# salute-developers/GigaAM

Hardware: AMD Instinct MI355X
Metric: RTFx v2_ctc batch32x20s (log-mel + encoder + greedy decode) (higher is better)
Workload: dtype f32 (GEMMs: 3-term split on fp16 MFMA, fp32 accumulate)

## Files before the change

### gigaam_amd/_lib.py

```python
from __future__ import annotations

import ctypes as C
import os
from typing import Optional

_HERE = os.path.dirname(os.path.abspath(__file__))
LIB_NAME = "libgigaam_hip.so"
LIB_PATH = os.path.join(_HERE, LIB_NAME)

SUBS_CONV2D, SUBS_CONV1D = 0, 1
ATT_ROTARY, ATT_REL_POS = 0, 1
NORM_BATCH, NORM_LAYER = 0, 1
HEAD_NONE, HEAD_CTC, HEAD_RNNT, HEAD_EMO = 0, 1, 2, 3
DTYPE_F32, DTYPE_F16, DTYPE_BF16, DTYPE_F64, DTYPE_I64 = 0, 1, 2, 3, 4
GEMM_F32, GEMM_F16X3, GEMM_F16 = 0, 1, 2
RS_U8, RS_I16, RS_I24, RS_I32, RS_F32, RS_MULAW, RS_ALAW = range(7)
RS_FORM_SINGLE, RS_FORM_TABLE, RS_FORM_ROWS = 0, 1, 2
PF_CLASSES = ["gemm", "conv2", "attn", "norm", "convmod", "stem", "frontend", "decode", "misc", "align_bt", "align_out"]


class GamConfig(C.Structure):
    _fields_ = [(n, C.c_int32) for n in (
        "sample_rate", "n_mels", "hop_length", "win_length", "n_fft", "center",
        "feat_in", "n_layers", "d_model", "subsampling", "subs_kernel_size", "subsampling_factor",
# ... 30 lines not shown
    "gam_ctc_greedy": (C.c_int, [_P, _P, _P, C.c_int, C.c_int64, _P, _P, _P, _P]),
    "gam_ctc_align": (C.c_int, [_P, _P, _P, C.c_int, C.c_int64, _P, _P, C.c_int, _P, _P, _P, _P, _P, _P, _P]),
    "gam_op_ctc_align": (C.c_int, [_P, _P, _P, C.c_int, C.c_int64, C.c_int, _P, _P, C.c_int, _P, _P, _P, _P, _P, _P, _P]),
    "gam_op_ctc_align_long": (C.c_int, [_P, _P, C.c_int64, C.c_int, _P, C.c_int, _P, _P, _P, _P, _P, _P, _P]),
    "gam_op_ctc_star_row": (C.c_int, [_P, _P, _P, C.c_int, C.c_int64, C.c_int, C.c_float, _P, _P]),
    "gam_ctc_align_star": (C.c_int, [_P, _P, _P, C.c_int, C.c_int64, _P, _P, C.c_int, C.c_float, _P, _P, _P, _P, _P, _P, _P]),
    "gam_op_ctc_align_star": (C.c_int, [_P, _P, _P, C.c_int, C.c_int64, C.c_int, _P, _P, _P, C.c_int, _P, _P, _P, _P, _P, _P, _P]),
    "gam_op_ctc_align_long_star": (C.c_int, [_P, _P, C.c_int64, C.c_int, _P, _P, C.c_int, _P, _P, _P, _P, _P, _P, _P]),
    "gam_op_ctc_stitch": (C.c_int, [_P, _P, _P, C.c_int, C.c_int64, C.c_int, _P, _P, _P, _P, C.c_int64, _P, _P]),
    "gam_op_ctc_greedy_long": (C.c_int, [_P, _P, C.c_int64, C.c_int, _P, _P, _P, _P]),
    "gam_set_ctc_align_workspace": (C.c_int, [_P, C.c_int64]),
    "gam_tune_ctc_align_long": (C.c_int, [C.c_int, C.c_int]),
    "gam_ctc_kws": (C.c_int, [_P, _P, _P, C.c_int, C.c_int64, C.c_int, _P, _P, _P, _P, _P, _P]),
    "gam_op_ctc_kws": (C.c_int, [_P, _P, _P, C.c_int, C.c_int64, C.c_int, C.c_int, _P, _P, _P, _P, _P, _P]),
    "gam_set_keywords": (C.c_int, [_P, _P, _P, C.c_int, _P]),
    "gam_ctc_kws_state_bytes": (C.c_int64, [_P]),
    "gam_op_ctc_kws_stream": (C.c_int, [_P, _P, C.c_int64, C.c_int, C.c_int64, C.c_int, _P, C.c_int, _P, _P, _P, _P, _P, _P, _P]),
    "gam_ctc_beam": (C.c_int, [_P, _P, _P, C.c_int, C.c_int64, C.c_int, _P, _P, _P, _P, _P, _P]),
    "gam_op_ctc_beam": (C.c_int, [_P, _P, _P, C.c_int, C.c_int64, C.c_int, C.c_int, _P, _P, _P, _P, _P, _P]),
    "gam_ctc_beam_stream_bytes": (C.c_int64, [_P, C.c_int, C.c_int64]),
    "gam_op_ctc_beam_stream": (C.c_int, [_P, _P, C.c_int64, C.c_int, C.c_int64, C.c_int, C.c_int, _P, C.c_int64, _P, _P, _P, _P, _P, _P, _P]),
    "gam_set_hotwords": (C.c_int, [_P, _P, _P, C.c_int, C.c_float]),
    "gam_set_lm": (C.c_int, [_P, _P, C.c_int, _P, C.c_int64, C.c_int, _P, C.c_int64, C.c_int, C.c_int, C.c_int, C.c_int, C.c_int,
                             C.c_float, C.c_float, C.c_float]),
    "gam_rnnt_greedy": (C.c_int, [_P, _P, _P, C.c_int, C.c_int64, C.c_int, _P, _P, _P, _P, _P, C.c_int, _P]),
    "gam_ctc_beam_nbest": (C.c_int, [_P, _P, _P, C.c_int, C.c_int64, C.c_int, C.c_int, _P, _P, _P, _P, _P, _P, _P]),
    "gam_op_ctc_beam_nbest": (C.c_int, [_P, _P, _P, C.c_int, C.c_int64, C.c_int, C.c_int, C.c_int, _P, _P, _P, _P, _P, _P, _P]),
    "gam_rnnt_beam_nbest": (C.c_int, [_P, _P, _P, C.c_int, C.c_int64, C.c_int, C.c_int, C.c_int, _P, _P, _P, _P, _P, _P, _P]),
    "gam_op_rnnt_beam_nbest": (C.c_int, [_P, _P, _P, C.c_int, C.c_int64, C.c_int, C.c_int, C.c_int, _P, _P, _P, _P, _P, _P, _P]),
    "gam_rnnt_beam": (C.c_int, [_P, _P, _P, C.c_int, C.c_int64, C.c_int, C.c_int, _P, _P, _P, _P, _P, _P]),
    "gam_op_rnnt_beam": (C.c_int, [_P, _P, _P, C.c_int, C.c_int64, C.c_int, C.c_int, _P, _P, _P, _P, _P, _P]),
    "gam_rnnt_align": (C.c_int, [_P, _P, _P, C.c_int, C.c_int64, _P, _P, C.c_int, _P, _P, _P, _P, _P]),
    "gam_op_rnnt_align": (C.c_int, [_P, _P, _P, C.c_int, C.c_int64, _P, _P, C.c_int, _P, _P, _P, _P, _P, _P]),
    "gam_op_rnnt_lattice_align": (C.c_int, [_P, _P, _P, C.c_int, C.c_int64, C.c_int, _P, _P, C.c_int, _P, _P, _P, _P, _P]),
    "gam_set_rnnt_align_workspace": (C.c_int, [_P, C.c_int64]),
    "gam_ctc_confidence": (C.c_int, [_P, _P, _P, C.c_int, C.c_int64, _P, _P, _P, C.c_int, C.c_int, C.c_int, _P, _P, _P, _P]),
    "gam_op_ctc_confidence": (C.c_int, [_P, _P, _P, C.c_int, C.c_int64, C.c_int, _P, _P, _P, C.c_int, C.c_int, C.c_int, _P, _P, _P, _P]),
    "gam_rnnt_confidence": (C.c_int, [_P, _P, _P, C.c_int, C.c_int64, _P, _P, _P, C.c_int, C.c_int, _P, _P, _P]),
    "gam_op_rnnt_confidence": (C.c_int, [_P, _P, _P, C.c_int, C.c_int64, _P, _P, _P, C.c_int, C.c_int, _P, _P, _P]),
    "gam_emo_probs": (C.c_int, [_P, _P, _P, C.c_int, C.c_int64, _P, _P]),
    "gam_rnnt_predict": (C.c_int, [_P, _P, _P, _P, C.c_int, _P, _P, _P, _P]),
    "gam_rnnt_joint": (C.c_int, [_P, _P, _P, C.c_int, C.c_int, C.c_int, _P, _P]),
    "gam_set_gemm_mode": (C.c_int, [_P, C.c_int]),
    "gam_get_gemm_mode": (C.c_int, [_P]),
    "gam_set_rnnt_cluster": (C.c_int, [_P, C.c_int]),
    "gam_get_rnnt_cluster": (C.c_int, [_P]),
    "gam_rnnt_cluster_plan_info": (C.c_int, [C.c_int] * 8 + [C.POINTER(C.c_int32)]),
    "gam_rnnt_last_decode": (C.c_int, [_P, C.POINTER(C.c_int32)]),
    "gam_debug_buffer_hash": (C.c_int, [_P, C.c_int, C.POINTER(C.c_uint64), C.POINTER(C.c_int64)]),
    "gam_range_flag": (C.c_int, [_P, C.POINTER(C.c_int), _P]),
    "gam_range_flag_fetch": (C.c_int, [_P, _P, _P]),
    "gam_op_gemm": (C.c_int, [_P, _P, _P, _P, _P, C.c_int, C.c_int, C.c_int, C.c_int, _P]),
    "gam_op_gemm_ex": (C.c_int, [_P, _P, _P, _P, _P, C.c_float, _P, C.c_int, C.c_int, C.c_int, C.c_int, _P]),
    "gam_op_attention": (C.c_int, [_P, _P, _P, _P, _P, _P, C.c_int, C.c_int, C.c_int, _P]),
    "gam_op_attention_ex": (C.c_int, [_P, _P, _P, _P, C.c_int64, _P, _P, _P, C.c_int, C.c_int, C.c_int, C.c_int, _P, _P, _P, _P]),
    "gam_op_layernorm": (C.c_int, [_P, C.POINTER(GamLnOp), _P]),
    "gam_op_convmod": (C.c_int, [_P, _P, _P, _P, _P, _P, _P, _P, _P, C.c_int, C.c_int, C.c_int, C.c_int, C.c_int, C.c_int, C.c_int, _P]),
    "gam_tune_sp": (C.c_int, [C.c_int, C.c_int, C.c_int]),
    "gam_plan_sp": (C.c_int, [C.c_int, C.c_int, C.c_int, C.c_int, C.POINTER(C.c_int), C.POINTER(C.c_int), C.POINTER(C.c_int)]),
    "gam_plan_sp_ex": (C.c_int, [C.c_int, C.c_int, C.c_int, C.c_int, C.POINTER(C.c_int), C.POINTER(C.c_int), C.POINTER(C.c_int), C.POINTER(C.c_int)]),
    "gam_tune_sp_stages": (C.c_int, [C.c_int]),
    "gam_resample_plan": (C.c_int, [C.c_int, C.c_int, C.POINTER(C.c_int), C.POINTER(C.c_int), C.POINTER(C.c_int)]),
    "gam_resample_tile": (C.c_int, [C.c_int, C.c_int, C.POINTER(C.c_int), C.POINTER(C.c_int)]),
    "gam_resample_table": (C.c_int, [C.c_int, C.c_int, _P, _P]),
    "gam_resample_out_len": (C.c_int64, [C.c_int, C.c_int, C.c_int64]),
    "gam_op_resample": (C.c_int, [_P, C.c_int, C.c_int, C.c_int, _P, C.c_int, C.c_int64, C.c_int, C.c_int, _P, _P, _P, C.c_int64, _P, _P]),
    "gam_profile_enable": (C.c_int, [_P, C.c_int]),
    "gam_profile_pause": (C.c_int, [_P, C.c_int]),
    "gam_profile_read": (C.c_int, [_P, C.c_int, C.POINTER(C.c_double), C.POINTER(C.c_int64), C.POINTER(C.c_double)]),
    "gam_profile_read_bytes": (C.c_int, [_P, C.c_int, C.POINTER(C.c_double)]),
    "gam_last_error": (C.c_char_p, [_P]),
    "gam_comm_unique_id": (C.c_int, [C.c_char_p]),
    "gam_comm_create": (C.c_int, [C.c_char_p, C.c_int, C.c_int, C.c_int, C.POINTER(_P)]),
    "gam_comm_world": (C.c_int, [_P]),
    "gam_gather_ids": (C.c_int, [_P, _P, _P, _P, _P, C.c_int, C.c_int, _P, _P, _P, _P, _P]),
    "gam_comm_last_error": (C.c_char_p, [_P]),
    "gam_comm_destroy": (None, [_P]),
}

_lib: Optional[C.CDLL] = None


class GigaAMHipError(RuntimeError):
    pass


def load_library(path: Optional[str] = None) -> C.CDLL:
    global _lib
    if _lib is not None and path is None:
        return _lib
    p = path or os.environ.get("GIGAAM_HIP_LIB", LIB_PATH)
    if not os.path.exists(p):
        raise GigaAMHipError(
            f"{p} not found: the HIP extension is not built. Run `python -c 'import __graft_entry__ as g; g.build()'` "
            "(hipcc --offload-arch=gfx950). There is no CPU fallback.")
    lib = C.CDLL(p)
    for name, (res, args) in SIGNATURES.items():
        fn = getattr(lib, name)
        fn.restype = res
        fn.argtypes = args
    if lib.gam_abi_version() != 1:
        raise GigaAMHipError("libgigaam_hip.so ABI version mismatch")
    if path is None:
        _lib = lib
    return lib
```

### gigaam_amd/csrc/gam_api.hip

```cpp
#include <hip/hip_runtime.h>

#include <algorithm>
#include <cmath>
#include <cstdarg>
#include <cstdio>
#include <cstring>
#include <map>
#include <string>
#include <vector>

#include "../../include/gigaam_hip.h"
#include "gam_align.h"
#include "gam_align_long.h"
#include "gam_kws.h"
#include "gam_attn.h"
#include "gam_beam.h"
#include "gam_beam_stream.h"
#include "gam_rnnt_beam.h"
#include "gam_attn16.h"
#include "gam_comm.h"
#include "gam_common.h"
#include "gam_convmod.h"
#include "gam_decode.h"
#include "gam_rnnt_align.h"
// ... 2 lines not shown
#include "gam_frontend.h"
#include "gam_gemm.h"
#include "gam_gemm_sp.h"
#include "gam_norm.h"
#include "gam_pack.h"
#include "gam_resample.h"
#include "gam_stem.h"
#include "gam_stitch.h"

namespace {

struct HostTensor {
  std::vector<float> data;
  std::vector<int64_t> shape;
  int64_t numel() const {
    int64_t n = 1;
    for (auto s : shape) n *= s;
    return n;
  }
};

struct DevBuf {
  float* p = nullptr;
  size_t cap = 0;
  DevBuf() = default;
  DevBuf(DevBuf&& o) noexcept : p(o.p), cap(o.cap) { o.p = nullptr; o.cap = 0; }
  DevBuf& operator=(DevBuf&& o) noexcept { std::swap(p, o.p); std::swap(cap, o.cap); return *this; }
  ~DevBuf() { (void)release(); }
  hipError_t release() {
    const hipError_t e = p ? hipFree(p) : hipSuccess;
    p = nullptr; cap = 0;
    return e;
  }
  hipError_t alloc(size_t floats) {
    hipError_t e = release();
    if (e == hipSuccess) e = hipMalloc(&p, floats * sizeof(float));
    if (e == hipSuccess) cap = floats; else p = nullptr;
    return e;
  }
  template <class T> T* as() const { return reinterpret_cast<T*>(p); }
};

struct W16 {
  _Float16* sp = nullptr;
  _Float16* h16 = nullptr;
  float inv = 1.0f;
};

struct LayerW {
  float *ln_ff1_w, *ln_ff1_b, *ff1_w1, *ff1_b1, *ff1_w2, *ff1_b2;
  float *ln_att_w, *ln_att_b, *wqkv, *bqkv, *wo, *bo;
  float *wpos, *pos_u, *pos_v;
  float *ln_conv_w, *ln_conv_b, *pw1_w, *pw1_b, *dw_w, *dw_b, *cn_scale, *cn_shift, *pw2_w, *pw2_b;
  float *ln_ff2_w, *ln_ff2_b, *ff2_w1, *ff2_b1, *ff2_w2, *ff2_b2;
  float *ln_out_w, *ln_out_b;
  W16 s_ff1_w1, s_ff1_w2, s_wqkv, s_wo, s_wpos, s_pw1, s_pw2, s_ff2_w1, s_ff2_w2;
};

struct ProfEvent {
  hipEvent_t a, b;
  int cls;
};

}

struct gam_handle {
  gam_config cfg;
  int device = 0;
  bool finalized = false;
  bool has_encoder = false, has_head = false;
  std::map<std::string, HostTensor> staged;
  std::vector<DevBuf> owned;
  std::string err;

  float* dft_basis = nullptr;
  int* mel_band = nullptr;
  float* mel_wts = nullptr;
  int mel_nw = 0;
  int nf = 0, kpad = 0;
  float *c1_w = nullptr, *c1_b = nullptr, *c2_w = nullptr, *c2_b = nullptr, *lin_w = nullptr, *lin_b = nullptr;
  W16 s_c1, s_c2, s_lin;
  int gemm_mode = 1;
  int f1 = 0, f2 = 0;
  std::vector<LayerW> layers;
  float *rot_cos = nullptr, *rot_sin = nullptr;
  float* rel_pe = nullptr;
  float* rel_pe_sp = nullptr;
  float *ctc_w = nullptr, *ctc_b = nullptr;
  float *emo_w = nullptr, *emo_b = nullptr;
  float *jn_enc_w = nullptr, *jn_enc_b = nullptr, *jn_pred_t = nullptr, *jn_pred_b = nullptr;
  float *jn_out_w = nullptr, *jn_out_b = nullptr, *lstm_whh_t = nullptr, *lstm_tab = nullptr;
  float *lstm_whh_q = nullptr, *jn_pred_q = nullptr;
  float* jn_pred_w = nullptr;
  DevBuf jz, jp, jl;
  float *lstm_wih_x = nullptr, *lstm_whh_x = nullptr, *lstm_bias_x = nullptr;
  int use_rowscale = 1;
  int use_range = 1;
  int ncu = 256;
  int rnnt_cluster = -1;
  int rnnt_coop = 1;
  int rnnt_force_timeout = 0;
  int rnnt_no_repair = 0;
  int rnnt_exclusive = 0;
  int last_rnnt_c = 0, last_rnnt_kern = -1, last_rnnt_refused = 0;
  DevBuf rnnt_x;
  hipEvent_t dec_evt = nullptr;
  hipStream_t dec_stream = nullptr;
  bool dec_evt_set = false;

  DevBuf wavp, spec, img, c2, xin, y1, x, y, yr, hbuf, qkv, ctx, ubuf, zbuf, tok, logits, encp, pbuf, aplanes;
  DevBuf op_planes, op_sp, splitk_ws;
  DevBuf align_star;
  DevBuf align_bp;
  DevBuf align_long_ws;
  DevBuf greedy_long_ws;
  size_t al_ws_limit = GAM_AL_WS_DEFAULT;
  DevBuf beam_nodes;
  DevBuf rb_ws, rb_nodes;
  DevBuf ra_g, ra_pp, ra_lat, ra_bp;
  DevBuf cf_stats;
  size_t ra_ws_limit = GAM_RA_WS_DEFAULT;
  DevBuf hw_trie;
  int hw_nodes = 0, hw_words = 0, hw_max_tok = -1;
  float hw_boost = 0.f;
  int hw_gen = 0, lm_gen = 0;
  DevBuf kw_dev;
  int kw_K = 0, kw_ntok = 0, kw_max_tok = -1;
  int kw_gen = 0;
  DevBuf kws_mb;
  DevBuf lm_cls, lm_wt, lm_ng;
  int lm_V = 0, lm_wslots = 0, lm_wprobe = 0, lm_nslots = 0, lm_nprobe = 0, lm_order = 0, lm_bos = 0, lm_eos = 0, lm_unk = 0;
  float lm_unk_logp = 0.f, lm_alpha = 0.f, lm_beta = 0.f;
  DevBuf dec_splitk_ws;
  int last_rows = 0, last_rows_padded = 0;
  DevBuf pack_idx;
  int use_pack = 1;
  int use_splitk = 1;
  int fuse_reduce = 1;
  int use_graph = 1;
  int graph_max_rows = 2048;
  uint64_t ws_generation = 0;
  struct GraphEntry {
    enum Seen { UNSEEN, SEEN_ONCE, PLAIN_ONLY };
    uint64_t gen = 0; Seen seen = UNSEEN; hipGraphExec_t exec = nullptr;
  };
  std::map<std::vector<int>, GraphEntry> graphs;
  long graph_replays = 0, graph_captures_failed = 0;
  int graph_count = 0;
  hipStream_t cap_stream = nullptr;
  DevBuf lens;
  DevBuf rsbuf, op_rs;
  int* range_flag = nullptr;

  int prof_on = 0;
  std::vector<ProfEvent> prof_events;
  size_t prof_used = 0;
  double prof_work[GAM_PF_NCLASS] = {0};
  double prof_bytes[GAM_PF_NCLASS] = {0};
  int64_t prof_launches[GAM_PF_NCLASS] = {0};
};

namespace {

int fail(gam_handle* h, int code, const char* fmt, ...) {
  char buf[512];
  va_list ap;
  va_start(ap, fmt);
  vsnprintf(buf, sizeof buf, fmt, ap);
  va_end(ap);
  if (h) h->err = buf;
  return code;
}

#define HIPCHK(h, expr)                                                                        \
  do {                                                                                         \
    hipError_t e_ = (expr);                                                                    \
    if (e_ != hipSuccess) return fail(h, -2, "%s failed: %s (%s:%d)", #expr, hipGetErrorString(e_), __FILE__, __LINE__); \
  } while (0)

void* dev_upload(gam_handle* h, const void* src, size_t bytes, size_t alloc_bytes) {
  h->owned.emplace_back();
  DevBuf& b = h->owned.back();
  if (b.alloc((alloc_bytes + 3) / 4) != hipSuccess) return nullptr;
  if (src && bytes && hipMemcpy(b.p, src, bytes, hipMemcpyHostToDevice) != hipSuccess) return nullptr;
  return b.p;
}

float* upload(gam_handle* h, const std::vector<float>& v) {
  return (float*)dev_upload(h, v.data(), v.size() * sizeof(float), std::max<size_t>(v.size(), 4) * sizeof(float));
}

// ... 104 lines not shown
  gam_handle* h;
  hipStream_t s;
  ProfEvent* ev = nullptr;
  ProfScope(gam_handle* h_, hipStream_t s_, int cls, double work) : h(h_), s(s_) {
    if (!h->prof_on || (h->prof_on == 2 && cls != GAM_PF_GEMM && cls != GAM_PF_CONV2)) return;
    if (h->prof_used == h->prof_events.size()) {
      ProfEvent e;
      if (hipEventCreate(&e.a) != hipSuccess || hipEventCreate(&e.b) != hipSuccess) return;
      h->prof_events.push_back(e);
    }
    ev = &h->prof_events[h->prof_used++];
    ev->cls = cls;
    h->prof_work[cls] += work;
    h->prof_launches[cls] += 1;
    hipEventRecord(ev->a, s);
  }
  ~ProfScope() {
    if (ev) hipEventRecord(ev->b, s);
  }
};

struct PendingReduce {
  const float* part = nullptr;
  int nsplit = 0;
  const float* bias = nullptr;
  const float* resid = nullptr;
  float alpha = 1.0f;
  GamGemmArgs full;
  int act = 0;
  void clear() { part = nullptr; nsplit = 0; }
};

int flush_pending(gam_handle* h, hipStream_t s, PendingReduce* p) {
  if (p == nullptr || p->part == nullptr) return 0;
  const hipError_t e = gam_launch_splitk_reduce(p->full, p->act, p->nsplit, s);
  const int M = p->full.M, N = p->full.N;
  p->clear();
  if (e != hipSuccess) return fail(h, -2, "split-K reduce launch (M=%d N=%d): %s", M, N, hipGetErrorString(e));
  return 0;
}

static inline bool split_mode(const gam_handle* h) { return h->gemm_mode != GAM_GEMM_F32; }

int gemm(gam_handle* h, hipStream_t s, const GamGemmArgs& a_in, int act, int cls = GAM_PF_GEMM, const W16* w16 = nullptr,
         PendingReduce* defer = nullptr) {
  GamGemmArgs a = a_in;
  if (int r = flush_pending(h, s, defer)) return r;
  a.range_flag = h->use_range ? h->range_flag : nullptr;
  if (!split_mode(h)) a.c_guard = 0;
  ProfScope ps(h, s, cls, 2.0 * (double)a.M * (double)a.N * (double)a.K);
  if (ps.ev) {
    const double abytes = a.a_mode == 0 ? ((double)(a.M - 1) * (double)std::min<long>(a.lda, a.K) + a.K) * 4.0
                                        : (double)a.M / a.conv_f2 * 2.0 * a.conv_fp * a.conv_c * 4.0;
    h->prof_bytes[cls] += abytes * (a.n_switch > 0 ? 2.0 : 1.0) + 4.0 * a.N * a.K + 4.0 * a.M * a.N * (a.R ? 2.0 : 1.0);
  }
  hipError_t e;
  if (a.Asp != nullptr) {
    if (!split_mode(h)) return fail(h, -2, "sp32 A operand outside the split-fp16 GEMM mode");
    if (w16 == nullptr || w16->sp == nullptr) return fail(h, -2, "sp32 A without sp32 W planes");
    a.wscale_inv = w16->inv;
    a.Wsp = w16->sp;
    a.h16 = 0;
    if (a.a_fmt == 2) {
      if (a.K % 64 != 0 || (a.a_mode == 0 ? a.lda % 64 != 0 : a.conv_c % 64 != 0) || w16->h16 == nullptr)
        return fail(h, -2, "GAM_GEMM_F16: K / row pitch of a GEMM operand is not a multiple of 64 (M=%d N=%d K=%d)", a.M, a.N, a.K);
      a.h16 = 1; a.K /= 2; a.lda /= 2; a.conv_c /= 2;
      a.Wsp = w16->h16;
    }
    GamSpPlan plan = gam_gemm_sp_plan(a.M, a.N, a.K, a.a_mode, h->ncu);
    if (!h->use_splitk) plan.s = 1;
    a.sp_mt = plan.mt; a.sp_nw = plan.nw; a.sp_ns = plan.ns;
    GamGemmArgs full = a;
    if (plan.s > 1) {
      if (int r = ensure(h, h->splitk_ws, (size_t)plan.s * a.M * a.N + 64)) return r;
      a.splitk = plan.s; a.partial = h->splitk_ws.p;
    }
    e = gam_launch_gemm_sp(a, act, s);
    if (e != hipSuccess) return fail(h, -2, "sp gemm launch (M=%d N=%d K=%d): %s", a.M, a.N, a.K, hipGetErrorString(e));
    if (plan.s > 1 && defer != nullptr && h->fuse_reduce && act == GAM_ACT_NONE && !a.c_split && !a.c_guard && a.lens == nullptr &&
        !a.remap && a.ldc == a.N && a.bias != nullptr && a.R != nullptr && a.ldr == a.N) {
      defer->part = a.partial; defer->nsplit = plan.s; defer->bias = a.bias; defer->resid = a.R; defer->alpha = a.alpha;
      defer->full = full; defer->full.partial = a.partial; defer->act = act;
    } else if (plan.s > 1) {
      full.partial = a.partial;
      e = gam_launch_splitk_reduce(full, act, plan.s, s);
      if (e != hipSuccess) return fail(h, -2, "split-K reduce launch (M=%d N=%d): %s", a.M, a.N, hipGetErrorString(e));
    }
    return 0;
  }
  if (a.a_rs != nullptr || a.c_split) return fail(h, -2, "row-scaled A or split C without sp32 operands (M=%d N=%d K=%d)", a.M, a.N, a.K);
  int S = 1;
  if (h->use_splitk && a.a_mode == 0 && a.K % 32 == 0) {
    const int tiles = gam_cdiv(a.M, 128) * gam_cdiv(a.N, 128), nk = a.K / 32, ncu = 256;
    if (tiles * 2 <= ncu && nk >= 4) {
      S = std::min(16, std::min(ncu / tiles, nk / 2));
      while (S > 1 && nk % S != 0) --S;
    }
  }
  GamGemmArgs full = a;
  if (S > 1) {
    DevBuf& ws = cls == GAM_PF_DECODE ? h->dec_splitk_ws : h->splitk_ws;
    if (int r = ensure(h, ws, (size_t)S * a.M * a.N + 64)) return r;
    a.splitk = S; a.ldw = a.K; a.K = a.K / S; a.partial = ws.p;
  }
  e = gam_launch_gemm(a, act, s);
  if (e != hipSuccess) return fail(h, -2, "gemm launch (M=%d N=%d K=%d): %s", a.M, a.N, a.K, hipGetErrorString(e));
  if (S > 1) {
// ... 33 lines not shown

int64_t half_up(int64_t l) { return l <= 0 ? 0 : (l + 1) / 2; }

struct DecodeScope {
  gam_handle* h;
  hipStream_t s;
  DecodeScope(gam_handle* h_, hipStream_t s_) : h(h_), s(s_) {
    if (h->dec_evt == nullptr && hipEventCreateWithFlags(&h->dec_evt, hipEventDisableTiming) != hipSuccess) { h->dec_evt = nullptr; (void)hipGetLastError(); }
    if (h->dec_evt != nullptr && h->dec_evt_set && h->dec_stream != s) (void)hipStreamWaitEvent(s, h->dec_evt, 0);
  }
  ~DecodeScope() {
    if (h->dec_evt != nullptr && hipEventRecord(h->dec_evt, s) == hipSuccess) { h->dec_stream = s; h->dec_evt_set = true; }
  }
};

#define GAM_DECODE_ENTRY(h, stream)      \
  hipStream_t s = (hipStream_t)(stream); \
  if (!(h)) return -1;                   \
  HIPCHK(h, hipSetDevice((h)->device));  \
  DecodeScope ds(h, s)

int head_check(gam_handle* h, int want, const char* who) {
  if (!h) return -1;
  if (who && !h->finalized) return fail(h, -1, "%s before gam_finalize", who);
  if (h->cfg.head_type != want || !h->has_head)
    return fail(h, -1, "model has no %s head", want == GAM_HEAD_CTC ? "CTC" : want == GAM_HEAD_RNNT ? "RNN-T" : "emotion");
  return 0;
}

template <class Args> void rnnt_pred_weights(const gam_handle* h, Args& a) {
  a.gate_tab = h->lstm_tab; a.whh_t = h->lstm_whh_t; a.wih_x = h->lstm_wih_x; a.whh_x = h->lstm_whh_x; a.bias_x = h->lstm_bias_x;
}
template <class Args> void rnnt_joint_weights(const gam_handle* h, Args& a) {
  a.wpred_t = h->jn_pred_t; a.bpred = h->jn_pred_b; a.wout = h->jn_out_w; a.bout = h->jn_out_b;
}

}

extern "C" {

int gam_abi_version(void) { return GAM_ABI_VERSION; }

const char* gam_last_error(const gam_handle* h) { return h ? h->err.c_str() : "null handle"; }

int gam_create(const gam_config* cfg, int device_id, gam_handle** out) {
  if (!cfg || !out) return -1;
  gam_handle* h = new gam_handle();
  h->cfg = *cfg;
  h->device = device_id;
  *out = h;
  if (const char* e = getenv("GAM_SPLITK")) h->use_splitk = atoi(e);
  if (const char* e = getenv("GAM_PACK")) h->use_pack = atoi(e);
  if (const char* e = getenv("GAM_FUSE_REDUCE")) h->fuse_reduce = atoi(e);
  if (const char* e = getenv("GAM_GRAPH")) h->use_graph = atoi(e);
  if (const char* e = getenv("GAM_GRAPH_MAX_ROWS")) h->graph_max_rows = atoi(e);
  if (const char* e = getenv("GAM_RNNT_CLUSTER")) h->rnnt_cluster = std::max(-1, std::min(8, atoi(e)));
  if (const char* e = getenv("GAM_RNNT_ALIGN_WS")) h->ra_ws_limit = (size_t)std::max(1ll, atoll(e));
  if (const char* e = getenv("GAM_CTC_ALIGN_WS")) h->al_ws_limit = (size_t)std::max(1ll, atoll(e));
  if (const char* e = getenv("GAM_RNNT_EXCLUSIVE")) h->rnnt_exclusive = atoi(e);
  if (const char* e = getenv("GAM_RNNT_COOP")) h->rnnt_coop = atoi(e);
  if (const char* e = getenv("GAM_RNNT_FORCE_TIMEOUT")) h->rnnt_force_timeout = atoi(e);
  if (const char* e = getenv("GAM_RNNT_NO_REPAIR")) h->rnnt_no_repair = atoi(e);
  {
    int n = 0;
    if (hipDeviceGetAttribute(&n, hipDeviceAttributeMultiprocessorCount, device_id) == hipSuccess && n > 0) h->ncu = n;
    int co = 0;
    if (hipDeviceGetAttribute(&co, hipDeviceAttributeCooperativeLaunch, device_id) != hipSuccess || co == 0) h->rnnt_coop = 0;
  }
  if (const char* e = getenv("GAM_ROWSCALE")) h->use_rowscale = atoi(e);
  if (const char* e = getenv("GAM_RANGE")) h->use_range = atoi(e);
  if (const char* e = getenv("GAM_GEMM_MODE"))
    h->gemm_mode = strcmp(e, "f32") == 0 ? GAM_GEMM_F32 : (strcmp(e, "f16") == 0 ? GAM_GEMM_F16 : GAM_GEMM_F16X3);
  const gam_config& c = h->cfg;
  if (c.d_model <= 0 || c.n_heads <= 0 || c.d_model % c.n_heads != 0)
    return fail(h, -1, "bad d_model/n_heads %d/%d", c.d_model, c.n_heads);
  if (c.d_model / c.n_heads != GAM_ATT_DK) return fail(h, -1, "head dim %d unsupported (kernels are built for %d)", c.d_model / c.n_heads, GAM_ATT_DK);
  if (c.d_model % 64 != 0 || c.d_model > 1024) return fail(h, -1, "d_model %d unsupported", c.d_model);
  if (c.subsampling_factor != 4) return fail(h, -1, "subsampling_factor %d unsupported", c.subsampling_factor);
  if (c.subsampling == GAM_SUBS_CONV2D && c.subs_kernel_size != 3) return fail(h, -1, "conv2d stem needs kernel 3");
  if (c.subsampling == GAM_SUBS_CONV1D && c.subs_kernel_size != 5) return fail(h, -1, "conv1d stem needs kernel 5");
  if (c.win_length != c.n_fft) return fail(h, -1, "win_length != n_fft unsupported");
  if (c.n_mels > 64 || c.n_mels != c.feat_in) return fail(h, -1, "n_mels %d / feat_in %d unsupported", c.n_mels, c.feat_in);
  if (c.head_type == GAM_HEAD_RNNT && (c.pred_rnn_layers < 1 || c.pred_rnn_layers > 4 || c.pred_hidden > GAM_RNNT_MAXH || c.joint_hidden > GAM_RNNT_MAXH || c.num_classes > GAM_RNNT_MAXV || c.joint_hidden % 16 != 0 || c.pred_hidden % 16 != 0))
    return fail(h, -1, "RNN-T head shape unsupported");
  if (hipSetDevice(device_id) != hipSuccess) return fail(h, -2, "hipSetDevice(%d) failed", device_id);
  return 0;
}

void gam_destroy(gam_handle* h) {
  if (!h) return;
  hipSetDevice(h->device);
  for (auto& e : h->prof_events) { hipEventDestroy(e.a); hipEventDestroy(e.b); }
  for (auto& g : h->graphs)
    if (g.second.exec) hipGraphExecDestroy(g.second.exec);
  if (h->cap_stream) hipStreamDestroy(h->cap_stream);
  if (h->dec_evt) hipEventDestroy(h->dec_evt);
  if (getenv("GAM_GRAPH_DEBUG")) fprintf(stderr, "[gam] graph replays %ld, failed captures %ld\n", h->graph_replays, h->graph_captures_failed);
  delete h;
}

int gam_set_weight(gam_handle* h, const char* key, const void* host_ptr, int dtype, const int64_t* shape, int ndim) {
  if (!h || !key || !host_ptr) return -1;
  if (h->finalized) return fail(h, -1, "gam_set_weight after gam_finalize");
  HostTensor t;
  for (int i = 0; i < ndim; ++i) t.shape.push_back(shape[i]);
  const int64_t n = t.numel();
// ... 148 lines not shown
  if (int r = need(h, pe + "conv.0.bias", C, &b0)) return r;
  if (int r = need(h, pe + "conv.2.weight", (int64_t)C * C * ks, &w2)) return r;
  if (int r = need(h, pe + "conv.2.bias", C, &b2)) return r;
  const std::vector<float> r0 = swap_inner(w0->data, C, F, ks), r2 = swap_inner(w2->data, C, C, ks);
  if (int r = upload_to(h, DST(h->c1_w), r0)) return r;
  if (int r = up_split(h, r0, &h->s_c1, ks * F)) return r;
  if (int r = upload_to(h, DST(h->c1_b), b0->data)) return r;
  if (int r = upload_to(h, DST(h->c2_w), r2)) return r;
  if (int r = up_split(h, r2, &h->s_c2, ks * C)) return r;
  return upload_to(h, DST(h->c2_b), b2->data);
}

static int fin_qkv(gam_handle* h, const std::string& p, LayerW& L) {
  const int D = h->cfg.d_model;
  const HostTensor *wq, *bq, *wk, *bk, *wv, *bv;
  if (int r = need(h, p + "self_attn.linear_q.weight", (int64_t)D * D, &wq)) return r;
  if (int r = need(h, p + "self_attn.linear_q.bias", D, &bq)) return r;
  if (int r = need(h, p + "self_attn.linear_k.weight", (int64_t)D * D, &wk)) return r;
  if (int r = need(h, p + "self_attn.linear_k.bias", D, &bk)) return r;
  if (int r = need(h, p + "self_attn.linear_v.weight", (int64_t)D * D, &wv)) return r;
  if (int r = need(h, p + "self_attn.linear_v.bias", D, &bv)) return r;
  std::vector<float> w(wq->data), b(bq->data);
  w.insert(w.end(), wk->data.begin(), wk->data.end());
  w.insert(w.end(), wv->data.begin(), wv->data.end());
  b.insert(b.end(), bk->data.begin(), bk->data.end());
  b.insert(b.end(), bv->data.begin(), bv->data.end());
  if (int r = upload_to(h, DST(L.wqkv), w)) return r;
  if (int r = upload_to(h, DST(L.bqkv), b)) return r;
  return up_split(h, w, &L.s_wqkv, D);
}

static int fin_conv_norm(gam_handle* h, const std::string& p, LayerW& L) {
  const int D = h->cfg.d_model;
  const HostTensor *g, *be;
  if (int r = need(h, p + "conv.batch_norm.weight", D, &g)) return r;
  if (int r = need(h, p + "conv.batch_norm.bias", D, &be)) return r;
  if (h->cfg.conv_norm_type != GAM_NORM_BATCH) {
    if (int r = upload_to(h, DST(L.cn_scale), g->data)) return r;
    return upload_to(h, DST(L.cn_shift), be->data);
  }
  const HostTensor *rm, *rv;
  if (int r = need(h, p + "conv.batch_norm.running_mean", D, &rm)) return r;
  if (int r = need(h, p + "conv.batch_norm.running_var", D, &rv)) return r;
  std::vector<float> sc(D), sh(D);
  for (int i = 0; i < D; ++i) {
    const float inv = 1.0f / sqrtf(rv->data[i] + 1e-5f);
    sc[i] = g->data[i] * inv;
    sh[i] = be->data[i] - rm->data[i] * sc[i];
  }
  if (int r = upload_to(h, DST(L.cn_scale), sc)) return r;
  return upload_to(h, DST(L.cn_shift), sh);
}

static int fin_layer(gam_handle* h, int li, LayerW& L) {
  const gam_config& c = h->cfg;
  const int D = c.d_model, DFF = D * c.ff_expansion_factor;
  const std::string p = "encoder.layers." + std::to_string(li) + ".";
  memset(&L, 0, sizeof L);
  if (int r = upload_ln(h, p + "norm_feed_forward1", D, DST(L.ln_ff1_w), DST(L.ln_ff1_b))) return r;
  if (int r = upload_linear(h, p + "feed_forward1.linear1", DFF, D, DST(L.ff1_w1), DST(L.ff1_b1), &L.s_ff1_w1)) return r;
  if (int r = upload_linear(h, p + "feed_forward1.linear2", D, DFF, DST(L.ff1_w2), DST(L.ff1_b2), &L.s_ff1_w2)) return r;
  if (int r = upload_ln(h, p + "norm_self_att", D, DST(L.ln_att_w), DST(L.ln_att_b))) return r;
  if (int r = fin_qkv(h, p, L)) return r;
  if (int r = upload_linear(h, p + "self_attn.linear_out", D, D, DST(L.wo), DST(L.bo), &L.s_wo)) return r;
  if (c.self_attention_model == GAM_ATT_REL_POS) {
    const HostTensor *wp, *pu, *pv;
    if (int r = need(h, p + "self_attn.linear_pos.weight", (int64_t)D * D, &wp)) return r;
    if (int r = need(h, p + "self_attn.pos_bias_u", D, &pu)) return r;
    if (int r = need(h, p + "self_attn.pos_bias_v", D, &pv)) return r;
    if (int r = upload_to(h, DST(L.wpos), wp->data)) return r;
    if (int r = up_split(h, wp->data, &L.s_wpos, D)) return r;
    if (int r = upload_to(h, DST(L.pos_u), pu->data)) return r;
    if (int r = upload_to(h, DST(L.pos_v), pv->data)) return r;
  }
  if (int r = upload_ln(h, p + "norm_conv", D, DST(L.ln_conv_w), DST(L.ln_conv_b))) return r;
  if (int r = upload_linear(h, p + "conv.pointwise_conv1", 2 * D, D, DST(L.pw1_w), DST(L.pw1_b), &L.s_pw1)) return r;
  if (int r = upload_linear(h, p + "conv.depthwise_conv", D, c.conv_kernel_size, DST(L.dw_w), DST(L.dw_b), nullptr)) return r;
  if (int r = fin_conv_norm(h, p, L)) return r;
  if (int r = upload_linear(h, p + "conv.pointwise_conv2", D, D, DST(L.pw2_w), DST(L.pw2_b), &L.s_pw2)) return r;
  if (int r = upload_ln(h, p + "norm_feed_forward2", D, DST(L.ln_ff2_w), DST(L.ln_ff2_b))) return r;
  if (int r = upload_linear(h, p + "feed_forward2.linear1", DFF, D, DST(L.ff2_w1), DST(L.ff2_b1), &L.s_ff2_w1)) return r;
  if (int r = upload_linear(h, p + "feed_forward2.linear2", D, DFF, DST(L.ff2_w2), DST(L.ff2_b2), &L.s_ff2_w2)) return r;
  return upload_ln(h, p + "norm_out", D, DST(L.ln_out_w), DST(L.ln_out_b));
}

static int fin_rotary(gam_handle* h) {
  const int dk = h->cfg.d_model / h->cfg.n_heads, half = dk / 2, n = h->cfg.pos_emb_max_len;
  std::vector<float> cs((size_t)n * half), sn((size_t)n * half);
  for (int i = 0; i < half; ++i) {
    const float inv_freq = 1.0f / powf((float)n, (float)(2 * i) / (float)dk);
    for (int t = 0; t < n; ++t) {
      const float fr = (float)t * inv_freq;
      cs[(size_t)t * half + i] = (float)cos((double)fr);
      sn[(size_t)t * half + i] = (float)sin((double)fr);
    }
  }
  if (int r = upload_to(h, DST(h->rot_cos), cs)) return r;
  return upload_to(h, DST(h->rot_sin), sn);
}

static int fin_rel_pos(gam_handle* h) {
  const int D = h->cfg.d_model, n = h->cfg.pos_emb_max_len;
  std::vector<float> pe((size_t)(2 * n - 1) * D);
  for (int i = 0; i < D / 2; ++i) {
    const float w = expf((float)(2 * i) * (float)(-(log(10000.0) / D)));
    for (int r = -(n - 1); r <= n - 1; ++r) {
      const float ang = (float)r * w;
      pe[(size_t)(r + n - 1) * D + 2 * i] = (float)sin((double)ang);
      pe[(size_t)(r + n - 1) * D + 2 * i + 1] = (float)cos((double)ang);
    }
  }
  if (int r = upload_to(h, DST(h->rel_pe), pe)) return r;
  h->rel_pe_sp = (float*)dev_upload(h, nullptr, 0, pe.size() * sizeof(float));
  if (!h->rel_pe_sp) return fail(h, -2, "device upload failed (h->rel_pe_sp)");
  hipLaunchKernelGGL(gam_to_sp32_kernel, dim3((int)std::min<size_t>((pe.size() / 4 + 255) / 256, 4096)), dim3(256), 0, nullptr, h->rel_pe,
                     reinterpret_cast<_Float16*>(h->rel_pe_sp), pe.size() / 4, (const float*)nullptr, D);
  HIPCHK(h, hipGetLastError());
  HIPCHK(h, hipStreamSynchronize(nullptr));
  return 0;
}

static int fin_rnnt_upper(gam_handle* h) {
  const int PH = h->cfg.pred_hidden, LX = h->cfg.pred_rnn_layers - 1;
  const size_t G = (size_t)4 * PH;
  std::vector<float> wih_x(LX * PH * G), whh_x(LX * PH * G), bias_x(LX * G);
  for (int l = 1; l <= LX; ++l) {
    const std::string sfx = "_l" + std::to_string(l);
    const HostTensor *wi, *wh, *bi, *bh;
    if (int r = need(h, "head.decoder.lstm.weight_ih" + sfx, (int64_t)4 * PH * PH, &wi)) return r;
// ... 105 lines not shown
  if (B <= 0 || L <= 0) return fail(h, -1, "bad shape B=%d L=%lld", B, (long long)L);
  const gam_config& c = h->cfg;
  hipStream_t s = (hipStream_t)stream;
  HIPCHK(h, hipSetDevice(h->device));
  const int hop = c.hop_length, n = c.n_fft, half = n / 2;
  if (c.center && L <= half) return fail(h, -1, "input of %lld samples is too short for reflect padding (%d)", (long long)L, half);
  const int64_t Tf = gam_feat_frames(h, L);
  if (Tf <= 0) return fail(h, -1, "input of %lld samples yields no frames", (long long)L);
  const int64_t need = (Tf - 1) * hop + h->kpad;
  const int64_t Tfa = (need + hop - 1) / hop;
  const int64_t Lp = Tfa * hop;
  const int lds = (2 * h->nf + 3) / 4 * 4;
  if (int r = ensure(h, h->wavp, (size_t)B * Lp + h->kpad + 64)) return r;
  if (int r = ensure(h, h->spec, (size_t)B * Tfa * lds)) return r;
  {
    ProfScope ps(h, s, GAM_PF_FRONTEND, (double)B * (L + Lp) * 4.0);
    dim3 grid(gam_cdiv(Lp, 256), B);
    hipLaunchKernelGGL(gam_pad_wav_kernel, grid, dim3(256), 0, s, wav, h->wavp.p, B, (long)L, (long)Lp, half, c.center);
    HIPCHK(h, hipGetLastError());
    HIPCHK(h, hipMemsetAsync(h->wavp.p + (size_t)B * Lp, 0, (h->kpad + 64) * sizeof(float), s));
  }
  GamGemmArgs g = gemm_args(h->wavp.p, hop, h->dft_basis, nullptr, h->spec.p, lds, (int)(B * Tfa), 2 * h->nf, h->kpad);
  if (int r = gemm(h, s, g, GAM_ACT_NONE, GAM_PF_FRONTEND, nullptr)) return r;
  {
    GamPowMelArgs a;
    a.spec = h->spec.p; a.wts = h->mel_wts; a.nw = h->mel_nw; a.band = h->mel_band; a.feat = feat; a.wav_len = (const long long*)wav_len; a.feat_len = (long long*)feat_len;
    a.B = B; a.Tfa = (int)Tfa; a.Tf = (int)Tf; a.nf = h->nf; a.n_mels = c.n_mels; a.lds = lds;
    a.hop = hop; a.win = c.win_length; a.center = c.center;
    ProfScope ps(h, s, GAM_PF_FRONTEND, (double)B * Tf * (2.0 * h->nf + c.n_mels) * 4.0);
    dim3 grid(gam_cdiv(Tf, 64), B);
    const size_t pm_lds = (size_t)(64 * (h->nf + 1) + h->mel_nw) * sizeof(float);
    if (pm_lds > 160 * 1024) return fail(h, -1, "n_fft %d: the power / mel kernel's LDS image (%zu bytes) does not fit", c.n_fft, pm_lds);
    if (pm_lds > 64 * 1024) {
      static std::atomic<unsigned long long> attr_devs{0};
      HIPCHK(h, gam_set_max_lds(reinterpret_cast<const void*>(gam_powmel_kernel), (int)pm_lds, attr_devs));
    }
    hipLaunchKernelGGL(gam_powmel_kernel, grid, dim3(256), pm_lds, s, a);
    HIPCHK(h, hipGetLastError());
  }
  return 0;
}

struct EncPlan {
  int B;
  int64_t T;
  int T1, Tv;
  int Ta, N;
  int NR, Tmax;
  int T1a;
  int D, DFF, F, H, dk, nl;
  bool conv2d, rel, packed;
  bool sp;
  int spf;
  bool sp_stem;
  bool graph;
};

struct EncBufs {
  int *len0, *len1, *len2, *elen;
  int *cu, *row_t, *row_src;
  float* rs;
};

struct EncCtx {
  EncPlan p;
  EncBufs w;
  GamLnArgs ln;
};

static int enc_plan(gam_handle* h, int B, int64_t T, int n_layers_run, const int64_t* feat_len_host, EncPlan& p) {
  const gam_config& c = h->cfg;
  if (B <= 0 || T <= 0) return fail(h, -1, "bad shape B=%d T=%lld", B, (long long)T);
  p.B = B; p.T = T;
  p.D = c.d_model; p.F = c.feat_in; p.H = c.n_heads; p.dk = p.D / p.H; p.DFF = p.D * c.ff_expansion_factor;
  p.T1 = (int)half_up(T); p.Tv = (int)half_up(p.T1);
  if (p.Tv > c.pos_emb_max_len) return fail(h, -1, "%d encoder frames exceed pos_emb_max_len %d", p.Tv, c.pos_emb_max_len);
  if (p.Tv <= 0) return fail(h, -1, "no encoder frames");
  p.conv2d = c.subsampling == GAM_SUBS_CONV2D;
  p.rel = c.self_attention_model == GAM_ATT_REL_POS;
  p.nl = n_layers_run < 0 ? c.n_layers : std::min(n_layers_run, c.n_layers);
  p.Ta = p.conv2d ? std::max(p.Tv + 1, (p.T1 + 3) / 2) : std::max(p.Tv, (p.T1 + 5) / 2);
  p.N = B * p.Ta;
  const int pad = (c.subs_kernel_size - 1) / 2;
  p.T1a = p.conv2d ? 0 : std::max(p.T1, (int)((T + 2 * pad + 1) / 2));
  p.packed = false;
  p.NR = p.N; p.Tmax = p.Ta;
  const bool pack_regime = h->use_pack >= 2 || !h->use_graph || p.N >= h->graph_max_rows;
  if (feat_len_host != nullptr && h->use_pack && pack_regime && B > 1 && B <= 1024) {
    long long sum = 0;
    int mx = 0;
    for (int b = 0; b < B; ++b) {
      const int64_t l = std::min<int64_t>(std::max<int64_t>(feat_len_host[b], 0), T);
      const int l2 = (int)half_up(half_up(l));
      sum += l2;
      mx = std::max(mx, l2);
    }
    if (sum > 0 && sum * 100 <= (long long)p.N * 97) { p.packed = true; p.NR = (int)sum; p.Tmax = mx; }
  }
  p.sp = split_mode(h) && p.D % 32 == 0 && p.DFF % 32 == 0;
  const bool f16_fmt_ok = p.D % 64 == 0 && p.DFF % 64 == 0;
  p.spf = p.sp ? (h->gemm_mode == GAM_GEMM_F16 && f16_fmt_ok ? 2 : 1) : 0;
  p.sp_stem = p.sp && p.F % 32 == 0;
  p.graph = h->use_graph && !h->prof_on && p.nl > 0 && p.N < h->graph_max_rows && !p.packed;
  return 0;
}

static int enc_workspace(gam_handle* h, const EncPlan& p, EncBufs& w) {
  const size_t B = p.B, N = p.N, D = p.D, Ta = p.Ta;
  if (int r = ensure(h, h->lens, 4 * B)) return r;
  const size_t maxB = h->lens.cap / 4;
  w.len0 = h->lens.as<int>(); w.len1 = w.len0 + maxB; w.len2 = w.len0 + 2 * maxB; w.elen = w.len0 + 3 * maxB;
  if (int r = ensure(h, h->x, N * D)) return r;
  if (int r = ensure(h, h->y, N * D)) return r;
  if (int r = ensure(h, h->yr, N * D)) return r;
  if (int r = ensure(h, h->hbuf, N * p.DFF)) return r;
  if (int r = ensure(h, h->qkv, N * 3 * D)) return r;
  if (int r = ensure(h, h->ctx, N * D)) return r;
  if (int r = ensure(h, h->ubuf, N * 2 * D)) return r;
  if (int r = ensure(h, h->zbuf, N * D)) return r;
  if (int r = ensure(h, h->rsbuf, N + 64)) return r;
  if (p.packed)
    if (int r = ensure(h, h->pack_idx, (size_t)1032 + 2 * N)) return r;
  w.cu = p.packed ? reinterpret_cast<int*>(h->pack_idx.p) : nullptr;
  w.row_t = p.packed ? w.cu + 1032 : nullptr;
  w.row_src = p.packed ? w.row_t + N : nullptr;
  w.rs = p.sp && h->use_rowscale ? h->rsbuf.p : nullptr;
  if (p.conv2d) {
    if (int r = ensure(h, h->img, (B * 2 * Ta + 2) * (h->f1 + 1) * D)) return r;
    if (int r = ensure(h, h->c2, N * h->f2 * D)) return r;
  } else {
    if (int r = ensure(h, h->xin, (B * 2 * p.T1a + 8) * p.F)) return r;
    if (int r = ensure(h, h->y1, (B * 2 * Ta + 8) * D)) return r;
  }
  if (p.rel)
    if (int r = ensure(h, h->pbuf, (size_t)(2 * p.Tv - 1) * D)) return r;
  if (p.graph)
    if (int r = ensure(h, h->splitk_ws, (size_t)16 * N * std::max(p.DFF, 2 * p.D) + 64)) return r;
  return 0;
}

static GamLnArgs enc_ln_args(const gam_handle* h, const EncPlan& p, const EncBufs& w) {
  GamLnArgs ln;
  memset(&ln, 0, sizeof ln);
  ln.rows = p.NR; ln.d = p.D; ln.ta = p.Ta; ln.row_t = w.row_t; ln.dk = p.dk; ln.eps = 1e-5f; ln.rcos = h->rot_cos; ln.rsin = h->rot_sin;
  ln.rope_rows = h->cfg.pos_emb_max_len;
  ln.rs = w.rs;
  return ln;
}

static int enc_lengths(gam_handle* h, hipStream_t s, const EncPlan& p, const EncBufs& w, const int64_t* feat_len) {
  ProfScope ps(h, s, GAM_PF_MISC, 0.0);
  hipLaunchKernelGGL(gam_lengths_kernel, dim3(gam_cdiv(p.B, 64)), dim3(64), 0, s, (const long long*)feat_len, p.B, (int)p.T, 2,
                     w.len0, w.len1, w.len2, w.elen);
  HIPCHK(h, hipGetLastError());
  if (p.packed) {
    hipLaunchKernelGGL(gam_pack_index_kernel, dim3(1), dim3(256), 0, s, w.len2, p.B, p.Ta, p.NR, w.cu, w.row_t, w.row_src, h->range_flag);
    HIPCHK(h, hipGetLastError());
  }
  return 0;
}

static inline void gemm_formats(GamGemmArgs& g, int a_fmt, const float* a_rs, int c_split, int c_guard) {
  if (a_fmt) { g.Asp = reinterpret_cast<const _Float16*>(g.A); g.a_fmt = a_fmt; }
  g.a_rs = a_rs; g.c_split = c_split; g.c_guard = c_guard;
}

static int stem_conv2d(gam_handle* h, hipStream_t s, const EncPlan& p, const EncBufs& w, const float* feat) {
  const int B = p.B, Ta = p.Ta, N = p.N, C = p.D, D = p.D, FP = h->f1 + 1, F2 = h->f2;
  {
    GamConv1Args a;
    a.feat = feat; a.img = h->img.p; a.w = h->c1_w; a.bias = h->c1_b; a.len0 = w.len0; a.len1 = w.len1;
// ... 23 lines not shown
static int stem_conv1d(gam_handle* h, hipStream_t s, const EncPlan& p, const EncBufs& w, const float* feat) {
  const int B = p.B, Ta = p.Ta, T1a = p.T1a, N = p.N, C = p.D, D = p.D, F = p.F;
  const int64_t T = p.T;
  const int ks = h->cfg.subs_kernel_size, pad = (ks - 1) / 2;
  const int fmt = p.sp_stem ? 1 : 0;
  {
    ProfScope ps(h, s, GAM_PF_STEM, (double)B * T * F * 8.0);
    HIPCHK(h, hipMemsetAsync(h->xin.p, 0, ((size_t)B * 2 * T1a + 8) * F * sizeof(float), s));
    HIPCHK(h, hipMemsetAsync(h->y1.p, 0, ((size_t)B * 2 * Ta + 8) * C * sizeof(float), s));
    dim3 grid(gam_cdiv(T, 32), gam_cdiv(F, 32), B);
    int* const rf = h->use_range ? h->range_flag : nullptr;
    if (p.sp_stem) hipLaunchKernelGGL(gam_feat_to_rows_kernel<1>, grid, dim3(256), 0, s, feat, h->xin.p, w.len0, B, F, (int)T, 2 * T1a, pad, rf);
    else hipLaunchKernelGGL(gam_feat_to_rows_kernel<0>, grid, dim3(256), 0, s, feat, h->xin.p, w.len0, B, F, (int)T, 2 * T1a, pad, rf);
    HIPCHK(h, hipGetLastError());
  }
  GamGemmArgs g1 = gemm_args(h->xin.p, 2L * F, h->c1_w, h->c1_b, h->y1.p, C, B * T1a, C, ks * F);
  g1.lens = w.len1; g1.rpb = T1a; g1.fdiv = 1;
  g1.remap = 1; g1.out_rpb = 2 * Ta; g1.out_shift = pad; g1.rows_valid = std::min(T1a, 2 * Ta - pad);
  gemm_formats(g1, fmt, nullptr, fmt, 1);
  if (int r = gemm(h, s, g1, GAM_ACT_RELU, GAM_PF_CONV2, &h->s_c1)) return r;
  GamGemmArgs g2 = gemm_args(h->y1.p, 2L * C, h->c2_w, h->c2_b, p.packed ? h->y.p : h->x.p, D, N, D, ks * C);
  g2.lens = w.len2; g2.rpb = Ta; g2.fdiv = 1;
  gemm_formats(g2, fmt, nullptr, 0, 0);
  return gemm(h, s, g2, GAM_ACT_RELU, GAM_PF_CONV2, &h->s_c2);
}

static int enc_stem(gam_handle* h, hipStream_t s, const EncPlan& p, const EncBufs& w, const float* feat) {
  if (int r = p.conv2d ? stem_conv2d(h, s, p, w, feat) : stem_conv1d(h, s, p, w, feat)) return r;
  if (p.packed) {
    ProfScope ps(h, s, GAM_PF_STEM, (double)p.NR * p.D * 8.0);
    hipLaunchKernelGGL(gam_gather_rows_kernel, dim3(std::min(4096, gam_cdiv(p.NR * (p.D / 4), 256))), dim3(256), 0, s, h->y.p, w.row_src, h->x.p, p.NR, p.D);
    HIPCHK(h, hipGetLastError());
  }
  return 0;
}

static int launch_attention(gam_handle* h, hipStream_t s, const float* q, const float* k, const float* v, long ldq, float* ctx, int ctx_split,
                            const int* lens, const int* cu, int B, int Ta, int Tv, int H, const float* pbuf, const float* pos_u,
                            const float* pos_v) {
  const int D = H * GAM_ATT_DK;
  GamAttnArgs at;
  memset(&at, 0, sizeof at);
  at.q = q; at.k = k; at.v = v; at.ctx = ctx; at.ctx_split = ctx_split; at.lens = lens; at.cu = cu;
  at.B = B; at.Ta = Ta; at.Tv = Tv; at.H = H; at.ldq = ldq; at.ldv = ldq; at.ldo = D;
  at.scale = 1.0f / sqrtf((float)GAM_ATT_DK);
  at.pbuf = pbuf; at.pos_u = pos_u; at.pos_v = pos_v; at.ldp = D;
  hipError_t e = gam_launch_attn_mode(at, GAM_ATT_DK, split_mode(h), s, h->gemm_mode == GAM_GEMM_F16 ? 1 : 3, h->ncu);
  if (e != hipSuccess) return fail(h, -2, "attention launch: %s", hipGetErrorString(e));
  return 0;
}

static hipError_t launch_convmod(gam_handle* h, hipStream_t s, const float* u, float* z, const float* dw_w, const float* dw_b, const float* n_scale,
                                 const float* n_shift, const int* lens, const int* cu, int B, int Ta, int Tv, int d, int ks, bool layer_norm,
                                 int z_split) {
  GamConvModArgs cm;
  memset(&cm, 0, sizeof cm);
  cm.u = u; cm.z = z; cm.dw_w = dw_w; cm.dw_b = dw_b; cm.n_scale = n_scale; cm.n_shift = n_shift;
  cm.lens = lens; cm.cu = cu; cm.B = B; cm.Ta = Ta; cm.Tv = Tv; cm.d = d; cm.ks = ks; cm.eps = 1e-5f;
  cm.z_split = z_split; cm.range_flag = h->use_range ? h->range_flag : nullptr;
  return gam_launch_convmod(cm, layer_norm, s);
}

static int norm_to_y(gam_handle* h, hipStream_t s, const EncCtx& c, const float* w, const float* b, PendingReduce* pend) {
  GamLnArgs a = c.ln;
  a.x = h->x.p; a.out1 = h->y.p; a.w1 = w; a.b1 = b;
  a.split1 = c.p.spf;
  return layernorm(h, s, a, 0, pend);
}

static int ffn_block(gam_handle* h, hipStream_t s, const EncCtx& c, const float* w1, const float* b1, const W16& s_w1, const float* w2,
                     const float* b2, const W16& s_w2, PendingReduce* pend) {
  const int D = c.p.D, DFF = c.p.DFF, NR = c.p.NR, spf = c.p.spf;
  GamGemmArgs g = gemm_args(h->y.p, D, w1, b1, h->hbuf.p, DFF, NR, DFF, D);
  gemm_formats(g, spf, c.w.rs, spf, 1);
  if (int r = gemm(h, s, g, GAM_ACT_SILU, GAM_PF_GEMM, &s_w1)) return r;
  GamGemmArgs g2 = gemm_args(h->hbuf.p, DFF, w2, b2, h->x.p, D, NR, D, DFF);
  g2.R = h->x.p; g2.ldr = D; g2.alpha = 0.5f;
  gemm_formats(g2, spf, nullptr, 0, 0);
  return gemm(h, s, g2, GAM_ACT_NONE, GAM_PF_GEMM, &s_w2, pend);
}

static int attn_block(gam_handle* h, hipStream_t s, const EncCtx& c, const LayerW& L, PendingReduce* pend) {
  const EncPlan& p = c.p;
  const int D = p.D, NR = p.NR, Tv = p.Tv, spf = p.spf;
  float* const rs = c.w.rs;
  GamLnArgs a = c.ln;
  a.x = h->x.p; a.out1 = h->y.p; a.out2 = h->yr.p; a.w1 = L.ln_att_w; a.b1 = L.ln_att_b;
  a.split1 = spf; a.split2 = spf;
  if (int r = layernorm(h, s, a, p.rel ? 0 : 1, pend)) return r;
  const bool one_launch = p.rel || (p.sp && (2 * D) % 256 == 0);
  if (one_launch) {
    GamGemmArgs gq = gemm_args(p.rel ? h->y.p : h->yr.p, D, L.wqkv, L.bqkv, h->qkv.p, 3 * D, NR, 3 * D, D);
    gemm_formats(gq, spf, rs, 0, 1);
    if (!p.rel) { gq.Asp2 = reinterpret_cast<const _Float16*>(h->y.p); gq.n_switch = 2 * D; }
    if (int r = gemm(h, s, gq, GAM_ACT_NONE, GAM_PF_GEMM, &L.s_wqkv)) return r;
  } else {
    GamGemmArgs gq = gemm_args(h->yr.p, D, L.wqkv, L.bqkv, h->qkv.p, 3 * D, NR, 2 * D, D);
    gemm_formats(gq, spf, rs, 0, 1);
    if (int r = gemm(h, s, gq, GAM_ACT_NONE, GAM_PF_GEMM, &L.s_wqkv)) return r;
    W16 wv16 = L.s_wqkv;
    const size_t off = (size_t)2 * D * D;
    wv16.h16 += off;
    if (wv16.sp) wv16.sp += 2 * off;
    GamGemmArgs gv = gemm_args(h->y.p, D, L.wqkv + off, L.bqkv + 2 * D, h->qkv.p + 2 * D, 3 * D, NR, D, D);
    gemm_formats(gv, spf, rs, 0, 1);
    if (int r = gemm(h, s, gv, GAM_ACT_NONE, GAM_PF_GEMM, &wv16)) return r;
  }
  if (p.rel) {
    const size_t pe0 = (size_t)(h->cfg.pos_emb_max_len - 1 - (Tv - 1)) * D;
    GamGemmArgs gp = gemm_args(h->rel_pe + pe0, D, L.wpos, nullptr, h->pbuf.p, D, 2 * Tv - 1, D, D);
    if (p.sp) { gp.Asp = reinterpret_cast<const _Float16*>(h->rel_pe_sp + pe0); gp.a_fmt = 1; }
    if (int r = gemm(h, s, gp, GAM_ACT_NONE, GAM_PF_GEMM, &L.s_wpos)) return r;
  }
  {
    ProfScope ps(h, s, GAM_PF_ATTN, 4.0 * (double)p.B * p.H * (double)Tv * Tv * p.dk);
    if (int r = launch_attention(h, s, h->qkv.p, h->qkv.p + D, h->qkv.p + 2 * D, 3 * D, h->ctx.p, spf, p.B > 1 ? c.w.len2 : nullptr, c.w.cu, p.B,
                                 p.packed ? p.Tmax : p.Ta, Tv, p.H, p.rel ? h->pbuf.p : nullptr, L.pos_u, L.pos_v))
      return r;
  }
  GamGemmArgs go = gemm_args(h->ctx.p, D, L.wo, L.bo, h->x.p, D, NR, D, D);
  go.R = h->x.p; go.ldr = D;
  gemm_formats(go, spf, nullptr, 0, 0);
  return gemm(h, s, go, GAM_ACT_NONE, GAM_PF_GEMM, &L.s_wo, pend);
}

static int conv_block(gam_handle* h, hipStream_t s, const EncCtx& c, const LayerW& L, PendingReduce* pend) {
  const EncPlan& p = c.p;
  const int D = p.D, NR = p.NR, ks = h->cfg.conv_kernel_size;
  if (int r = norm_to_y(h, s, c, L.ln_conv_w, L.ln_conv_b, pend)) return r;
  GamGemmArgs g1 = gemm_args(h->y.p, D, L.pw1_w, L.pw1_b, h->ubuf.p, 2 * D, NR, 2 * D, D);
  gemm_formats(g1, p.spf, c.w.rs, 0, 0);
  if (int r = gemm(h, s, g1, GAM_ACT_NONE, GAM_PF_GEMM, &L.s_pw1)) return r;
  {
    ProfScope ps(h, s, GAM_PF_CONVMOD, (double)NR * D * 3 * 4.0);
    hipError_t e = launch_convmod(h, s, h->ubuf.p, h->zbuf.p, L.dw_w, L.dw_b, L.cn_scale, L.cn_shift, c.w.len2, c.w.cu, p.B,
                                  p.packed ? p.Tmax : p.Ta, p.Tv, D, ks, h->cfg.conv_norm_type == GAM_NORM_LAYER, p.spf);
    if (e != hipSuccess) return fail(h, -2, "conv-module launch (k=%d): %s", ks, hipGetErrorString(e));
  }
  GamGemmArgs g2 = gemm_args(h->zbuf.p, D, L.pw2_w, L.pw2_b, h->x.p, D, NR, D, D);
  g2.R = h->x.p; g2.ldr = D;
  gemm_formats(g2, p.spf, nullptr, 0, 0);
  return gemm(h, s, g2, GAM_ACT_NONE, GAM_PF_GEMM, &L.s_pw2, pend);
}

static int norm_out_block(gam_handle* h, hipStream_t s, const EncCtx& c, const LayerW& L, const LayerW* next, PendingReduce* pend) {
  GamLnArgs a = c.ln;
  a.x = h->x.p; a.out1 = h->x.p; a.w1 = L.ln_out_w; a.b1 = L.ln_out_b;
  if (next != nullptr) {
    a.out2 = h->y.p; a.w2 = next->ln_ff1_w; a.b2 = next->ln_ff1_b;
    a.split2 = c.p.spf;
    return layernorm(h, s, a, 2, pend);
  }
  a.rs = nullptr;
  return layernorm(h, s, a, 0, pend);
}

static int run_layers(gam_handle* h, hipStream_t s, const EncCtx& c) {
  const int nl = c.p.nl;
  if (nl > 0)
    if (int r = norm_to_y(h, s, c, h->layers[0].ln_ff1_w, h->layers[0].ln_ff1_b, nullptr)) return r;
  PendingReduce pend;
  for (int li = 0; li < nl; ++li) {
    const LayerW& L = h->layers[li];
    if (int r = ffn_block(h, s, c, L.ff1_w1, L.ff1_b1, L.s_ff1_w1, L.ff1_w2, L.ff1_b2, L.s_ff1_w2, &pend)) return r;
    if (int r = attn_block(h, s, c, L, &pend)) return r;
    if (int r = conv_block(h, s, c, L, &pend)) return r;
    if (int r = norm_to_y(h, s, c, L.ln_ff2_w, L.ln_ff2_b, &pend)) return r;
    if (int r = ffn_block(h, s, c, L.ff2_w1, L.ff2_b1, L.s_ff2_w1, L.ff2_w2, L.ff2_b2, L.s_ff2_w2, &pend)) return r;
    if (int r = norm_out_block(h, s, c, L, li + 1 < nl ? &h->layers[li + 1] : nullptr, &pend)) return r;
  }
  return flush_pending(h, s, &pend);
}

static int replay_layers(gam_handle* h, hipStream_t s, const EncCtx& c, bool* replayed) {
  typedef gam_handle::GraphEntry Entry;
  const EncPlan& p = c.p;
  *replayed = false;
  if (!p.graph) return 0;
  const GamSpForce& frc = gam_sp_force();
  const std::vector<int> key = {p.B, p.Ta, p.Tv, p.nl, h->gemm_mode, (int)p.sp, h->use_splitk, h->fuse_reduce, frc.mt.load(), frc.nw.load(), frc.s.load(), frc.ns.load()};
  Entry& ge = h->graphs[key];
  if (ge.gen != h->ws_generation) {
    if (ge.exec) { hipGraphExecDestroy(ge.exec); --h->graph_count; }
    ge = Entry();
    ge.gen = h->ws_generation;
  }
  if (ge.exec == nullptr && ge.seen == Entry::SEEN_ONCE && h->graph_count >= 32) ge.seen = Entry::PLAIN_ONLY;
  if (ge.exec == nullptr && ge.seen == Entry::SEEN_ONCE) {
    hipGraph_t graph = nullptr;
// ... 1250 lines not shown
int gam_rnnt_joint(gam_handle* h, const float* enc, const float* dec, int B, int T, int U, float* log_probs, void* stream) {
  if (int r = head_check(h, GAM_HEAD_RNNT, "gam_rnnt_joint")) return r;
  if (B <= 0 || T <= 0 || U <= 0 || !enc || !dec || !log_probs) return fail(h, -1, "bad gam_rnnt_joint arguments");
  HIPCHK(h, hipSetDevice(h->device));
  const gam_config& c = h->cfg;
  const int D = c.d_model, PH = c.pred_hidden, JH = c.joint_hidden, V = c.num_classes;
  const size_t rows = (size_t)B * T * U;
  if (rows * std::max(JH, V) > ((size_t)1 << 31)) return fail(h, -1, "gam_rnnt_joint: B x T x U = %zu rows is too large for one call", rows);
  hipStream_t s = (hipStream_t)stream;
  DecodeScope ds(h, s);
  if (int r = ensure(h, h->encp, (size_t)B * T * JH)) return r;
  if (int r = ensure(h, h->jp, (size_t)B * U * JH)) return r;
  if (int r = ensure(h, h->jz, rows * JH)) return r;
  if (int r = ensure(h, h->jl, rows * V)) return r;
  GamGemmArgs ge = gemm_args(enc, D, h->jn_enc_w, h->jn_enc_b, h->encp.p, JH, B * T, JH, D);
  if (int r = gemm(h, s, ge, GAM_ACT_NONE, GAM_PF_DECODE)) return r;
  GamGemmArgs gp = gemm_args(dec, PH, h->jn_pred_w, h->jn_pred_b, h->jp.p, JH, B * U, JH, PH);
  if (int r = gemm(h, s, gp, GAM_ACT_NONE, GAM_PF_DECODE)) return r;
  {
    ProfScope ps(h, s, GAM_PF_DECODE, (double)rows * JH * 4.0);
    const int grid = (int)std::min<size_t>((rows * JH + 255) / 256, 8192);
    hipLaunchKernelGGL(gam_joint_hidden_kernel, dim3(grid), dim3(256), 0, s, h->encp.p, h->jp.p, h->jz.p, B, T, U, JH);
    HIPCHK(h, hipGetLastError());
  }
  GamGemmArgs go = gemm_args(h->jz.p, JH, h->jn_out_w, h->jn_out_b, h->jl.p, V, (int)rows, V, JH);
  if (int r = gemm(h, s, go, GAM_ACT_NONE, GAM_PF_DECODE)) return r;
  ProfScope ps(h, s, GAM_PF_DECODE, (double)rows * V * 8.0);
  hipLaunchKernelGGL(gam_log_softmax_kernel, dim3(gam_cdiv((long)rows, 4)), dim3(256), 0, s, h->jl.p, log_probs, (int)rows, V);
  HIPCHK(h, hipGetLastError());
  return 0;
}

int gam_emo_probs(gam_handle* h, const float* encoded, const int32_t* enc_len, int B, int64_t Tp, float* probs,
                  void* stream) {
  if (int r = head_check(h, GAM_HEAD_EMO, nullptr)) return r;
  if (B <= 0 || Tp <= 0 || !encoded || !probs) return fail(h, -1, "bad emotion-head arguments");
  HIPCHK(h, hipSetDevice(h->device));
  hipStream_t s = (hipStream_t)stream;
  const int D = h->cfg.d_model, NC = h->cfg.num_classes;
  ProfScope ps(h, s, GAM_PF_DECODE, (double)B * D * Tp * 4.0);
  hipLaunchKernelGGL(gam_emo_head_kernel, dim3(B), dim3(256), (size_t)(D + NC) * sizeof(float), s, encoded, enc_len,
                     h->emo_w, h->emo_b, probs, D, (int)Tp, NC);
  HIPCHK(h, hipGetLastError());
  return 0;
}

int gam_op_gemm(gam_handle* h, const float* A, const float* W, const float* bias, float* C, int M, int N, int K, int act,
                void* stream) {
  return gam_op_gemm_ex(h, A, W, bias, nullptr, 1.0f, C, M, N, K, act, stream);
}

int gam_op_gemm_ex(gam_handle* h, const float* A, const float* W, const float* bias, const float* R, float alpha, float* C, int M,
                   int N, int K, int act, void* stream) {
  if (!h) return -1;
  HIPCHK(h, hipSetDevice(h->device));
  GamGemmArgs g = gemm_args(A, K, W, bias, C, N, M, N, K);
  g.R = R; g.ldr = N; g.alpha = alpha;
  hipStream_t s = (hipStream_t)stream;
  if (!split_mode(h) || K % 32 != 0 || N % 4 != 0) return gemm(h, s, g, act);
  const size_t wn = (size_t)N * K, an = (size_t)M * K;
  W16 w16;
  if (int r = ensure(h, h->op_sp, wn + 64)) return r;
  hipLaunchKernelGGL(gam_to_sp32_kernel, dim3((int)std::min<size_t>((wn / 4 + 255) / 256, 4096)), dim3(256), 0, s, W,
                     (_Float16*)h->op_sp.p, wn / 4, (const float*)nullptr, K);
  w16.sp = (_Float16*)h->op_sp.p;
  if (int r = ensure(h, h->op_rs, (size_t)M + 64)) return r;
  hipLaunchKernelGGL(gam_rowscale_kernel, dim3(gam_cdiv(M, 4)), dim3(256), 0, s, A, h->op_rs.p, M, K, (long)K);
  g.a_rs = h->op_rs.p;
  if (int r = ensure(h, h->aplanes, an + 64)) return r;
  g.Asp = (const _Float16*)h->aplanes.p;
  g.a_fmt = (h->gemm_mode == GAM_GEMM_F16 && K % 64 == 0) ? 2 : 1;
  if (g.a_fmt == 2) {
    if (int r = ensure(h, h->op_planes, wn / 2 + 64)) return r;
    w16.h16 = (_Float16*)h->op_planes.p;
    hipLaunchKernelGGL(gam_to_h16_kernel, dim3((int)std::min<size_t>((wn / 4 + 255) / 256, 4096)), dim3(256), 0, s, W, w16.h16,
                       wn / 4, (const float*)nullptr, K);
    hipLaunchKernelGGL(gam_to_h16_kernel, dim3((int)std::min<size_t>((an / 4 + 255) / 256, 8192)), dim3(256), 0, s, A,
                       (_Float16*)h->aplanes.p, an / 4, (const float*)h->op_rs.p, K);
  } else {
    hipLaunchKernelGGL(gam_to_sp32_kernel, dim3((int)std::min<size_t>((an / 4 + 255) / 256, 8192)), dim3(256), 0, s, A,
                       (_Float16*)h->aplanes.p, an / 4, (const float*)h->op_rs.p, K);
  }
  return gemm(h, s, g, act, GAM_PF_GEMM, &w16);
}

int gam_op_attention(gam_handle* h, const float* q, const float* k, const float* v, float* ctx, const int32_t* lens, int B,
                     int T, int H, void* stream) {
  if (!h) return -1;
  if (B <= 0 || T <= 0 || H <= 0) return fail(h, -1, "bad attention shape");
  HIPCHK(h, hipSetDevice(h->device));
  return launch_attention(h, (hipStream_t)stream, q, k, v, H * GAM_ATT_DK, ctx, 0, lens, nullptr, B, T, T, H, nullptr, nullptr, nullptr);
}

int gam_op_attention_ex(gam_handle* h, const float* q, const float* k, const float* v, int64_t ldq, float* ctx, const int32_t* lens,
                        const int32_t* cu, int B, int Ta, int Tv, int H, const float* pbuf, const float* pos_u, const float* pos_v,
                        void* stream) {
  if (!h) return -1;
  const int D = H * GAM_ATT_DK;
  if (B <= 0 || Ta <= 0 || Tv <= 0 || H <= 0) return fail(h, -1, "bad attention shape");
  if (cu == nullptr && Tv > Ta) return fail(h, -1, "attention: Tv %d > Ta %d in the padded layout", Tv, Ta);
  if (ldq < D || ldq % 4 != 0) return fail(h, -1, "attention: row stride %ld (H*48 = %d, multiple of 4)", (long)ldq, D);
  if (pbuf != nullptr && (pos_u == nullptr || pos_v == nullptr)) return fail(h, -1, "attention: pbuf without pos_u / pos_v");
  auto al16 = [](const void* p) { return (reinterpret_cast<uintptr_t>(p) & 15) == 0; };
  if (!al16(q) || !al16(k) || !al16(v) || !al16(ctx) || (pbuf && (!al16(pbuf) || !al16(pos_u) || !al16(pos_v))))
    return fail(h, -1, "attention: operands must be 16-byte aligned");
  HIPCHK(h, hipSetDevice(h->device));
  return launch_attention(h, (hipStream_t)stream, q, k, v, (long)ldq, ctx, 0, lens, cu, B, Ta, Tv, H, pbuf, pos_u, pos_v);
}

int gam_op_layernorm(gam_handle* h, const gam_ln_op* op, void* stream) {
  if (!h) return -1;
  if (!op) return fail(h, -1, "layernorm: null argument block");
  const gam_ln_op& o = *op;
  if (o.mode < 0 || o.mode > 2) return fail(h, -1, "layernorm: mode %d outside 0..2", o.mode);
  if (o.rows <= 0 || o.d <= 0) return fail(h, -1, "layernorm: bad shape rows %d d %d", o.rows, o.d);
  if (o.split1 < 0 || o.split1 > 2 || o.split2 < 0 || o.split2 > 2)
    return fail(h, -1, "layernorm: store format %d / %d outside 0..2", o.split1, o.split2);
  if (!o.out1 || !o.w1 || !o.b1) return fail(h, -1, "layernorm: out1 / w1 / b1 are mandatory");
  if (!o.part && !o.x) return fail(h, -1, "layernorm: x is mandatory without part");
  if (o.part && o.mode != 2 && !o.xstore) return fail(h, -1, "layernorm: part without xstore");
  if (o.mode != 0 && !o.out2) return fail(h, -1, "layernorm: mode %d needs out2", o.mode);
  if (o.mode == 2 && (!o.w2 || !o.b2)) return fail(h, -1, "layernorm: mode 2 needs w2 / b2");
  if (o.mode == 1) {
    if (!o.rcos || !o.rsin || o.rope_rows <= 0) return fail(h, -1, "layernorm: mode 1 needs rcos / rsin of rope_rows > 0 rows");
    if (o.dk <= 0) return fail(h, -1, "layernorm: mode 1 needs dk > 0");
    if (!o.row_t && o.ta <= 0) return fail(h, -1, "layernorm: mode 1 needs row_t or ta > 0");
  }
  auto al16 = [](const void* p) { return (reinterpret_cast<uintptr_t>(p) & 15) == 0; };
  if (!al16(o.x) || !al16(o.out1) || !al16(o.out2) || !al16(o.w1) || !al16(o.b1) || !al16(o.w2) || !al16(o.b2) || !al16(o.rcos) ||
      !al16(o.rsin) || !al16(o.part) || !al16(o.pbias) || !al16(o.presid) || !al16(o.xstore))
    return fail(h, -1, "layernorm: operands must be 16-byte aligned");
  HIPCHK(h, hipSetDevice(h->device));
  GamLnArgs a;
  memset(&a, 0, sizeof a);
  a.x = o.x; a.out1 = o.out1; a.out2 = o.out2; a.w1 = o.w1; a.b1 = o.b1; a.w2 = o.w2; a.b2 = o.b2;
  a.rcos = o.rcos; a.rsin = o.rsin; a.rows = o.rows; a.d = o.d; a.ta = o.ta; a.dk = o.dk; a.eps = o.eps;
  a.split1 = o.split1; a.split2 = o.split2; a.rs = o.rs; a.rope_rows = o.rope_rows;
  a.part = o.part; a.nsplit = o.nsplit; a.pbias = o.pbias; a.presid = o.presid; a.palpha = o.palpha; a.xstore = o.xstore;
  a.row_t = o.row_t;
  hipError_t e = gam_launch_layernorm(a, o.mode, (hipStream_t)stream);
  if (e != hipSuccess)
    return fail(h, -2, "layernorm launch (mode %d, rows %d, d %d, dk %d, split %d/%d, nsplit %d): %s", o.mode, o.rows, o.d, o.dk,
                o.split1, o.split2, o.part ? o.nsplit : 0, hipGetErrorString(e));
  return 0;
}

int gam_op_convmod(gam_handle* h, const float* u, float* z, const float* dw_w, const float* dw_b, const float* n_scale,
                   const float* n_shift, const int32_t* lens, const int32_t* cu, int B, int Ta, int Tv, int d, int ks, int layer_norm,
                   int z_split, void* stream) {
  if (!h) return -1;
  if (!h->finalized) return fail(h, -1, "gam_op_convmod before gam_finalize");
  if (!u || !z || !dw_w || !dw_b || !n_scale || !n_shift || !lens) return fail(h, -1, "conv module: null operand");
  if (B <= 0 || Ta <= 0 || Tv <= 0 || d <= 0) return fail(h, -1, "conv module: bad shape B %d Ta %d Tv %d d %d", B, Ta, Tv, d);
  if (cu == nullptr && Tv > Ta) return fail(h, -1, "conv module: Tv %d > Ta %d in the padded layout", Tv, Ta);
  if (z_split < 0 || z_split > 2) return fail(h, -1, "conv module: store format %d outside 0..2", z_split);
  if (z_split && d % 32 != 0) return fail(h, -1, "conv module: a split-fp16 z needs d %% 32 == 0 (d = %d)", d);
  auto al16 = [](const void* p) { return (reinterpret_cast<uintptr_t>(p) & 15) == 0; };
  if (d % 4 == 0 && (!al16(u) || !al16(z) || !al16(dw_b) || !al16(n_scale) || !al16(n_shift)))
    return fail(h, -1, "conv module: operands must be 16-byte aligned");
  HIPCHK(h, hipSetDevice(h->device));
  hipError_t e = launch_convmod(h, (hipStream_t)stream, u, z, dw_w, dw_b, n_scale, n_shift, lens, cu, B, Ta, Tv, d, ks, layer_norm != 0, z_split);
  if (e != hipSuccess) return fail(h, -2, "conv-module launch (k=%d, d=%d, %s): %s", ks, d, layer_norm ? "LayerNorm" : "BatchNorm", hipGetErrorString(e));
  return 0;
}

int gam_set_gemm_mode(gam_handle* h, int mode) {
  if (!h || (mode != GAM_GEMM_F32 && mode != GAM_GEMM_F16X3 && mode != GAM_GEMM_F16)) return fail(h, -1, "unknown GEMM mode %d", mode);
  h->gemm_mode = mode;
  return 0;
}

int gam_get_gemm_mode(const gam_handle* h) { return h ? h->gemm_mode : -1; }

int gam_debug_buffer_hash(gam_handle* h, int which, uint64_t* hash_out, int64_t* floats_out) {
  if (!h || !hash_out) return -1;
  const DevBuf* b = which == 0 ? &h->tok : which == 1 ? &h->encp : which == 2 ? &h->rnnt_x : which == 3 ? &h->logits : nullptr;
  if (!b) return fail(h, -1, "no such buffer %d", which);
  HIPCHK(h, hipSetDevice(h->device));
  HIPCHK(h, hipDeviceSynchronize());
  std::vector<uint32_t> host(b->cap);
  if (b->cap) HIPCHK(h, hipMemcpy(host.data(), b->p, b->cap * sizeof(float), hipMemcpyDeviceToHost));
  uint64_t x = 1469598103934665603ull;
  for (uint32_t v : host) { x ^= v; x *= 1099511628211ull; }
  *hash_out = x;
  if (floats_out) *floats_out = (int64_t)b->cap;
  return 0;
}

int gam_set_rnnt_cluster(gam_handle* h, int workgroups_per_utterance) {
  if (!h) return -1;
  if (workgroups_per_utterance < -1 || workgroups_per_utterance > 8) return fail(h, -1, "cluster size %d outside -1 (auto) .. 8", workgroups_per_utterance);
  h->rnnt_cluster = workgroups_per_utterance;
  return 0;
}

int gam_get_rnnt_cluster(gam_handle* h) { return h ? h->rnnt_cluster : -2; }

int gam_rnnt_cluster_plan_info(int ncu, int cluster, int exclusive, int B, int H, int JH, int V, int L, int32_t* out) {
  if (!out || B <= 0 || H <= 0 || JH <= 0 || V <= 0 || L <= 0) return -1;
  const RnntClusterPlan p = rnnt_cluster_plan(ncu, cluster, exclusive, B, H, JH, V, L);
  memset(out, 0, 8 * sizeof(int32_t));
  if (p.C == 0) return 0;
  out[0] = p.C; out[1] = p.nr; out[2] = p.kern; out[3] = p.resident ? 1 : 0;
  out[4] = p.wout_slice_in_lds; out[5] = p.wpred_slice_in_lds; out[6] = (int32_t)p.lds; out[7] = (int32_t)p.grid;
  return 0;
}

int gam_rnnt_last_decode(gam_handle* h, int32_t* out) {
  if (!h || !out) return -1;
  out[0] = h->last_rnnt_c; out[1] = h->last_rnnt_kern; out[2] = h->last_rnnt_refused;
  return 0;
}

int gam_last_encode_rows(gam_handle* h, int* rows_padded) {
  if (!h) return -1;
  if (rows_padded) *rows_padded = h->last_rows_padded;
  return h->last_rows;
// ... 127 lines not shown
```

### gigaam_amd/csrc/gam_common.h

```cpp
#pragma once
#include <hip/hip_runtime.h>
#include <stdint.h>
#include <math.h>

#define GAM_WAVE 64

typedef float f32x4 __attribute__((ext_vector_type(4)));
typedef float f32x2 __attribute__((ext_vector_type(2)));
typedef float f32x16 __attribute__((ext_vector_type(16)));

static inline int gam_cdiv(long a, long b) { return (int)((a + b - 1) / b); }

#include <atomic>
static inline hipError_t gam_set_max_lds(const void* kern, int bytes, std::atomic<unsigned long long>& mask) {
  int dev = 0;
  hipError_t e = hipGetDevice(&dev);
  if (e != hipSuccess) return e;
  const unsigned long long bit = 1ull << (dev & 63);
  if (mask.load(std::memory_order_acquire) & bit) return hipSuccess;
  e = hipFuncSetAttribute(kern, hipFuncAttributeMaxDynamicSharedMemorySize, bytes);
  if (e == hipSuccess) mask.fetch_or(bit, std::memory_order_release);
  return e;
}

// ... 127 lines not shown
  } else {
    _Float16* p = reinterpret_cast<_Float16*>(base) + row_off * 2 + (c >> 5) * 64 + (c & 31);
    unsigned h, l;
    gam_split2(x0, x1, h, l);
    *reinterpret_cast<unsigned*>(p) = h;
    *reinterpret_cast<unsigned*>(p + 32) = l;
  }
}
__device__ __forceinline__ void gam_store1(float* base, size_t row_off, int c, float x, int split) {
  if (!split) {
    base[row_off + c] = x;
  } else if (split == 2) {
    reinterpret_cast<_Float16*>(base)[row_off + c] = (_Float16)x;
  } else {
    _Float16* p = reinterpret_cast<_Float16*>(base) + row_off * 2 + (c >> 5) * 64 + (c & 31);
    const _Float16 h = (_Float16)x;
    p[0] = h;
    p[32] = (_Float16)(x - (float)h);
  }
}

template <int NS>
__device__ __forceinline__ f32x4 gam_sum_slices_n(const float* __restrict__ p, size_t slice) {
  f32x4 t[NS];
#pragma unroll
  for (int s_ = 0; s_ < NS; ++s_) t[s_] = *reinterpret_cast<const f32x4*>(p + s_ * slice);
  f32x4 acc = (f32x4){0.f, 0.f, 0.f, 0.f};
#pragma unroll
  for (int s_ = 0; s_ < NS; ++s_) acc += t[s_];
  return acc;
}
template <int SMAX = 16>
__device__ __forceinline__ f32x4 gam_sum_slices(const float* __restrict__ p, size_t slice, int ns) {
  switch (ns) {
    case 1: return gam_sum_slices_n<1>(p, slice);
    case 2: return gam_sum_slices_n<2>(p, slice);
    case 3: return gam_sum_slices_n<3>(p, slice);
    case 4: return gam_sum_slices_n<4>(p, slice);
    default: break;
  }
  if (SMAX >= 8) {
    if (ns == 6) return gam_sum_slices_n<6>(p, slice);
    if (ns == 8) return gam_sum_slices_n<8>(p, slice);
  }
  if (SMAX >= 16) {
    if (ns == 12) return gam_sum_slices_n<12>(p, slice);
    if (ns == 16) return gam_sum_slices_n<16>(p, slice);
  }
  f32x4 acc = (f32x4){0.f, 0.f, 0.f, 0.f};
  for (int s_ = 0; s_ < ns; ++s_) acc += *reinterpret_cast<const f32x4*>(p + s_ * slice);
  return acc;
}

enum { GAM_ACT_NONE = 0, GAM_ACT_SILU = 1, GAM_ACT_RELU = 2 };
```

### gigaam_amd/csrc/gam_convmod.h

```cpp
#pragma once
#include "gam_common.h"
#include "gam_pack.h"
#include <type_traits>

struct GamConvModArgs {
  const float* u;
  float* z;
  const float* dw_w;
  const float* dw_b;
  const float* n_scale;
  const float* n_shift;
  const int* lens;
  const int* cu;
  int B, Ta, Tv, d, ks;
  float eps;
  int z_split;
  int* range_flag;
};

template <int KS>
__global__ __launch_bounds__(512, 4) void gam_convmod_bn_kernel(GamConvModArgs a) {
  constexpr int NRG = 32, TT = 128, PAD = (KS - 1) / 2, ROWS = (TT + KS - 1 + NRG - 1) / NRG * NRG, OUT = TT / NRG;
  __shared__ f32x4 tile[ROWS * 16];
  __shared__ f32x4 wl[KS * 16];
  const int tid = threadIdx.x;
  const int q = tid & 15, rg = tid >> 4;
  const int b = blockIdx.z, c = blockIdx.y * 64 + q * 4, t0 = blockIdx.x * TT;
  int klen = a.lens[b];
  klen = klen < a.Tv ? klen : a.Tv;
  const GamRows ur = gam_rows(a.cu, b, a.Ta, klen);
  if (t0 >= ur.lim) return;
  const size_t rowbase = ur.base;
  const int rlim = ur.lim;
  constexpr int NLD = ROWS / NRG;
  f32x4 ua[NLD], ub[NLD];
#pragma unroll
  for (int u = 0; u < NLD; ++u) {
    const int t = t0 - PAD + rg + NRG * u;
    const int tc = t < 0 ? 0 : (t < rlim ? t : rlim - 1);
    const float* up = a.u + (rowbase + tc) * (size_t)(2 * a.d);
    ua[u] = *reinterpret_cast<const f32x4*>(up + c);
    ub[u] = *reinterpret_cast<const f32x4*>(up + a.d + c);
  }
  {
#pragma unroll
    for (int i = 0; i < (KS + NRG - 1) / NRG; ++i) {
      const int k = rg + NRG * i;
      if (k < KS) wl[k * 16 + q] = (f32x4){a.dw_w[(size_t)c * KS + k], a.dw_w[(size_t)(c + 1) * KS + k],
                                           a.dw_w[(size_t)(c + 2) * KS + k], a.dw_w[(size_t)(c + 3) * KS + k]};
    }
  }
#pragma unroll
  for (int u = 0; u < NLD; ++u) {
    const int rr = rg + NRG * u;
    const int t = t0 - PAD + rr;
    const bool live = t >= 0 && t < klen;
    const f32x4 glu = (f32x4){ua[u].x * gam_sigmoid(ub[u].x), ua[u].y * gam_sigmoid(ub[u].y),
                              ua[u].z * gam_sigmoid(ub[u].z), ua[u].w * gam_sigmoid(ub[u].w)};
    tile[rr * 16 + q] = live ? glu : (f32x4){0.f, 0.f, 0.f, 0.f};
  }
  __syncthreads();
  const f32x4* trow = tile + (rg * OUT) * 16 + q;
  const f32x4* wq = wl + q;
  int lofs = 0;
  f32x4 win[OUT + KS - 1];
#pragma unroll
  for (int r = 0; r < OUT + 1; ++r) win[r] = trow[r * 16];
  f32x4 acc[OUT];
#pragma unroll
  for (int i = 0; i < OUT; ++i) acc[i] = (f32x4){0.f, 0.f, 0.f, 0.f};
  f32x4 w_cur = wq[0], w_nxt = wq[16];
#pragma unroll
  for (int k = 0; k < KS; ++k) {
    const f32x4 w = w_cur;
    w_cur = w_nxt;
#pragma unroll
    for (int i = 0; i < OUT; ++i) {
      acc[i].x = fmaf(w.x, win[i + k].x, acc[i].x);
      acc[i].y = fmaf(w.y, win[i + k].y, acc[i].y);
      acc[i].z = fmaf(w.z, win[i + k].z, acc[i].z);
      acc[i].w = fmaf(w.w, win[i + k].w, acc[i].w);
    }
    static_assert(OUT == 4, "the pin below names the 16 accumulator components of a tap");
    asm volatile("" : "+v"(lofs), "+v"(acc[0].x), "+v"(acc[0].y), "+v"(acc[0].z), "+v"(acc[0].w), "+v"(acc[1].x), "+v"(acc[1].y),
                 "+v"(acc[1].z), "+v"(acc[1].w), "+v"(acc[2].x), "+v"(acc[2].y), "+v"(acc[2].z), "+v"(acc[2].w), "+v"(acc[3].x),
                 "+v"(acc[3].y), "+v"(acc[3].z), "+v"(acc[3].w));
    if (k + 2 < KS) w_nxt = wq[(k + 2) * 16 + lofs];
    if (k + OUT + 1 < OUT + KS - 1) win[k + OUT + 1] = trow[(k + OUT + 1) * 16 + lofs];
  }
  const f32x4 bias = *reinterpret_cast<const f32x4*>(a.dw_b + c);
  const f32x4 sc = *reinterpret_cast<const f32x4*>(a.n_scale + c);
  const f32x4 sh = *reinterpret_cast<const f32x4*>(a.n_shift + c);
#pragma unroll
  for (int i = 0; i < OUT; ++i) {
    const int t = t0 + rg * OUT + i;
    const f32x4 y = (acc[i] + bias) * sc + sh;
    const float v0 = gam_silu(y.x), v1 = gam_silu(y.y), v2 = gam_silu(y.z), v3 = gam_silu(y.w);
    if (t < rlim) {
      gam_range_note(a.range_flag, v0, v1, v2, v3);
      gam_store4(a.z, (rowbase + t) * (size_t)a.d, c, v0, v1, v2, v3, a.z_split);
    }
  }
}

template <int KS>
__global__ __launch_bounds__(256) void gam_convmod_ln_kernel(GamConvModArgs a) {
  constexpr int TT = 8, PAD = (KS - 1) / 2, ROWS = TT + KS - 1, MAXC = 4;
  extern __shared__ __attribute__((aligned(16))) float gam_smem_cm[];
  float* tile = gam_smem_cm;
  float* red = gam_smem_cm + ROWS * a.d;
  const int tid = threadIdx.x, lane = tid & 63, wave = tid >> 6;
  const int b = blockIdx.y, t0 = blockIdx.x * TT;
  int klen = a.lens[b];
  klen = klen < a.Tv ? klen : a.Tv;
  const GamRows ur = gam_rows(a.cu, b, a.Ta, klen);
  if (t0 >= ur.lim) return;
  const size_t rowbase = ur.base;
  const int rlim = ur.lim;
  for (int r0 = 0; r0 < ROWS; r0 += 4) {
    float ua[4][MAXC], ub[4][MAXC];
#pragma unroll
    for (int q = 0; q < 4; ++q) {
      const int t = t0 - PAD + r0 + q;
      const int tc = t < 0 ? 0 : (t < rlim ? t : rlim - 1);
      const float* up = a.u + (rowbase + tc) * (size_t)(2 * a.d);
#pragma unroll
      for (int ci = 0; ci < MAXC; ++ci) {
        const int c = tid + ci * 256 < a.d ? tid + ci * 256 : a.d - 1;
        ua[q][ci] = up[c];
        ub[q][ci] = up[a.d + c];
      }
    }
#pragma unroll
    for (int q = 0; q < 4; ++q) {
      const int rr = r0 + q, t = t0 - PAD + rr;
      const bool ok = t >= 0 && t < klen;
#pragma unroll
      for (int ci = 0; ci < MAXC; ++ci) {
        const int c = tid + ci * 256;
        if (rr < ROWS && c < a.d) tile[rr * a.d + c] = ok ? ua[q][ci] * gam_sigmoid(ub[q][ci]) : 0.f;
      }
    }
  }
  __syncthreads();
  float y[MAXC][TT];
#pragma unroll
  for (int ci = 0; ci < MAXC; ++ci) {
    const int c = tid + ci * 256;
    if (c < a.d) {
      float w[KS];
#pragma unroll
      for (int k = 0; k < KS; ++k) w[k] = a.dw_w[(size_t)c * KS + k];
      const float bias = a.dw_b[c];
#pragma unroll
      for (int i = 0; i < TT; ++i) {
        float acc = 0.f;
#pragma unroll
        for (int k = 0; k < KS; ++k) acc = fmaf(w[k], tile[(i + k) * a.d + c], acc);
        y[ci][i] = acc + bias;
      }
    } else {
#pragma unroll
      for (int i = 0; i < TT; ++i) y[ci][i] = 0.f;
    }
  }
  float mean[TT], rstd[TT];
#pragma unroll
  for (int i = 0; i < TT; ++i) {
    float s = 0.f;
#pragma unroll
    for (int ci = 0; ci < MAXC; ++ci) s += y[ci][i];
    s = gam_wave_sum(s);
    if (lane == 0) red[wave * TT + i] = s;
  }
  __syncthreads();
#pragma unroll
  for (int i = 0; i < TT; ++i) mean[i] = (red[i] + red[TT + i] + red[2 * TT + i] + red[3 * TT + i]) / (float)a.d;
  __syncthreads();
#pragma unroll
  for (int i = 0; i < TT; ++i) {
    float s = 0.f;
#pragma unroll
    for (int ci = 0; ci < MAXC; ++ci) {
      const int c = tid + ci * 256;
      if (c < a.d) { const float dlt = y[ci][i] - mean[i]; s += dlt * dlt; }
    }
    s = gam_wave_sum(s);
    if (lane == 0) red[wave * TT + i] = s;
  }
  __syncthreads();
#pragma unroll
  for (int i = 0; i < TT; ++i)
    rstd[i] = 1.0f / sqrtf((red[i] + red[TT + i] + red[2 * TT + i] + red[3 * TT + i]) / (float)a.d + a.eps);
#pragma unroll
  for (int ci = 0; ci < MAXC; ++ci) {
    const int c = tid + ci * 256;
    if (c < a.d) {
      const float g = a.n_scale[c], be = a.n_shift[c];
#pragma unroll
      for (int i = 0; i < TT; ++i) {
        const int t = t0 + i;
        if (t < rlim) {
          const float v = gam_silu((y[ci][i] - mean[i]) * rstd[i] * g + be);
          gam_range_note(a.range_flag, v, 0.f, 0.f, 0.f);
          gam_store1(a.z, (rowbase + t) * (size_t)a.d, c, v, a.z_split);
        }
      }
    }
  }
}

template <int KS>
__global__ __launch_bounds__(256) void gam_convmod_ln4_kernel(GamConvModArgs a) {
  constexpr int TT = 16, PAD = (KS - 1) / 2, ROWS = TT + KS - 1;
  __shared__ float red[4][TT];
  const int tid = threadIdx.x, lane = tid & 63, wave = tid >> 6;
  const int b = blockIdx.y, t0 = blockIdx.x * TT;
  const bool live = tid * 4 < a.d;
  const int c = live ? tid * 4 : 0;
  int klen = a.lens[b];
  klen = klen < a.Tv ? klen : a.Tv;
  const GamRows ur = gam_rows(a.cu, b, a.Ta, klen);
  if (t0 >= ur.lim) return;
  const size_t rowbase = ur.base;
  const int rlim = ur.lim;
  f32x4 ua[ROWS], ub[ROWS];
#pragma unroll
  for (int r = 0; r < ROWS; ++r) {
    const int t = t0 - PAD + r;
    const int tc = t < 0 ? 0 : (t < rlim ? t : rlim - 1);
    const float* up = a.u + (rowbase + tc) * (size_t)(2 * a.d);
    ua[r] = *reinterpret_cast<const f32x4*>(up + c);
    ub[r] = *reinterpret_cast<const f32x4*>(up + a.d + c);
  }
  f32x4 w[KS];
#pragma unroll
  for (int k = 0; k < KS; ++k)
    w[k] = (f32x4){a.dw_w[(size_t)c * KS + k], a.dw_w[(size_t)(c + 1) * KS + k], a.dw_w[(size_t)(c + 2) * KS + k],
                   a.dw_w[(size_t)(c + 3) * KS + k]};
  const f32x4 bias = *reinterpret_cast<const f32x4*>(a.dw_b + c);
#pragma unroll
  for (int r = 0; r < ROWS; ++r) {
    const int t = t0 - PAD + r;
    const bool live = t >= 0 && t < klen;
    const f32x4 glu = (f32x4){ua[r].x * gam_sigmoid(ub[r].x), ua[r].y * gam_sigmoid(ub[r].y), ua[r].z * gam_sigmoid(ub[r].z),
                              ua[r].w * gam_sigmoid(ub[r].w)};
    ua[r] = live ? glu : (f32x4){0.f, 0.f, 0.f, 0.f};
  }
  f32x4 y[TT];
#pragma unroll
  for (int i = 0; i < TT; ++i) {
    f32x4 acc = (f32x4){0.f, 0.f, 0.f, 0.f};
#pragma unroll
    for (int k = 0; k < KS; ++k) {
      acc.x = fmaf(w[k].x, ua[i + k].x, acc.x);
      acc.y = fmaf(w[k].y, ua[i + k].y, acc.y);
      acc.z = fmaf(w[k].z, ua[i + k].z, acc.z);
      acc.w = fmaf(w[k].w, ua[i + k].w, acc.w);
    }
    y[i] = acc + bias;
  }
  float mean[TT], rstd[TT];
#pragma unroll
  for (int i = 0; i < TT; ++i) {
    float s = live ? (y[i].x + y[i].y) + (y[i].z + y[i].w) : 0.f;
    s = gam_wave_sum(s);
    if (lane == 0) red[wave][i] = s;
  }
  __syncthreads();
#pragma unroll
  for (int i = 0; i < TT; ++i) mean[i] = (red[0][i] + red[1][i] + red[2][i] + red[3][i]) / (float)a.d;
  __syncthreads();
#pragma unroll
  for (int i = 0; i < TT; ++i) {
    const float d0 = y[i].x - mean[i], d1 = y[i].y - mean[i], d2 = y[i].z - mean[i], d3 = y[i].w - mean[i];
    float s = live ? (d0 * d0 + d1 * d1) + (d2 * d2 + d3 * d3) : 0.f;
    s = gam_wave_sum(s);
    if (lane == 0) red[wave][i] = s;
  }
  __syncthreads();
#pragma unroll
  for (int i = 0; i < TT; ++i) rstd[i] = 1.0f / sqrtf((red[0][i] + red[1][i] + red[2][i] + red[3][i]) / (float)a.d + a.eps);
  if (!live) return;
  const f32x4 gm = *reinterpret_cast<const f32x4*>(a.n_scale + c);
  const f32x4 be = *reinterpret_cast<const f32x4*>(a.n_shift + c);
#pragma unroll
  for (int i = 0; i < TT; ++i) {
    const int t = t0 + i;
    if (t < rlim) {
      const float v0 = gam_silu((y[i].x - mean[i]) * rstd[i] * gm.x + be.x), v1 = gam_silu((y[i].y - mean[i]) * rstd[i] * gm.y + be.y);
      const float v2 = gam_silu((y[i].z - mean[i]) * rstd[i] * gm.z + be.z), v3 = gam_silu((y[i].w - mean[i]) * rstd[i] * gm.w + be.w);
      gam_range_note(a.range_flag, v0, v1, v2, v3);
      gam_store4(a.z, (rowbase + t) * (size_t)a.d, c, v0, v1, v2, v3, a.z_split);
    }
  }
}

static inline hipError_t gam_launch_convmod(const GamConvModArgs& a, int layer_norm, hipStream_t s) {
  if (!layer_norm) {
    if (a.d % 64 != 0) return hipErrorInvalidValue;
    dim3 grid(gam_cdiv(a.Ta, 128), a.d / 64, a.B);
    if (a.ks == 31) hipLaunchKernelGGL(gam_convmod_bn_kernel<31>, grid, dim3(512), 0, s, a);
    else if (a.ks == 5) hipLaunchKernelGGL(gam_convmod_bn_kernel<5>, grid, dim3(512), 0, s, a);
    else if (a.ks == 9) hipLaunchKernelGGL(gam_convmod_bn_kernel<9>, grid, dim3(512), 0, s, a);
    else return hipErrorInvalidValue;
  } else {
    if (a.d > 1024) return hipErrorInvalidValue;
    dim3 grid(gam_cdiv(a.Ta, 8), a.B);
    if ((a.ks == 5 || a.ks == 9) && a.d % 4 == 0) {
      dim3 g4(gam_cdiv(a.Ta, 16), a.B);
      if (a.ks == 5) hipLaunchKernelGGL(gam_convmod_ln4_kernel<5>, g4, dim3(256), 0, s, a);
      else hipLaunchKernelGGL(gam_convmod_ln4_kernel<9>, g4, dim3(256), 0, s, a);
    } else if (a.ks == 5) {
      const size_t sm = ((8 + 4) * a.d + 32) * sizeof(float);
      hipLaunchKernelGGL(gam_convmod_ln_kernel<5>, grid, dim3(256), sm, s, a);
    } else if (a.ks == 31) {
      const size_t sm = ((8 + 30) * a.d + 32) * sizeof(float);
      static std::atomic<unsigned long long> attr_devs{0};
      if (hipError_t e = gam_set_max_lds(reinterpret_cast<const void*>(gam_convmod_ln_kernel<31>), 160 * 1024, attr_devs)) return e;
      hipLaunchKernelGGL(gam_convmod_ln_kernel<31>, grid, dim3(256), sm, s, a);
    } else if (a.ks == 9) {
      const size_t sm = ((8 + 8) * a.d + 32) * sizeof(float);
      if (sm > 64 * 1024) {
        static std::atomic<unsigned long long> attr_devs9{0};
        if (hipError_t e = gam_set_max_lds(reinterpret_cast<const void*>(gam_convmod_ln_kernel<9>), 160 * 1024, attr_devs9)) return e;
      }
      hipLaunchKernelGGL(gam_convmod_ln_kernel<9>, grid, dim3(256), sm, s, a);
    } else return hipErrorInvalidValue;
  }
  return hipGetLastError();
}
```

### gigaam_amd/csrc/gam_gemm.h

```cpp
#pragma once
#include "gam_common.h"
#include <stdlib.h>

struct GamGemmArgs {
  const float* A;
  const float* W;
  const float* bias;
  const float* R;
  float* C;
  int M, N, K;
  long lda, ldc, ldr;
  float alpha;
  int a_mode;
  int conv_fp;
  int conv_c;
  int conv_f2;
  const int* lens;
  int rpb, fdiv;
  int remap, out_rpb, out_shift, rows_valid;
  int skip_pad;
  const _Float16* Asp;
  const _Float16* Wsp;
  const _Float16* Asp2;
  int n_switch;
// ... 154 lines not shown
    *reinterpret_cast<float4*>(a_ + 32 * LD) = va1;                             \
    *reinterpret_cast<float4*>(a_ + 64 * LD) = va2;                             \
    *reinterpret_cast<float4*>(a_ + 96 * LD) = va3;                             \
    *reinterpret_cast<float4*>(b_) = vb0;                                       \
    *reinterpret_cast<float4*>(b_ + 32 * LD) = vb1;                             \
    *reinterpret_cast<float4*>(b_ + 64 * LD) = vb2;                             \
    *reinterpret_cast<float4*>(b_ + 96 * LD) = vb3;                             \
  }
#define GAM_MFMA(AV, BV, ACC) ACC = __builtin_amdgcn_mfma_f32_32x32x2f32(AV, BV, ACC, 0, 0, 0)

  const int frag = (lane & 31) * LD + (lane >> 5) * 4;
#define GAM_COMPUTE(AB, BB)                                                                     \
  _Pragma("unroll") for (int s = 0; s < 4; ++s) {                                               \
    const float4 a0 = *reinterpret_cast<const float4*>((AB) + s * 8);                           \
    const float4 a1 = *reinterpret_cast<const float4*>((AB) + 32 * LD + s * 8);                 \
    const float4 b0 = *reinterpret_cast<const float4*>((BB) + s * 8);                           \
    const float4 b1 = *reinterpret_cast<const float4*>((BB) + 32 * LD + s * 8);                 \
                         \
    GAM_MFMA(a0.x, b0.x, acc00); GAM_MFMA(a0.x, b1.x, acc01); GAM_MFMA(a1.x, b0.x, acc10); GAM_MFMA(a1.x, b1.x, acc11); \
    GAM_MFMA(a0.y, b0.y, acc00); GAM_MFMA(a0.y, b1.y, acc01); GAM_MFMA(a1.y, b0.y, acc10); GAM_MFMA(a1.y, b1.y, acc11); \
    GAM_MFMA(a0.z, b0.z, acc00); GAM_MFMA(a0.z, b1.z, acc01); GAM_MFMA(a1.z, b0.z, acc10); GAM_MFMA(a1.z, b1.z, acc11); \
    GAM_MFMA(a0.w, b0.w, acc00); GAM_MFMA(a0.w, b1.w, acc01); GAM_MFMA(a1.w, b0.w, acc10); GAM_MFMA(a1.w, b1.w, acc11); \
  }
  GAM_GLOAD(0);
  const float* Ab = As + wm * 64 * LD + frag;
  const float* Bb = Bs + wn * 64 * LD + frag;
  for (int kt = 0; kt < nk; ++kt) {
    __syncthreads();
    GAM_LSTORE();
    __syncthreads();
    if (kt + 1 < nk) GAM_GLOAD(kt + 1);
    GAM_COMPUTE(Ab, Bb);
  }
#undef GAM_COMPUTE
#undef GAM_GLOAD
#undef GAM_LSTORE
#undef GAM_MFMA

  gam_gemm_epilogue<ACT>(g, acc00, acc01, acc10, acc11, m0, n0, wm, wn, lane);
}

template <int ACT>
static inline void gam_launch_gemm_t(const GamGemmArgs& a, int grid, hipStream_t stream) {
  static std::atomic<unsigned long long> attr_devs{0};
  if (gam_set_max_lds(reinterpret_cast<const void*>(gam_gemm_f32_kernel<ACT>), GAM_GEMM_SMEM, attr_devs) != hipSuccess) return;
  hipLaunchKernelGGL((gam_gemm_f32_kernel<ACT>), dim3(grid, a.splitk > 1 ? a.splitk : 1), dim3(256), GAM_GEMM_SMEM, stream, a);
}

static inline hipError_t gam_launch_gemm(const GamGemmArgs& a_in, int act, hipStream_t stream) {
  GamGemmArgs a = a_in;
  if (a.ldw == 0) a.ldw = a.K;
  if (a.M <= 0 || a.N <= 0) return hipSuccess;
  if (a.K % GAM_GEMM_BK != 0 || a.K <= 0) return hipErrorInvalidValue;
  const int grid = gam_cdiv(a.M, GAM_GEMM_BM) * gam_cdiv(a.N, GAM_GEMM_BN);
  switch (act) {
    case GAM_ACT_SILU: gam_launch_gemm_t<GAM_ACT_SILU>(a, grid, stream); break;
    case GAM_ACT_RELU: gam_launch_gemm_t<GAM_ACT_RELU>(a, grid, stream); break;
    default: gam_launch_gemm_t<GAM_ACT_NONE>(a, grid, stream); break;
  }
  return hipGetLastError();
}

template <int ACT, int VEC, int SMAX = 16>
__global__ __launch_bounds__(256) void gam_splitk_reduce_kernel(GamGemmArgs g, int S) {
  const int cpr = (g.N + VEC - 1) / VEC;
  const size_t total = (size_t)g.M * cpr;
  const size_t slice = (size_t)g.M * (size_t)g.N;
  for (size_t i = (size_t)blockIdx.x * 256 + threadIdx.x; i < total; i += (size_t)gridDim.x * 256) {
    const int row = (int)(i / cpr), col = (int)(i % cpr) * VEC;
    float v[VEC];
#pragma unroll
    for (int e = 0; e < VEC; ++e) v[e] = 0.f;
    const float* p = g.partial + (size_t)row * g.N + col;
    if (VEC == 4) {
      const f32x4 t = gam_sum_slices<SMAX>(p, slice, S);
      v[0] = t.x; v[1 % VEC] = t.y; v[2 % VEC] = t.z; v[3 % VEC] = t.w;
    } else {
      for (int s = 0; s < S; ++s) v[0] += p[s * slice];
    }
    bool masked = false;
    long orow = row;
    if (g.lens != nullptr || g.remap) {
      const int bb = row / g.rpb, tt = row - bb * g.rpb;
      if (g.lens != nullptr) masked = (tt / g.fdiv) >= g.lens[bb];
      if (g.remap) {
        if (tt >= g.rows_valid) continue;
        orow = (long)bb * g.out_rpb + tt + g.out_shift;
      }
    }
#pragma unroll
    for (int e = 0; e < VEC; ++e) {
      float x = v[e];
      if (g.bias != nullptr) x += g.bias[col + e];
      if (ACT == GAM_ACT_SILU) x = gam_silu(x);
      if (ACT == GAM_ACT_RELU) x = fmaxf(x, 0.0f);
      if (masked) x = 0.0f;
      x *= g.alpha;
      if (g.R != nullptr) x += g.R[orow * g.ldr + col + e];
      v[e] = x;
    }
    if (VEC == 4) {
      if (g.c_guard) gam_range_note(g.range_flag, v[0], v[1 % VEC], v[2 % VEC], v[3 % VEC]);
      if (g.c_split) gam_store4(g.C, (size_t)orow * g.ldc, col, v[0], v[1 % VEC], v[2 % VEC], v[3 % VEC], g.c_split);
      else *reinterpret_cast<f32x4*>(g.C + orow * g.ldc + col) = (f32x4){v[0], v[1 % VEC], v[2 % VEC], v[3 % VEC]};
    } else {
      if (g.c_guard) gam_range_note(g.range_flag, v[0], 0.f, 0.f, 0.f);
      gam_store1(g.C, (size_t)orow * g.ldc, col, v[0], g.c_split);
    }
  }
}

static inline hipError_t gam_launch_splitk_reduce(const GamGemmArgs& a, int act, int S, hipStream_t stream) {
  auto al16 = [](const void* p) { return (reinterpret_cast<uintptr_t>(p) & 15) == 0; };
  const bool vec = a.N % 4 == 0 && a.ldc % 4 == 0 && al16(a.C) && al16(a.partial) &&
                   (a.R == nullptr || (a.ldr % 4 == 0 && al16(a.R)));
  const size_t total = (size_t)a.M * (vec ? a.N / 4 : a.N);
  const int grid = (int)((total + 255) / 256 < 2048 ? (total + 255) / 256 : 2048);
#define GAM_RED(ACTV)                                                                                      \
  if (vec && S <= 4) hipLaunchKernelGGL((gam_splitk_reduce_kernel<ACTV, 4, 4>), dim3(grid), dim3(256), 0, stream, a, S); \
  else if (vec) hipLaunchKernelGGL((gam_splitk_reduce_kernel<ACTV, 4, 16>), dim3(grid), dim3(256), 0, stream, a, S); \
  else hipLaunchKernelGGL((gam_splitk_reduce_kernel<ACTV, 1>), dim3(grid), dim3(256), 0, stream, a, S);
  switch (act) {
    case GAM_ACT_SILU: GAM_RED(GAM_ACT_SILU); break;
    case GAM_ACT_RELU: GAM_RED(GAM_ACT_RELU); break;
    default: GAM_RED(GAM_ACT_NONE); break;
  }
#undef GAM_RED
  return hipGetLastError();
}
```

### gigaam_amd/csrc/gam_gemm_sp.h

```cpp
#pragma once
#include "gam_gemm.h"
#include <type_traits>
#if defined(GAM_SP_INSTRUMENT) && GAM_SP_INSTRUMENT
#include <algorithm>
#include <vector>
#endif

#ifndef GAM_SP_INSTRUMENT
#define GAM_SP_INSTRUMENT 0
#endif
#if GAM_SP_INSTRUMENT
#define GAM_SP_TL(i)                                                                  \
  if (g.tlog != nullptr && threadIdx.x == 0) {                                        \
    g.tlog[(size_t)lid * 8 + (i)] = wall_clock64();                                   \
    if ((i) == 1 || (i) == 2) g.tlog[(size_t)lid * 8 + 4 + (i)] = clock64();          \
    if ((i) == 0) g.tlog[(size_t)lid * 8 + 7] = blockIdx.x;                            \
  }
#else
#define GAM_SP_TL(i)
#endif

template <int MT, int NW, int NS = 2>
struct GamGemmSpCfg {
  static constexpr int BM = 64 * MT;
// ... 265 lines not shown
      }
    }
    r_rsc[i] = accscale * ((ok && g.a_rs != nullptr) ? g.a_rs[row] : 1.0f);
    r_ok[i] = ok; r_masked[i] = masked; r_orow[i] = orow;
  }
  if (part) {
#pragma unroll
    for (int i = 0; i < 2 * MT; ++i) {
      if (!r_ok[i]) continue;
      float* P = g.partial + ((size_t)blockIdx.y * (size_t)g.M + (size_t)(mw + 16 * i + lrow)) * (size_t)g.N;
#pragma unroll
      for (int pp = 0; pp < 2; ++pp)
#pragma unroll
        for (int hf = 0; hf < 2; ++hf) {
          const int ecol = nw + 32 * pp + lq8 + 4 * hf;
          if (ecol < g.N) *reinterpret_cast<f32x4*>(P + ecol) = acc[i][2 * pp + hf] * r_rsc[i];
        }
    }
  }
#define GAM_SP_LDR(I, D)                                                                          \
  _Pragma("unroll") for (int pp = 0; pp < 2; ++pp) _Pragma("unroll") for (int hf = 0; hf < 2; ++hf) { \
    const int col = nw + 32 * pp + lq8 + 4 * hf;                                                  \
    D[pp][hf] = (r_ok[I] && col < g.N) ? *reinterpret_cast<const f32x4*>(g.R + r_orow[I] * g.ldr + col) : (f32x4){0.f, 0.f, 0.f, 0.f}; \
  }
  f32x4 rv[2][2], rn[2][2];
  const bool resid = g.R != nullptr && !part;
  if (resid) GAM_SP_LDR(0, rv);
#pragma unroll
  for (int i = 0; i < 2 * MT; ++i) {
    if (resid && i + 1 < 2 * MT) GAM_SP_LDR(i + 1, rn);
    const bool masked = r_masked[i];
    const long orow = r_orow[i];
    const float rsc = r_rsc[i];
    if (r_ok[i] && !part) {
#pragma unroll
      for (int pp = 0; pp < 2; ++pp) {
        const int ecol = nw + 32 * pp + lq8;
        if (ecol >= g.N) continue;
        const bool both = ecol + 4 < g.N;
        f32x4 v[2];
#pragma unroll
        for (int hf = 0; hf < 2; ++hf) {
          f32x4 t = acc[i][2 * pp + hf];
          t = t * rsc + bv[pp][hf];
          if (ACT == GAM_ACT_SILU) { t.x = gam_silu(t.x); t.y = gam_silu(t.y); t.z = gam_silu(t.z); t.w = gam_silu(t.w); }
          if (ACT == GAM_ACT_RELU) { t.x = fmaxf(t.x, 0.f); t.y = fmaxf(t.y, 0.f); t.z = fmaxf(t.z, 0.f); t.w = fmaxf(t.w, 0.f); }
          if (masked) t = (f32x4){0.f, 0.f, 0.f, 0.f};
          t = t * g.alpha;
          if (resid) t += rv[pp][hf];
          if (!both && hf == 1) t = (f32x4){0.f, 0.f, 0.f, 0.f};
          v[hf] = t;
        }
        if (g.c_guard) { gam_range_note(g.range_flag, v[0].x, v[0].y, v[0].z, v[0].w); gam_range_note(g.range_flag, v[1].x, v[1].y, v[1].z, v[1].w); }
        if (g.c_split == 2) {
          _Float16* cp = reinterpret_cast<_Float16*>(g.C) + orow * g.ldc + ecol;
          const gam_half4 h0 = __builtin_convertvector(v[0], gam_half4), h1 = __builtin_convertvector(v[1], gam_half4);
          if (both) *reinterpret_cast<gam_half8*>(cp) = (gam_half8){h0[0], h0[1], h0[2], h0[3], h1[0], h1[1], h1[2], h1[3]};
          else *reinterpret_cast<gam_half4*>(cp) = h0;
        } else if (g.c_split) {
          _Float16* cp = reinterpret_cast<_Float16*>(g.C) + orow * (2 * g.ldc) + (ecol >> 5) * 64 + (ecol & 31);
          gam_half4 hi0, lo0, hi1, lo1;
          gam_split4(v[0], hi0, lo0);
          gam_split4(v[1], hi1, lo1);
          if (both) {
            *reinterpret_cast<gam_half8*>(cp) = (gam_half8){hi0[0], hi0[1], hi0[2], hi0[3], hi1[0], hi1[1], hi1[2], hi1[3]};
            *reinterpret_cast<gam_half8*>(cp + 32) = (gam_half8){lo0[0], lo0[1], lo0[2], lo0[3], lo1[0], lo1[1], lo1[2], lo1[3]};
          } else {
            *reinterpret_cast<gam_half4*>(cp) = hi0;
            *reinterpret_cast<gam_half4*>(cp + 32) = lo0;
          }
        } else {
          *reinterpret_cast<f32x4*>(g.C + orow * g.ldc + ecol) = v[0];
          if (both) *reinterpret_cast<f32x4*>(g.C + orow * g.ldc + ecol + 4) = v[1];
        }
      }
    }
    if (resid && i + 1 < 2 * MT) {
#pragma unroll
      for (int pp = 0; pp < 2; ++pp)
#pragma unroll
        for (int hf = 0; hf < 2; ++hf) rv[pp][hf] = rn[pp][hf];
    }
  }
#undef GAM_SP_LDR
#if GAM_SP_INSTRUMENT
  if (g.tlog != nullptr) { __builtin_amdgcn_s_waitcnt(0x0070); __syncthreads(); }
  GAM_SP_TL(3);
#endif
}

static inline bool gam_gemm_sp_epilogue_ok(const GamGemmArgs& a) {
  auto al16 = [](const void* p) { return (reinterpret_cast<uintptr_t>(p) & 15) == 0; };
  return a.N % 4 == 0 && a.ldc % 4 == 0 && al16(a.C) && (a.bias == nullptr || al16(a.bias)) &&
         (a.R == nullptr || (a.ldr % 4 == 0 && al16(a.R)));
}

template <int ACT, int MT, int NW, int NS = 2, bool H16 = false>
static inline void gam_launch_gemm_sp_t(const GamGemmArgs& a, int grid, hipStream_t stream) {
  static std::atomic<unsigned long long> attr_devs{0};
  constexpr int smem = GamGemmSpCfg<MT, NW, NS>::SMEM;
  static_assert(smem <= 160 * 1024, "LDS stages do not fit a CU");
  auto kern = gam_gemm_sp_kernel<ACT, MT, NW, NS, H16>;
  if (gam_set_max_lds(reinterpret_cast<const void*>(kern), smem, attr_devs) != hipSuccess) return;
  hipLaunchKernelGGL(kern, dim3(grid, a.splitk > 1 ? a.splitk : 1), dim3(128 * NW), smem, stream, a);
}

struct GamSpPlan { int mt, nw, s, ns; };
// ... 23 lines not shown
    const bool shared = wgs > ncu;
    const double tk_u = 0.256 * t + 0.142, tf_u = S > 1 ? 4.9 : 14.1;
    t_kt = tk_u * (shared ? 1.82 : 1.0);
    t_fix = tf_u * (shared ? 0.73 : 1.0);
    rounds = (double)((wgs + (shared ? 2 : 1) * ncu - 1) / ((shared ? 2 : 1) * ncu));
    const long cap2 = 2L * ncu, rem = wgs % cap2;
    if (shared && wgs > cap2 && rem != 0 && rem <= ncu) {
      (void)a_mode;
      double us2 = (double)(wgs / cap2) * (nkt * t_kt + t_fix) + (nkt * tk_u + tf_u);
      if (S > 1) us2 += 7.1 + (double)(S + 2) * M * N * 4.0 / 3.87e6;
      return us2;
    }
  }
  (void)a_mode;
  double us = rounds * (nkt * t_kt + t_fix);
  if (S > 1) us += 7.1 + (double)(S + 2) * M * N * 4.0 / 3.87e6;
  return us;
}
static inline GamSpPlan gam_gemm_sp_plan(int M, int N, int K, int a_mode = 0, int ncu = 256) {
  GamSpForce& frc = gam_sp_force();
  const int f_mt = frc.mt.load(std::memory_order_relaxed), f_nw = frc.nw.load(std::memory_order_relaxed);
  int f_s = frc.s.load(std::memory_order_relaxed), f_ns = frc.ns.load(std::memory_order_relaxed);
  GamSpPlan best = {3, 4, 1, 2};
  double bt = 1e30;
  const int nk = K / 32;
  if (f_s > 1 && (f_s > 8 || nk % f_s != 0 || nk / f_s < 4)) f_s = 1;
  if (f_ns == 3 && a_mode != 0) f_ns = 2;
  for (int w = 4; w >= 2; w -= 2) {
    if ((f_nw == 2 || f_nw == 4) && w != f_nw) continue;
    for (int t = (w == 2 ? 3 : 4); t >= 2; --t) {
      if (f_mt >= 2 && f_mt <= 4 && t != f_mt && !(w == 2 && f_mt == 4)) continue;
      for (int S = 1; S <= 8; ++S) {
        if (f_s >= 1 && S != f_s) continue;
        if (S > 1 && (nk % S != 0 || nk / S < 4)) continue;
        if (f_s < 1 && S > 1 && (long)gam_cdiv(M, 64 * t) * gam_cdiv(N, 64 * w) * 2 > ncu) continue;
        for (int ns = 2; ns <= 3; ++ns) {
          if (ns == 3 && (!gam_sp_has_ns3(t, w) || a_mode != 0)) continue;
          if ((f_ns == 2 || f_ns == 3) && ns != f_ns && !(f_ns == 3 && !gam_sp_has_ns3(t, w))) continue;
          const double us = gam_gemm_sp_model(M, N, K, a_mode, t, w, S, ncu, ns);
          if (us < bt - 1e-9) { bt = us; best = {t, w, S, ns}; }
        }
      }
    }
  }
  return best;
}

static inline hipError_t gam_launch_gemm_sp(const GamGemmArgs& a_in, int act, hipStream_t stream) {
  GamGemmArgs a = a_in;
  if (a.M <= 0 || a.N <= 0) return hipSuccess;
  if (a.K <= 0 || a.K % 32 != 0 || a.Asp == nullptr || a.Wsp == nullptr) return hipErrorInvalidValue;
  if (a.a_mode == 0 ? (a.lda % 32 != 0) : (a.conv_c % 32 != 0)) return hipErrorInvalidValue;
  if (!gam_gemm_sp_epilogue_ok(a)) return hipErrorInvalidValue;
  int mt = a.sp_mt, nw = a.sp_nw, ns = a.sp_ns;
  if (mt < 2 || mt > 4 || (nw != 2 && nw != 4) || (nw == 2 && mt == 4)) {
    const GamSpPlan p = gam_gemm_sp_plan(a.M, a.N, a.K, a.a_mode);
    mt = p.mt; nw = p.nw; ns = p.ns;
    if (a.splitk > 1 && a.partial == nullptr) return hipErrorInvalidValue;
  }
  if (ns != 3 || !gam_sp_has_ns3(mt, nw)) ns = 2;
  if (a.splitk > 1 && (a.partial == nullptr || (a.K / 32) % a.splitk != 0)) return hipErrorInvalidValue;
  if (a.n_switch > 0 && (a.Asp2 == nullptr || a.a_mode != 0 || a.n_switch % (64 * nw) != 0)) return hipErrorInvalidValue;
  if (a.splitk <= 1) { a.splitk = 0; a.partial = nullptr; }
  const int grid = gam_cdiv(a.M, 64 * mt) * gam_cdiv(a.N, 64 * nw);
  a.ntiles = grid;
#if GAM_SP_INSTRUMENT
  static long long* tl_dev = nullptr;
  static int tl_cap = 0;
  static const bool tl_on = getenv("GAM_SP_TLOG") != nullptr;
  a.tlog = nullptr;
  if (tl_on) {
    if (grid > tl_cap) { if (tl_dev) (void)hipFree(tl_dev); (void)hipMalloc(&tl_dev, (size_t)grid * 64); tl_cap = grid; }
    (void)hipMemsetAsync(tl_dev, 0, (size_t)grid * 64, stream);
    a.tlog = tl_dev;
  }
#endif
#define GAM_LSP(ACTV)                                                            \
  if (a.h16) {           \
    if (ns == 3) {                                                               \
      if (nw == 4) gam_launch_gemm_sp_t<ACTV, 2, 4, 3, true>(a, grid, stream);   \
      else if (mt == 2) gam_launch_gemm_sp_t<ACTV, 2, 2, 3, true>(a, grid, stream); \
      else gam_launch_gemm_sp_t<ACTV, 3, 2, 3, true>(a, grid, stream);           \
    } else if (nw == 2) {                                                        \
      if (mt == 2) gam_launch_gemm_sp_t<ACTV, 2, 2, 2, true>(a, grid, stream);   \
      else gam_launch_gemm_sp_t<ACTV, 3, 2, 2, true>(a, grid, stream);           \
    } else switch (mt) {                                                         \
      case 2: gam_launch_gemm_sp_t<ACTV, 2, 4, 2, true>(a, grid, stream); break; \
      case 3: gam_launch_gemm_sp_t<ACTV, 3, 4, 2, true>(a, grid, stream); break; \
      default: gam_launch_gemm_sp_t<ACTV, 4, 4, 2, true>(a, grid, stream); break; \
    }                                                                            \
  } else if (ns == 3) {                                                          \
    if (nw == 4) gam_launch_gemm_sp_t<ACTV, 2, 4, 3>(a, grid, stream);           \
    else if (mt == 2) gam_launch_gemm_sp_t<ACTV, 2, 2, 3>(a, grid, stream);      \
    else gam_launch_gemm_sp_t<ACTV, 3, 2, 3>(a, grid, stream);                   \
  } else if (nw == 2) switch (mt) {                                              \
    case 2: gam_launch_gemm_sp_t<ACTV, 2, 2>(a, grid, stream); break;            \
    default: gam_launch_gemm_sp_t<ACTV, 3, 2>(a, grid, stream); break;           \
  } else switch (mt) {                                                           \
    case 2: gam_launch_gemm_sp_t<ACTV, 2, 4>(a, grid, stream); break;            \
    case 3: gam_launch_gemm_sp_t<ACTV, 3, 4>(a, grid, stream); break;            \
    default: gam_launch_gemm_sp_t<ACTV, 4, 4>(a, grid, stream); break;           \
  }
  switch (act) {
    case GAM_ACT_SILU: GAM_LSP(GAM_ACT_SILU); break;
    case GAM_ACT_RELU: GAM_LSP(GAM_ACT_RELU); break;
    default: GAM_LSP(GAM_ACT_NONE); break;
  }
#undef GAM_LSP
#if GAM_SP_INSTRUMENT
  if (tl_on) {
    std::vector<long long> t((size_t)grid * 8);
    (void)hipStreamSynchronize(stream);
    (void)hipMemcpy(t.data(), tl_dev, t.size() * 8, hipMemcpyDeviceToHost);
    long long t_first = t[0], t_last = 0;
    for (int i = 0; i < grid; ++i) { t_first = std::min(t_first, t[i * 8]); t_last = std::max(t_last, t[i * 8 + 3]); }
    auto stat = [&](auto f, const char* name) {
      std::vector<double> v(grid);
      for (int i = 0; i < grid; ++i) v[i] = f(i);
      std::sort(v.begin(), v.end());
      fprintf(stderr, "    %-26s min %7.2f  p50 %7.2f  p90 %7.2f  max %7.2f us\n", name, v[0], v[grid / 2], v[(size_t)(grid * 0.9)], v[grid - 1]);
    };
    fprintf(stderr, "[tlog] M=%d N=%d K=%d MT=%d NW=%d tiles=%d: first entry -> last exit %.2f us\n", a.M, a.N, a.K, mt, nw, grid, (t_last - t_first) * 0.01);
    stat([&](int i) { return (t[i * 8] - t_first) * 0.01; }, "entry after first entry");
    stat([&](int i) { return (t[i * 8 + 1] - t[i * 8]) * 0.01; }, "prologue (2 k-tiles land)");
    stat([&](int i) { return (t[i * 8 + 2] - t[i * 8 + 1]) * 0.01; }, "main loop");
    stat([&](int i) { return (t[i * 8 + 2] - t[i * 8 + 1]) * 0.01 / (a.K / 32); }, "  per k-tile");
    stat([&](int i) { return (double)(t[i * 8 + 6] - t[i * 8 + 5]) / std::max<long long>(1, t[i * 8 + 2] - t[i * 8 + 1]) * 100.0; }, "  shader MHz in loop");
    stat([&](int i) { return (t[i * 8 + 3] - t[i * 8 + 2]) * 0.01; }, "epilogue");
    stat([&](int i) { return (t_last - t[i * 8 + 3]) * 0.01; }, "idle after exit");
    double x_loop[8] = {0}; int x_n[8] = {0};
    for (int i = 0; i < grid; ++i) { const int x = (int)(t[i * 8 + 7] & 7); x_loop[x] += (t[i * 8 + 2] - t[i * 8 + 1]) * 0.01; ++x_n[x]; }
    fprintf(stderr, "    mean loop us by XCD:");
    for (int x = 0; x < 8; ++x) fprintf(stderr, " %.1f", x_n[x] ? x_loop[x] / x_n[x] : 0.0);
    fprintf(stderr, "\n");
  }
#endif
  return hipGetLastError();
}

__global__ __launch_bounds__(256) void gam_to_sp32_kernel(const float* __restrict__ x, _Float16* __restrict__ y,
                                                          size_t n4, const float* __restrict__ rs, int K) {
  const size_t stride = (size_t)gridDim.x * 256;
  for (size_t i = (size_t)blockIdx.x * 256 + threadIdx.x; i < n4; i += stride) {
    f32x4 v = reinterpret_cast<const f32x4*>(x)[i];
    const size_t e = i * 4;
    if (rs != nullptr) v = v * (1.0f / rs[e / (size_t)K]);
    gam_half4 h, l;
    gam_split4(v, h, l);
    _Float16* p = y + (e >> 5) * 64 + (e & 31);
    *reinterpret_cast<gam_half4*>(p) = h;
    *reinterpret_cast<gam_half4*>(p + 32) = l;
  }
}

__global__ __launch_bounds__(256) void gam_to_h16_kernel(const float* __restrict__ x, _Float16* __restrict__ y, size_t n4,
                                                         const float* __restrict__ rs, int K) {
  const size_t stride = (size_t)gridDim.x * 256;
  for (size_t i = (size_t)blockIdx.x * 256 + threadIdx.x; i < n4; i += stride) {
    f32x4 v = reinterpret_cast<const f32x4*>(x)[i];
    if (rs != nullptr) v = v * (1.0f / rs[(i * 4) / (size_t)K]);
    reinterpret_cast<gam_half4*>(y)[i] = __builtin_convertvector(v, gam_half4);
  }
}

__global__ __launch_bounds__(256) void gam_rowscale_kernel(const float* __restrict__ x, float* __restrict__ rs, int rows,
                                                           int K, long lda) {
  const int row = blockIdx.x * 4 + (threadIdx.x >> 6), lane = threadIdx.x & 63;
  if (row >= rows) return;
  const float* xr = x + (size_t)row * lda;
  float m = 0.f;
  for (int k = lane; k < K; k += 64) m = fmaxf(m, fabsf(xr[k]));
  m = gam_wave_max(m);
  float s_, inv_;
  gam_row_scale(m, s_, inv_);
  if (lane == 0) rs[row] = inv_;
}
```

### gigaam_amd/engine.py

```python
from __future__ import annotations

import contextlib
import ctypes as C
import functools
import math
import os
import threading
from typing import Any, Callable, Dict, List, Mapping, Optional, Sequence, Tuple

import numpy as np
import torch
from torch import Tensor

from . import _lib
from ._lib import GamConfig, GigaAMHipError


def _get(cfg: Any, key: str, default: Any = None) -> Any:
    if cfg is None:
        return default
    if isinstance(cfg, Mapping):
        return cfg.get(key, default)
    return getattr(cfg, key, default)

# ... 1202 lines not shown
                dump = dcount = None
                if dump_cap > 0:
                    dump = torch.zeros((b, dump_cap, self.cfg.num_classes), dtype=torch.float32, device=self.device)
                    dcount = torch.zeros((b,), dtype=torch.int32, device=self.device)
                rc = self.lib.gam_rnnt_greedy(self._h, _ptr(encoded), _ptr(enc_len), b, tp, max_symbols, _ptr(ids),
                                              _ptr(frames), _ptr(counts), _ptr(dump), _ptr(dcount), dump_cap, self._stream())
                self._check(rc, "gam_rnnt_greedy")
                if overlap:
                    st = torch.cuda.current_stream(self.device)
                    evt = torch.cuda.Event()
                    evt.record(st)
                    for t in (encoded, enc_len, whole):
                        t.record_stream(st)
                else:
                    evt, st = self._fetch_flag(word)
        finally:
            if overlap:
                self._check(self.lib.gam_set_rnnt_cluster(self._h, self._rnnt_cluster_user), "gam_set_rnnt_cluster")
        return Decoded(ids, frames, counts, out.ext, evt, st, dump, dcount, whole=whole)

    def rnnt_predict(self, labels: Optional[Tensor], state: Optional[Tuple[Tensor, Tensor]], batch_size: int = 1):
        ph, nl = self.cfg.pred_hidden, self.cfg.pred_rnn_layers
        if labels is not None:
            labels = self._dev(labels.reshape(-1), torch.int32)
            b = labels.shape[0]
        else:
            b = batch_size if state is None else state[0].shape[1]
        h_in = c_in = None
        if state is not None:
            h_in, c_in = self._dev(state[0], torch.float32), self._dev(state[1], torch.float32)
            if tuple(h_in.shape) != (nl, b, ph) or tuple(c_in.shape) != (nl, b, ph):
                raise GigaAMHipError(f"predictor state must be two [{nl},{b},{ph}] tensors, got {tuple(h_in.shape)} / {tuple(c_in.shape)}")
        g = torch.empty((b, ph), dtype=torch.float32, device=self.device)
        h_out = torch.empty((nl, b, ph), dtype=torch.float32, device=self.device)
        c_out = torch.empty_like(h_out)
        with torch.cuda.device(self.device):
            rc = self.lib.gam_rnnt_predict(self._h, _ptr(labels), _ptr(h_in), _ptr(c_in), b, _ptr(g), _ptr(h_out), _ptr(c_out), self._stream())
        self._check(rc, "gam_rnnt_predict")
        return g, (h_out, c_out)

    def rnnt_joint(self, enc: Tensor, dec: Tensor) -> Tensor:
        enc, dec = self._dev(enc, torch.float32), self._dev(dec, torch.float32)
        b, t, d = enc.shape
        b2, u, ph = dec.shape
        if b != b2 or d != self.cfg.d_model or ph != self.cfg.pred_hidden:
            raise GigaAMHipError(f"joint expects [B,T,{self.cfg.d_model}] and [B,U,{self.cfg.pred_hidden}], got {tuple(enc.shape)} / {tuple(dec.shape)}")
        out = torch.empty((b, t, u, self.cfg.num_classes), dtype=torch.float32, device=self.device)
        with torch.cuda.device(self.device):
            rc = self.lib.gam_rnnt_joint(self._h, _ptr(enc), _ptr(dec), b, t, u, _ptr(out), self._stream())
        self._check(rc, "gam_rnnt_joint")
        return out

    def op_gemm(self, a: Tensor, w: Tensor, bias: Optional[Tensor] = None, act: int = 0, resid: Optional[Tensor] = None,
                alpha: float = 1.0) -> Tensor:
        a = self._dev(a, torch.float32)
        w = self._dev(w, torch.float32)
        bias = None if bias is None else self._dev(bias, torch.float32)
        resid = None if resid is None else self._dev(resid, torch.float32)
        m, k = a.shape
        n = w.shape[0]
        out = torch.empty((m, n), dtype=torch.float32, device=self.device)
        with torch.cuda.device(self.device):
            rc = self.lib.gam_op_gemm_ex(self._h, _ptr(a), _ptr(w), _ptr(bias), _ptr(resid), alpha, _ptr(out), m, n, k, act,
                                         self._stream())
        self._check(rc, "gam_op_gemm_ex")
        return out

    def op_attention(self, q: Tensor, k: Tensor, v: Tensor, lens: Optional[Tensor] = None) -> Tensor:
        q, k, v = (self._dev(t, torch.float32) for t in (q, k, v))
        b, t, d = q.shape
        lens_d = None if lens is None else self._dev(lens, torch.int32)
        out = torch.empty_like(q)
        with torch.cuda.device(self.device):
            rc = self.lib.gam_op_attention(self._h, _ptr(q), _ptr(k), _ptr(v), _ptr(out), _ptr(lens_d), b, t, d // 48, self._stream())
        self._check(rc, "gam_op_attention")
        return out

    def op_attention_ex(self, q: Tensor, k: Tensor, v: Tensor, B: int, Ta: int, Tv: int, H: int, lens: Optional[Tensor] = None,
                        cu: Optional[Tensor] = None, pbuf: Optional[Tensor] = None, pos_u: Optional[Tensor] = None,
                        pos_v: Optional[Tensor] = None) -> Tensor:
        ldq = q.stride(0)
        if not (q.is_cuda and k.is_cuda and v.is_cuda) or k.stride(0) != ldq or v.stride(0) != ldq or any(t.stride(1) != 1 for t in (q, k, v)):
            raise GigaAMHipError("op_attention_ex: q, k, v must be CUDA row views with one row stride")
        lens_d, cu_d = (None if t is None else self._dev(t, torch.int32) for t in (lens, cu))
        pbuf, pos_u, pos_v = (None if t is None else self._dev(t, torch.float32) for t in (pbuf, pos_u, pos_v))
        out = torch.full((q.shape[0], H * 48), float("nan"), dtype=torch.float32, device=self.device)
        with torch.cuda.device(self.device):
            rc = self.lib.gam_op_attention_ex(self._h, _ptr(q), _ptr(k), _ptr(v), ldq, _ptr(out), _ptr(lens_d), _ptr(cu_d), B, Ta, Tv, H,
                                              _ptr(pbuf), _ptr(pos_u), _ptr(pos_v), self._stream())
        self._check(rc, "gam_op_attention_ex")
        return out

    def _op_ptr(self, what: str, name: str, t: Optional[Tensor], dtype: torch.dtype = torch.float32) -> Optional[int]:
        if t is None:
            return None
        if not (t.is_cuda and t.device == self.device and t.dtype == dtype and t.is_contiguous()):
            raise GigaAMHipError(f"{what}: {name} must be a contiguous {dtype} tensor on {self.device}")
        return t.data_ptr()

    def op_layernorm(self, mode: int, rows: int, d: int, x: Optional[Tensor], out1: Tensor, w1: Tensor, b1: Tensor, *,
                     out2: Optional[Tensor] = None, w2: Optional[Tensor] = None, b2: Optional[Tensor] = None, split1: int = 0,
                     split2: int = 0, rs: Optional[Tensor] = None, rcos: Optional[Tensor] = None, rsin: Optional[Tensor] = None,
                     dk: int = 0, ta: int = 0, rope_rows: Optional[int] = None, row_t: Optional[Tensor] = None,
                     part: Optional[Tensor] = None, nsplit: int = 0, pbias: Optional[Tensor] = None, presid: Optional[Tensor] = None,
                     palpha: float = 1.0, xstore: Optional[Tensor] = None, eps: float = 1e-5) -> None:
        what = "op_layernorm"
        op = _lib.GamLnOp()
        for name, t in (("x", x), ("out1", out1), ("out2", out2), ("w1", w1), ("b1", b1), ("w2", w2), ("b2", b2), ("rcos", rcos),
                        ("rsin", rsin), ("rs", rs), ("part", part), ("pbias", pbias), ("presid", presid), ("xstore", xstore)):
            setattr(op, name, self._op_ptr(what, name, t))
        op.row_t = self._op_ptr(what, "row_t", row_t, torch.int32)
        op.mode, op.rows, op.d, op.split1, op.split2, op.dk, op.ta, op.nsplit = mode, rows, d, split1, split2, dk, ta, nsplit
        op.rope_rows = (0 if rcos is None else rcos.shape[0]) if rope_rows is None else rope_rows
        op.eps, op.palpha = eps, palpha
        with torch.cuda.device(self.device):
            rc = self.lib.gam_op_layernorm(self._h, C.byref(op), self._stream())
        self._check(rc, "gam_op_layernorm")

    def op_convmod(self, u: Tensor, z: Tensor, dw_w: Tensor, dw_b: Tensor, n_scale: Tensor, n_shift: Tensor, lens: Tensor, B: int,
                   Ta: int, Tv: int, d: int, ks: int, layer_norm: bool, z_split: int = 0, cu: Optional[Tensor] = None) -> None:
        what = "op_convmod"
        ptrs = [self._op_ptr(what, n, t) for n, t in (("u", u), ("z", z), ("dw_w", dw_w), ("dw_b", dw_b), ("n_scale", n_scale),
                                                      ("n_shift", n_shift))]
        ptrs += [self._op_ptr(what, "lens", lens, torch.int32), self._op_ptr(what, "cu", cu, torch.int32)]
        with torch.cuda.device(self.device):
            rc = self.lib.gam_op_convmod(self._h, *ptrs, B, Ta, Tv, d, ks, int(bool(layer_norm)), z_split, self._stream())
        self._check(rc, "gam_op_convmod")

    def profile_enable(self, on=True) -> None:
        self._check(self.lib.gam_profile_enable(self._h, int(on)), "gam_profile_enable")

    def profile_level(self, on) -> None:
        self._check(self.lib.gam_profile_pause(self._h, int(on)), "gam_profile_pause")

    def profile_read(self) -> Dict[str, Dict[str, float]]:
        out = {}
        for i, name in enumerate(_lib.PF_CLASSES):
            ms, n, work = C.c_double(), C.c_int64(), C.c_double()
            self._check(self.lib.gam_profile_read(self._h, i, C.byref(ms), C.byref(n), C.byref(work)), "gam_profile_read")
            nbytes = C.c_double()
            self._check(self.lib.gam_profile_read_bytes(self._h, i, C.byref(nbytes)), "gam_profile_read_bytes")
            out[name] = {"ms": ms.value, "launches": int(n.value), "work": work.value, "bytes": nbytes.value}
        return out
```

### include/gigaam_hip.h

```cpp
#ifndef GIGAAM_HIP_H
#define GIGAAM_HIP_H

#include <stdint.h>

#ifdef __cplusplus
extern "C" {
#endif

#define GAM_ABI_VERSION 1

typedef struct gam_handle gam_handle;

enum { GAM_SUBS_CONV2D = 0, GAM_SUBS_CONV1D = 1 };
enum { GAM_ATT_ROTARY = 0, GAM_ATT_REL_POS = 1 };
enum { GAM_NORM_BATCH = 0, GAM_NORM_LAYER = 1 };
enum { GAM_HEAD_NONE = 0, GAM_HEAD_CTC = 1, GAM_HEAD_RNNT = 2, GAM_HEAD_EMO = 3 };
enum { GAM_DTYPE_F32 = 0, GAM_DTYPE_F16 = 1, GAM_DTYPE_BF16 = 2, GAM_DTYPE_F64 = 3, GAM_DTYPE_I64 = 4 };

typedef struct gam_config {
  int32_t sample_rate, n_mels, hop_length, win_length, n_fft, center;
  int32_t feat_in, n_layers, d_model, subsampling, subs_kernel_size, subsampling_factor;
  int32_t ff_expansion_factor, self_attention_model, n_heads, pos_emb_max_len;
  int32_t conv_norm_type, conv_kernel_size;
  int32_t head_type, num_classes, pred_hidden, pred_rnn_layers, joint_hidden;
// ... 100 lines not shown
int gam_op_rnnt_beam(gam_handle* h, const float* encp, const int32_t* enc_len, int B, int64_t Tp, int W, int max_symbols, int32_t* ids,
                     int32_t* frames, int32_t* counts, float* score, float* logp, void* stream);

int gam_rnnt_beam_nbest(gam_handle* h, const float* encoded, const int32_t* enc_len, int B, int64_t Tp, int W, int max_symbols, int N,
                        int32_t* ids, int32_t* frames, int32_t* counts, float* score, float* logp, int32_t* n_hyp, void* stream);
int gam_op_rnnt_beam_nbest(gam_handle* h, const float* encp, const int32_t* enc_len, int B, int64_t Tp, int W, int max_symbols, int N,
                           int32_t* ids, int32_t* frames, int32_t* counts, float* score, float* logp, int32_t* n_hyp, void* stream);

int gam_rnnt_align(gam_handle* h, const float* encoded, const int32_t* enc_len, int B, int64_t Tp, const int32_t* targets,
                   const int32_t* target_len, int Umax, int32_t* tok_frame, float* score, float* loglik, int32_t* status, void* stream);
int gam_op_rnnt_align(gam_handle* h, const float* encp, const int32_t* enc_len, int B, int64_t Tp, const int32_t* targets,
                      const int32_t* target_len, int Umax, int32_t* tok_frame, float* score, float* loglik, int32_t* status,
                      float* lattice_out, void* stream);
int gam_op_rnnt_lattice_align(gam_handle* h, const float* lattice, const int32_t* enc_len, int B, int64_t Tp, int V, const int32_t* targets,
                              const int32_t* target_len, int Umax, int32_t* tok_frame, float* score, float* loglik, int32_t* status,
                              void* stream);
int gam_set_rnnt_align_workspace(gam_handle* h, int64_t bytes);

int gam_ctc_confidence(gam_handle* h, const float* encoded, const int32_t* enc_len, int B, int64_t Tp, const int32_t* ids,
                       const int32_t* frames, const int32_t* counts, int cap, int measure, int agg, float* conf, int32_t* span,
                       int32_t* status, void* stream);
int gam_op_ctc_confidence(gam_handle* h, const float* log_probs, const int32_t* enc_len, int B, int64_t Tp, int V, const int32_t* ids,
                          const int32_t* frames, const int32_t* counts, int cap, int measure, int agg, float* conf, int32_t* span,
                          int32_t* status, void* stream);
int gam_rnnt_confidence(gam_handle* h, const float* encoded, const int32_t* enc_len, int B, int64_t Tp, const int32_t* ids,
                        const int32_t* frames, const int32_t* counts, int cap, int measure, float* conf, int32_t* status, void* stream);
int gam_op_rnnt_confidence(gam_handle* h, const float* encp, const int32_t* enc_len, int B, int64_t Tp, const int32_t* ids,
                           const int32_t* frames, const int32_t* counts, int cap, int measure, float* conf, int32_t* status, void* stream);

int gam_set_rnnt_cluster(gam_handle* h, int workgroups_per_utterance);
int gam_get_rnnt_cluster(gam_handle* h);
int gam_rnnt_cluster_plan_info(int ncu, int cluster, int exclusive, int B, int H, int JH, int V, int L, int32_t* out);
int gam_rnnt_last_decode(gam_handle* h, int32_t* out);

int gam_debug_buffer_hash(gam_handle* h, int which, uint64_t* hash_out, int64_t* floats_out);

int gam_rnnt_predict(gam_handle* h, const int32_t* labels, const float* h_in, const float* c_in, int B, float* g_out,
                     float* h_out, float* c_out, void* stream);
int gam_rnnt_joint(gam_handle* h, const float* enc, const float* dec, int B, int T, int U, float* log_probs, void* stream);

int gam_emo_probs(gam_handle* h, const float* encoded, const int32_t* enc_len, int B, int64_t Tp, float* probs,
                  void* stream);

enum { GAM_GEMM_F32 = 0, GAM_GEMM_F16X3 = 1, GAM_GEMM_F16 = 2 };
int gam_set_gemm_mode(gam_handle* h, int mode);
int gam_range_flag(gam_handle* h, int* flag_host, void* stream);
int gam_range_flag_fetch(gam_handle* h, int32_t* flag_dev, void* stream);
int gam_get_gemm_mode(const gam_handle* h);

int gam_op_gemm(gam_handle* h, const float* A, const float* W, const float* bias, float* C,
                int M, int N, int K, int act, void* stream);
int gam_op_gemm_ex(gam_handle* h, const float* A, const float* W, const float* bias, const float* R, float alpha,
                   float* C, int M, int N, int K, int act, void* stream);

int gam_op_attention(gam_handle* h, const float* q, const float* k, const float* v, float* ctx,
                     const int32_t* lens, int B, int T, int H, void* stream);
int gam_op_attention_ex(gam_handle* h, const float* q, const float* k, const float* v, int64_t ldq, float* ctx,
                        const int32_t* lens, const int32_t* cu, int B, int Ta, int Tv, int H, const float* pbuf,
                        const float* pos_u, const float* pos_v, void* stream);

typedef struct gam_ln_op {
  const float* x;
  float* out1;
  float* out2;
  const float* w1;
  const float* b1;
  const float* w2;
  const float* b2;
  const float* rcos;
  const float* rsin;
  const int32_t* row_t;
  float* rs;
  const float* part;
  const float* pbias;
  const float* presid;
  float* xstore;
  int32_t mode, rows, d, split1, split2, dk, ta, rope_rows, nsplit;
  float eps, palpha;
} gam_ln_op;
int gam_op_layernorm(gam_handle* h, const gam_ln_op* op, void* stream);

int gam_op_convmod(gam_handle* h, const float* u, float* z, const float* dw_w, const float* dw_b, const float* n_scale,
                   const float* n_shift, const int32_t* lens, const int32_t* cu, int B, int Ta, int Tv, int d, int ks,
                   int layer_norm, int z_split, void* stream);

int gam_tune_sp(int mt, int nw, int splitk);
int gam_plan_sp(int M, int N, int K, int n_cu, int* mt, int* nw, int* splitk);
int gam_plan_sp_ex(int M, int N, int K, int n_cu, int* mt, int* nw, int* splitk, int* stages);
int gam_tune_sp_stages(int stages);

enum { GAM_RS_FMT_U8 = 0, GAM_RS_FMT_I16 = 1, GAM_RS_FMT_I24 = 2, GAM_RS_FMT_I32 = 3, GAM_RS_FMT_F32 = 4, GAM_RS_FMT_MULAW = 5,
       GAM_RS_FMT_ALAW = 6 };
int gam_resample_plan(int rate_in, int rate_out, int* up, int* down, int* taps);
int gam_resample_tile(int rate_in, int rate_out, int* tile, int* form);
int gam_resample_table(int rate_in, int rate_out, float* coeff, int32_t* first);
int64_t gam_resample_out_len(int rate_in, int rate_out, int64_t n_in);
int gam_op_resample(const void* src, int fmt, int channels, int channel, const int64_t* len_in, int B, int64_t frames, int rate_in,
                    int rate_out, const float* coeff, const int32_t* first, float* dst, int64_t L_out, int64_t* len_out, void* stream);

enum { GAM_PF_GEMM = 0, GAM_PF_CONV2 = 1, GAM_PF_ATTN = 2, GAM_PF_NORM = 3, GAM_PF_CONVMOD = 4,
       GAM_PF_STEM = 5, GAM_PF_FRONTEND = 6, GAM_PF_DECODE = 7, GAM_PF_MISC = 8,
       GAM_PF_ALIGN_BT = 9, GAM_PF_ALIGN_OUT = 10,
       GAM_PF_NCLASS = 11 };
int gam_profile_enable(gam_handle* h, int on);
int gam_profile_read(gam_handle* h, int cls, double* ms, int64_t* launches, double* work);
int gam_profile_pause(gam_handle* h, int on);
int gam_profile_read_bytes(gam_handle* h, int cls, double* bytes);

typedef struct gam_comm gam_comm;
#define GAM_COMM_ID_BYTES 128
int gam_comm_unique_id(char id_out[GAM_COMM_ID_BYTES]);
int gam_comm_create(const char id[GAM_COMM_ID_BYTES], int rank, int world, int device_id, gam_comm** out);
int gam_comm_world(const gam_comm* c);
int gam_gather_ids(gam_comm* c, const int32_t* index, const int32_t* counts, const int32_t* ids, const int32_t* frames,
                   int rows, int cap, int32_t* all_index, int32_t* all_counts, int32_t* all_ids, int32_t* all_frames,
                   void* stream);
const char* gam_comm_last_error(const gam_comm* c);
void gam_comm_destroy(gam_comm* c);

const char* gam_last_error(const gam_handle* h);

#ifdef __cplusplus
}
#endif
#endif
```

Before: 21010.

## Fuse GLU gate into pointwise_conv1 split-fp16 GEMM epilogue with interleaved weights

Result: no change. 21150, median of 6 (+0.7%).

```diff
diff --git a/gigaam_amd/_lib.py b/gigaam_amd/_lib.py
--- a/gigaam_amd/_lib.py
+++ b/gigaam_amd/_lib.py
@@ -106,10 +106,15 @@
     "gam_range_flag_fetch": (C.c_int, [_P, _P, _P]),
     "gam_op_gemm": (C.c_int, [_P, _P, _P, _P, _P, C.c_int, C.c_int, C.c_int, C.c_int, _P]),
     "gam_op_gemm_ex": (C.c_int, [_P, _P, _P, _P, _P, C.c_float, _P, C.c_int, C.c_int, C.c_int, C.c_int, _P]),
+    "gam_op_gemm_fmt": (C.c_int, [_P, _P, _P, _P, _P, C.c_float, _P, C.c_int, C.c_int, C.c_int, C.c_int, C.c_int, _P]),
+    "gam_op_glu": (C.c_int, [_P, _P, _P, C.c_int64, C.c_int, _P]),
+    "gam_glu_column": (C.c_int, [C.c_int, C.c_int]),
+    "gam_glu_interleave": (C.c_int, [_P, _P, C.c_int, C.c_int, _P, _P]),
     "gam_op_attention": (C.c_int, [_P, _P, _P, _P, _P, _P, C.c_int, C.c_int, C.c_int, _P]),
     "gam_op_attention_ex": (C.c_int, [_P, _P, _P, _P, C.c_int64, _P, _P, _P, C.c_int, C.c_int, C.c_int, C.c_int, _P, _P, _P, _P]),
     "gam_op_layernorm": (C.c_int, [_P, C.POINTER(GamLnOp), _P]),
     "gam_op_convmod": (C.c_int, [_P, _P, _P, _P, _P, _P, _P, _P, _P, C.c_int, C.c_int, C.c_int, C.c_int, C.c_int, C.c_int, C.c_int, _P]),
+    "gam_op_convmod_gated": (C.c_int, [_P, _P, _P, _P, _P, _P, _P, _P, _P, C.c_int, C.c_int, C.c_int, C.c_int, C.c_int, C.c_int, C.c_int, _P]),
     "gam_tune_sp": (C.c_int, [C.c_int, C.c_int, C.c_int]),
     "gam_plan_sp": (C.c_int, [C.c_int, C.c_int, C.c_int, C.c_int, C.POINTER(C.c_int), C.POINTER(C.c_int), C.POINTER(C.c_int)]),
     "gam_plan_sp_ex": (C.c_int, [C.c_int, C.c_int, C.c_int, C.c_int, C.POINTER(C.c_int), C.POINTER(C.c_int), C.POINTER(C.c_int), C.POINTER(C.c_int)]),
diff --git a/gigaam_amd/csrc/gam_api.hip b/gigaam_amd/csrc/gam_api.hip
--- a/gigaam_amd/csrc/gam_api.hip
+++ b/gigaam_amd/csrc/gam_api.hip
@@ -78,6 +78,7 @@
   float *ln_att_w, *ln_att_b, *wqkv, *bqkv, *wo, *bo;
   float *wpos, *pos_u, *pos_v;
   float *ln_conv_w, *ln_conv_b, *pw1_w, *pw1_b, *dw_w, *dw_b, *cn_scale, *cn_shift, *pw2_w, *pw2_b;
+  float* pw1_bg;
   float *ln_ff2_w, *ln_ff2_b, *ff2_w1, *ff2_b1, *ff2_w2, *ff2_b2;
   float *ln_out_w, *ln_out_b;
   W16 s_ff1_w1, s_ff1_w2, s_wqkv, s_wo, s_wpos, s_pw1, s_pw2, s_ff2_w1, s_ff2_w2;
@@ -136,6 +137,7 @@
 
   DevBuf wavp, spec, img, c2, xin, y1, x, y, yr, hbuf, qkv, ctx, ubuf, zbuf, tok, logits, encp, pbuf, aplanes;
   DevBuf op_planes, op_sp, splitk_ws;
+  DevBuf op_glu;
   DevBuf align_star;
   DevBuf align_bp;
   DevBuf align_long_ws;
@@ -163,6 +165,7 @@
   int use_pack = 1;
   int use_splitk = 1;
   int fuse_reduce = 1;
+  int glu_epilogue = 1;
   int use_graph = 1;
   int graph_max_rows = 2048;
   uint64_t ws_generation = 0;
@@ -373,7 +376,7 @@
   if (ps.ev) {
     const double abytes = a.a_mode == 0 ? ((double)(a.M - 1) * (double)std::min<long>(a.lda, a.K) + a.K) * 4.0
                                         : (double)a.M / a.conv_f2 * 2.0 * a.conv_fp * a.conv_c * 4.0;
-    h->prof_bytes[cls] += abytes * (a.n_switch > 0 ? 2.0 : 1.0) + 4.0 * a.N * a.K + 4.0 * a.M * a.N * (a.R ? 2.0 : 1.0);
+    h->prof_bytes[cls] += abytes * (a.n_switch > 0 ? 2.0 : 1.0) + 4.0 * a.N * a.K + 4.0 * a.M * a.N * (a.R ? 2.0 : act == GAM_ACT_GLU ? 0.5 : 1.0);
   }
   hipError_t e;
   if (a.Asp != nullptr) {
@@ -513,6 +516,7 @@
   if (const char* e = getenv("GAM_SPLITK")) h->use_splitk = atoi(e);
   if (const char* e = getenv("GAM_PACK")) h->use_pack = atoi(e);
   if (const char* e = getenv("GAM_FUSE_REDUCE")) h->fuse_reduce = atoi(e);
+  if (const char* e = getenv("GAM_GLU_EPILOGUE")) h->glu_epilogue = atoi(e) != 0;
   if (const char* e = getenv("GAM_GRAPH")) h->use_graph = atoi(e);
   if (const char* e = getenv("GAM_GRAPH_MAX_ROWS")) h->graph_max_rows = atoi(e);
   if (const char* e = getenv("GAM_RNNT_CLUSTER")) h->rnnt_cluster = std::max(-1, std::min(8, atoi(e)));
@@ -767,6 +771,20 @@
   return upload_to(h, DST(L.cn_shift), sh);
 }
 
+static void glu_interleave(const std::vector<float>& w, const std::vector<float>& b, int d, int K, std::vector<float>& wg, std::vector<float>& bg) {
+  wg.resize((size_t)2 * d * K);
+  bg.resize(b.empty() ? 0 : (size_t)2 * d);
+  for (int j = 0; j < 2 * d; ++j) {
+    const int src = gam_glu_col(j, d);
+    std::copy(w.begin() + (size_t)src * K, w.begin() + (size_t)(src + 1) * K, wg.begin() + (size_t)j * K);
+    if (!b.empty()) bg[j] = b[src];
+  }
+}
+
+static inline bool glu_epilogue_model(const gam_handle* h) {
+  return h->glu_epilogue && h->cfg.d_model % 32 == 0 && (h->cfg.d_model * h->cfg.ff_expansion_factor) % 32 == 0;
+}
+
 static int fin_layer(gam_handle* h, int li, LayerW& L) {
   const gam_config& c = h->cfg;
   const int D = c.d_model, DFF = D * c.ff_expansion_factor;
@@ -789,7 +807,15 @@
     if (int r = upload_to(h, DST(L.pos_v), pv->data)) return r;
   }
   if (int r = upload_ln(h, p + "norm_conv", D, DST(L.ln_conv_w), DST(L.ln_conv_b))) return r;
-  if (int r = upload_linear(h, p + "conv.pointwise_conv1", 2 * D, D, DST(L.pw1_w), DST(L.pw1_b), &L.s_pw1)) return r;
+  if (glu_epilogue_model(h)) {
+    if (int r = upload_linear(h, p + "conv.pointwise_conv1", 2 * D, D, DST(L.pw1_w), DST(L.pw1_b), nullptr)) return r;
+    std::vector<float> wg, bg;
+    glu_interleave(find(h, p + "conv.pointwise_conv1.weight")->data, find(h, p + "conv.pointwise_conv1.bias")->data, D, D, wg, bg);
+    if (int r = up_split(h, wg, &L.s_pw1, D)) return r;
+    if (int r = upload_to(h, DST(L.pw1_bg), bg)) return r;
+  } else if (int r = upload_linear(h, p + "conv.pointwise_conv1", 2 * D, D, DST(L.pw1_w), DST(L.pw1_b), &L.s_pw1)) {
+    return r;
+  }
   if (int r = upload_linear(h, p + "conv.depthwise_conv", D, c.conv_kernel_size, DST(L.dw_w), DST(L.dw_b), nullptr)) return r;
   if (int r = fin_conv_norm(h, p, L)) return r;
   if (int r = upload_linear(h, p + "conv.pointwise_conv2", D, D, DST(L.pw2_w), DST(L.pw2_b), &L.s_pw2)) return r;
@@ -1001,6 +1027,7 @@
   bool conv2d, rel, packed;
   bool sp;
   int spf;
+  bool glu;
   bool sp_stem;
   bool graph;
 };
@@ -1050,6 +1077,7 @@
   const bool f16_fmt_ok = p.D % 64 == 0 && p.DFF % 64 == 0;
   p.spf = p.sp ? (h->gemm_mode == GAM_GEMM_F16 && f16_fmt_ok ? 2 : 1) : 0;
   p.sp_stem = p.sp && p.F % 32 == 0;
+  p.glu = p.sp && glu_epilogue_model(h);
   p.graph = h->use_graph && !h->prof_on && p.nl > 0 && p.N < h->graph_max_rows && !p.packed;
   return 0;
 }
@@ -1065,7 +1093,7 @@
   if (int r = ensure(h, h->hbuf, N * p.DFF)) return r;
   if (int r = ensure(h, h->qkv, N * 3 * D)) return r;
   if (int r = ensure(h, h->ctx, N * D)) return r;
-  if (int r = ensure(h, h->ubuf, N * 2 * D)) return r;
+  if (int r = ensure(h, h->ubuf, N * (p.glu ? D : 2 * D))) return r;
   if (int r = ensure(h, h->zbuf, N * D)) return r;
   if (int r = ensure(h, h->rsbuf, N + 64)) return r;
   if (p.packed)
@@ -1195,13 +1223,13 @@
 
 static hipError_t launch_convmod(gam_handle* h, hipStream_t s, const float* u, float* z, const float* dw_w, const float* dw_b, const float* n_scale,
                                  const float* n_shift, const int* lens, const int* cu, int B, int Ta, int Tv, int d, int ks, bool layer_norm,
-                                 int z_split) {
+                                 int z_split, bool gated = false) {
   GamConvModArgs cm;
   memset(&cm, 0, sizeof cm);
   cm.u = u; cm.z = z; cm.dw_w = dw_w; cm.dw_b = dw_b; cm.n_scale = n_scale; cm.n_shift = n_shift;
   cm.lens = lens; cm.cu = cu; cm.B = B; cm.Ta = Ta; cm.Tv = Tv; cm.d = d; cm.ks = ks; cm.eps = 1e-5f;
   cm.z_split = z_split; cm.range_flag = h->use_range ? h->range_flag : nullptr;
-  return gam_launch_convmod(cm, layer_norm, s);
+  return gam_launch_convmod(cm, layer_norm, s, gated);
 }
 
 static int norm_to_y(gam_handle* h, hipStream_t s, const EncCtx& c, const float* w, const float* b, PendingReduce* pend) {
@@ -1271,13 +1299,13 @@
   const EncPlan& p = c.p;
   const int D = p.D, NR = p.NR, ks = h->cfg.conv_kernel_size;
   if (int r = norm_to_y(h, s, c, L.ln_conv_w, L.ln_conv_b, pend)) return r;
-  GamGemmArgs g1 = gemm_args(h->y.p, D, L.pw1_w, L.pw1_b, h->ubuf.p, 2 * D, NR, 2 * D, D);
+  GamGemmArgs g1 = gemm_args(h->y.p, D, L.pw1_w, p.glu ? L.pw1_bg : L.pw1_b, h->ubuf.p, p.glu ? D : 2 * D, NR, 2 * D, D);
   gemm_formats(g1, p.spf, c.w.rs, 0, 0);
-  if (int r = gemm(h, s, g1, GAM_ACT_NONE, GAM_PF_GEMM, &L.s_pw1)) return r;
+  if (int r = gemm(h, s, g1, p.glu ? GAM_ACT_GLU : GAM_ACT_NONE, GAM_PF_GEMM, &L.s_pw1)) return r;
   {
-    ProfScope ps(h, s, GAM_PF_CONVMOD, (double)NR * D * 3 * 4.0);
+    ProfScope ps(h, s, GAM_PF_CONVMOD, (double)NR * D * (p.glu ? 2 : 3) * 4.0);
     hipError_t e = launch_convmod(h, s, h->ubuf.p, h->zbuf.p, L.dw_w, L.dw_b, L.cn_scale, L.cn_shift, c.w.len2, c.w.cu, p.B,
-                                  p.packed ? p.Tmax : p.Ta, p.Tv, D, ks, h->cfg.conv_norm_type == GAM_NORM_LAYER, p.spf);
+                                  p.packed ? p.Tmax : p.Ta, p.Tv, D, ks, h->cfg.conv_norm_type == GAM_NORM_LAYER, p.spf, p.glu);
     if (e != hipSuccess) return fail(h, -2, "conv-module launch (k=%d): %s", ks, hipGetErrorString(e));
   }
   GamGemmArgs g2 = gemm_args(h->zbuf.p, D, L.pw2_w, L.pw2_b, h->x.p, D, NR, D, D);
@@ -2634,14 +2662,38 @@
 
 int gam_op_gemm_ex(gam_handle* h, const float* A, const float* W, const float* bias, const float* R, float alpha, float* C, int M,
                    int N, int K, int act, void* stream) {
+  return gam_op_gemm_fmt(h, A, W, bias, R, alpha, C, M, N, K, act, 0, stream);
+}
+
+int gam_op_gemm_fmt(gam_handle* h, const float* A, const float* W, const float* bias, const float* R, float alpha, float* C, int M,
+                    int N, int K, int act, int c_split, void* stream) {
   if (!h) return -1;
+  if (act < GAM_ACT_NONE || act > GAM_ACT_GLU) return fail(h, -1, "gemm: activation %d outside 0..3", act);
+  if (c_split < 0 || c_split > 2) return fail(h, -1, "gemm: store format %d outside 0..2", c_split);
   HIPCHK(h, hipSetDevice(h->device));
-  GamGemmArgs g = gemm_args(A, K, W, bias, C, N, M, N, K);
-  g.R = R; g.ldr = N; g.alpha = alpha;
+  const bool glu = act == GAM_ACT_GLU;
+  GamGemmArgs g = gemm_args(A, K, W, bias, C, glu ? N / 2 : N, M, N, K);
+  g.R = R; g.ldr = N; g.alpha = alpha; g.c_split = c_split;
   hipStream_t s = (hipStream_t)stream;
+  const bool sp_shape = split_mode(h) && K > 0 && K % 32 == 0 && N % 4 == 0;
+  if (c_split && (!sp_shape || N % 32 != 0)) return fail(h, -1, "gemm: a split-fp16 C needs a split-fp16 mode, K %% 32 == 0 and N %% 32 == 0");
+  if (glu) {
+    if (!sp_shape) return fail(h, -1, "gemm: act 3 (GLU) exists in the split-fp16 kernel's epilogue only (mode %d, K %d, N %d)", h->gemm_mode, K, N);
+    if (!gam_glu_ok(g)) return fail(h, -1, "gemm: act 3 (GLU) needs N %% 8 == 0, an fp32 C and no residual (N %d, format %d, R %s)", N, c_split, R ? "given" : "null");
+  }
   if (!split_mode(h) || K % 32 != 0 || N % 4 != 0) return gemm(h, s, g, act);
   const size_t wn = (size_t)N * K, an = (size_t)M * K;
   W16 w16;
+  if (glu) {
+    if (int r = ensure(h, h->op_glu, wn + (size_t)N + 64)) return r;
+    float* wg = h->op_glu.p;
+    float* bg = wg + wn;
+    hipLaunchKernelGGL(gam_glu_rows_kernel, dim3((int)std::min<size_t>((wn / 4 + 255) / 256, 4096)), dim3(256), 0, s, W, wg, N / 2, K);
+    if (bias != nullptr) hipLaunchKernelGGL(gam_glu_rows_kernel, dim3(1), dim3(256), 0, s, bias, bg, N / 2, 1);
+    W = wg;
+    g.W = wg;
+    if (bias != nullptr) g.bias = bg;
+  }
   if (int r = ensure(h, h->op_sp, wn + 64)) return r;
   hipLaunchKernelGGL(gam_to_sp32_kernel, dim3((int)std::min<size_t>((wn / 4 + 255) / 256, 4096)), dim3(256), 0, s, W,
                      (_Float16*)h->op_sp.p, wn / 4, (const float*)nullptr, K);
@@ -2727,9 +2779,9 @@
   return 0;
 }
 
-int gam_op_convmod(gam_handle* h, const float* u, float* z, const float* dw_w, const float* dw_b, const float* n_scale,
-                   const float* n_shift, const int32_t* lens, const int32_t* cu, int B, int Ta, int Tv, int d, int ks, int layer_norm,
-                   int z_split, void* stream) {
+static int op_convmod_impl(gam_handle* h, const float* u, float* z, const float* dw_w, const float* dw_b, const float* n_scale,
+                           const float* n_shift, const int32_t* lens, const int32_t* cu, int B, int Ta, int Tv, int d, int ks, int layer_norm,
+                           int z_split, bool gated, void* stream) {
   if (!h) return -1;
   if (!h->finalized) return fail(h, -1, "gam_op_convmod before gam_finalize");
   if (!u || !z || !dw_w || !dw_b || !n_scale || !n_shift || !lens) return fail(h, -1, "conv module: null operand");
@@ -2741,10 +2793,47 @@
   if (d % 4 == 0 && (!al16(u) || !al16(z) || !al16(dw_b) || !al16(n_scale) || !al16(n_shift)))
     return fail(h, -1, "conv module: operands must be 16-byte aligned");
   HIPCHK(h, hipSetDevice(h->device));
-  hipError_t e = launch_convmod(h, (hipStream_t)stream, u, z, dw_w, dw_b, n_scale, n_shift, lens, cu, B, Ta, Tv, d, ks, layer_norm != 0, z_split);
+  hipError_t e = launch_convmod(h, (hipStream_t)stream, u, z, dw_w, dw_b, n_scale, n_shift, lens, cu, B, Ta, Tv, d, ks, layer_norm != 0, z_split, gated);
   if (e != hipSuccess) return fail(h, -2, "conv-module launch (k=%d, d=%d, %s): %s", ks, d, layer_norm ? "LayerNorm" : "BatchNorm", hipGetErrorString(e));
   return 0;
 }
+
+int gam_op_convmod(gam_handle* h, const float* u, float* z, const float* dw_w, const float* dw_b, const float* n_scale,
+                   const float* n_shift, const int32_t* lens, const int32_t* cu, int B, int Ta, int Tv, int d, int ks, int layer_norm,
+                   int z_split, void* stream) {
+  return op_convmod_impl(h, u, z, dw_w, dw_b, n_scale, n_shift, lens, cu, B, Ta, Tv, d, ks, layer_norm, z_split, false, stream);
+}
+
+int gam_op_convmod_gated(gam_handle* h, const float* u, float* z, const float* dw_w, const float* dw_b, const float* n_scale,
+                         const float* n_shift, const int32_t* lens, const int32_t* cu, int B, int Ta, int Tv, int d, int ks, int layer_norm,
+                         int z_split, void* stream) {
+  return op_convmod_impl(h, u, z, dw_w, dw_b, n_scale, n_shift, lens, cu, B, Ta, Tv, d, ks, layer_norm, z_split, true, stream);
+}
+
+int gam_op_glu(gam_handle* h, const float* u, float* y, int64_t rows, int d, void* stream) {
+  if (!h) return -1;
+  if (!u || !y || rows <= 0 || d <= 0) return fail(h, -1, "glu: bad arguments (rows %lld, d %d)", (long long)rows, d);
+  const bool vec = d % 4 == 0;
+  if (vec && ((reinterpret_cast<uintptr_t>(u) | reinterpret_cast<uintptr_t>(y)) & 15) != 0) return fail(h, -1, "glu: operands must be 16-byte aligned");
+  HIPCHK(h, hipSetDevice(h->device));
+  const size_t total = (size_t)rows * (vec ? d / 4 : d);
+  const dim3 grid((int)std::min<size_t>((total + 255) / 256, 4096));
+  if (vec) hipLaunchKernelGGL(gam_glu_kernel<4>, grid, dim3(256), 0, (hipStream_t)stream, u, y, (size_t)rows, d);
+  else hipLaunchKernelGGL(gam_glu_kernel<1>, grid, dim3(256), 0, (hipStream_t)stream, u, y, (size_t)rows, d);
+  HIPCHK(h, hipGetLastError());
+  return 0;
+}
+
+int gam_glu_interleave(const float* w, const float* b, int d, int K, float* w_out, float* b_out) {
+  if (!w || !w_out || d <= 0 || d % 4 != 0 || K <= 0 || (b != nullptr) != (b_out != nullptr)) return -1;
+  std::vector<float> wg, bg;
+  glu_interleave(std::vector<float>(w, w + (size_t)2 * d * K), b ? std::vector<float>(b, b + 2 * d) : std::vector<float>(), d, K, wg, bg);
+  std::copy(wg.begin(), wg.end(), w_out);
+  if (b) std::copy(bg.begin(), bg.end(), b_out);
+  return 0;
+}
+
+int gam_glu_column(int j, int d) { return (j < 0 || d <= 0 || d % 4 != 0 || j >= 2 * d) ? -1 : gam_glu_col(j, d); }
 
 int gam_set_gemm_mode(gam_handle* h, int mode) {
   if (!h || (mode != GAM_GEMM_F32 && mode != GAM_GEMM_F16X3 && mode != GAM_GEMM_F16)) return fail(h, -1, "unknown GEMM mode %d", mode);
diff --git a/gigaam_amd/csrc/gam_common.h b/gigaam_amd/csrc/gam_common.h
--- a/gigaam_amd/csrc/gam_common.h
+++ b/gigaam_amd/csrc/gam_common.h
@@ -203,4 +203,8 @@
   return acc;
 }
 
-enum { GAM_ACT_NONE = 0, GAM_ACT_SILU = 1, GAM_ACT_RELU = 2 };
+enum { GAM_ACT_NONE = 0, GAM_ACT_SILU = 1, GAM_ACT_RELU = 2, GAM_ACT_GLU = 3 };
+static inline __host__ __device__ int gam_glu_col(int j, int d) {
+  const int g = j >> 3, e = j & 7;
+  return e < 4 ? 4 * g + e : d + 4 * g + (e - 4);
+}
diff --git a/gigaam_amd/csrc/gam_convmod.h b/gigaam_amd/csrc/gam_convmod.h
--- a/gigaam_amd/csrc/gam_convmod.h
+++ b/gigaam_amd/csrc/gam_convmod.h
@@ -18,7 +18,7 @@
   int* range_flag;
 };
 
-template <int KS>
+template <int KS, bool GATED = false>
 __global__ __launch_bounds__(512, 4) void gam_convmod_bn_kernel(GamConvModArgs a) {
   constexpr int NRG = 32, TT = 128, PAD = (KS - 1) / 2, ROWS = (TT + KS - 1 + NRG - 1) / NRG * NRG, OUT = TT / NRG;
   __shared__ f32x4 tile[ROWS * 16];
@@ -38,9 +38,9 @@
   for (int u = 0; u < NLD; ++u) {
     const int t = t0 - PAD + rg + NRG * u;
     const int tc = t < 0 ? 0 : (t < rlim ? t : rlim - 1);
-    const float* up = a.u + (rowbase + tc) * (size_t)(2 * a.d);
+    const float* up = a.u + (rowbase + tc) * (size_t)(GATED ? a.d : 2 * a.d);
     ua[u] = *reinterpret_cast<const f32x4*>(up + c);
-    ub[u] = *reinterpret_cast<const f32x4*>(up + a.d + c);
+    if (!GATED) ub[u] = *reinterpret_cast<const f32x4*>(up + a.d + c);
   }
   {
 #pragma unroll
@@ -55,8 +55,9 @@
     const int rr = rg + NRG * u;
     const int t = t0 - PAD + rr;
     const bool live = t >= 0 && t < klen;
-    const f32x4 glu = (f32x4){ua[u].x * gam_sigmoid(ub[u].x), ua[u].y * gam_sigmoid(ub[u].y),
-                              ua[u].z * gam_sigmoid(ub[u].z), ua[u].w * gam_sigmoid(ub[u].w)};
+    const f32x4 glu = GATED ? ua[u]
+                            : (f32x4){ua[u].x * gam_sigmoid(ub[u].x), ua[u].y * gam_sigmoid(ub[u].y),
+                                      ua[u].z * gam_sigmoid(ub[u].z), ua[u].w * gam_sigmoid(ub[u].w)};
     tile[rr * 16 + q] = live ? glu : (f32x4){0.f, 0.f, 0.f, 0.f};
   }
   __syncthreads();
@@ -103,7 +104,7 @@
   }
 }
 
-template <int KS>
+template <int KS, bool GATED = false>
 __global__ __launch_bounds__(256) void gam_convmod_ln_kernel(GamConvModArgs a) {
   constexpr int TT = 8, PAD = (KS - 1) / 2, ROWS = TT + KS - 1, MAXC = 4;
   extern __shared__ __attribute__((aligned(16))) float gam_smem_cm[];
@@ -123,12 +124,12 @@
     for (int q = 0; q < 4; ++q) {
       const int t = t0 - PAD + r0 + q;
       const int tc = t < 0 ? 0 : (t < rlim ? t : rlim - 1);
-      const float* up = a.u + (rowbase + tc) * (size_t)(2 * a.d);
+      const float* up = a.u + (rowbase + tc) * (size_t)(GATED ? a.d : 2 * a.d);
 #pragma unroll
       for (int ci = 0; ci < MAXC; ++ci) {
         const int c = tid + ci * 256 < a.d ? tid + ci * 256 : a.d - 1;
         ua[q][ci] = up[c];
-        ub[q][ci] = up[a.d + c];
+        if (!GATED) ub[q][ci] = up[a.d + c];
       }
     }
 #pragma unroll
@@ -138,7 +139,7 @@
 #pragma unroll
       for (int ci = 0; ci < MAXC; ++ci) {
         const int c = tid + ci * 256;
-        if (rr < ROWS && c < a.d) tile[rr * a.d + c] = ok ? ua[q][ci] * gam_sigmoid(ub[q][ci]) : 0.f;
+        if (rr < ROWS && c < a.d) tile[rr * a.d + c] = ok ? (GATED ? ua[q][ci] : ua[q][ci] * gam_sigmoid(ub[q][ci])) : 0.f;
       }
     }
   }
@@ -210,7 +211,7 @@
   }
 }
 
-template <int KS>
+template <int KS, bool GATED = false>
 __global__ __launch_bounds__(256) void gam_convmod_ln4_kernel(GamConvModArgs a) {
   constexpr int TT = 16, PAD = (KS - 1) / 2, ROWS = TT + KS - 1;
   __shared__ float red[4][TT];
@@ -229,9 +230,9 @@
   for (int r = 0; r < ROWS; ++r) {
     const int t = t0 - PAD + r;
     const int tc = t < 0 ? 0 : (t < rlim ? t : rlim - 1);
-    const float* up = a.u + (rowbase + tc) * (size_t)(2 * a.d);
+    const float* up = a.u + (rowbase + tc) * (size_t)(GATED ? a.d : 2 * a.d);
     ua[r] = *reinterpret_cast<const f32x4*>(up + c);
-    ub[r] = *reinterpret_cast<const f32x4*>(up + a.d + c);
+    if (!GATED) ub[r] = *reinterpret_cast<const f32x4*>(up + a.d + c);
   }
   f32x4 w[KS];
 #pragma unroll
@@ -243,8 +244,9 @@
   for (int r = 0; r < ROWS; ++r) {
     const int t = t0 - PAD + r;
     const bool live = t >= 0 && t < klen;
-    const f32x4 glu = (f32x4){ua[r].x * gam_sigmoid(ub[r].x), ua[r].y * gam_sigmoid(ub[r].y), ua[r].z * gam_sigmoid(ub[r].z),
-                              ua[r].w * gam_sigmoid(ub[r].w)};
+    const f32x4 glu = GATED ? ua[r]
+                            : (f32x4){ua[r].x * gam_sigmoid(ub[r].x), ua[r].y * gam_sigmoid(ub[r].y), ua[r].z * gam_sigmoid(ub[r].z),
+                                      ua[r].w * gam_sigmoid(ub[r].w)};
     ua[r] = live ? glu : (f32x4){0.f, 0.f, 0.f, 0.f};
   }
   f32x4 y[TT];
@@ -296,37 +298,64 @@
   }
 }
 
-static inline hipError_t gam_launch_convmod(const GamConvModArgs& a, int layer_norm, hipStream_t s) {
+template <bool GATED>
+static inline hipError_t gam_launch_convmod_t(const GamConvModArgs& a, int layer_norm, hipStream_t s) {
   if (!layer_norm) {
     if (a.d % 64 != 0) return hipErrorInvalidValue;
     dim3 grid(gam_cdiv(a.Ta, 128), a.d / 64, a.B);
-    if (a.ks == 31) hipLaunchKernelGGL(gam_convmod_bn_kernel<31>, grid, dim3(512), 0, s, a);
-    else if (a.ks == 5) hipLaunchKernelGGL(gam_convmod_bn_kernel<5>, grid, dim3(512), 0, s, a);
-    else if (a.ks == 9) hipLaunchKernelGGL(gam_convmod_bn_kernel<9>, grid, dim3(512), 0, s, a);
+    if (a.ks == 31) hipLaunchKernelGGL((gam_convmod_bn_kernel<31, GATED>), grid, dim3(512), 0, s, a);
+    else if (a.ks == 5) hipLaunchKernelGGL((gam_convmod_bn_kernel<5, GATED>), grid, dim3(512), 0, s, a);
+    else if (a.ks == 9) hipLaunchKernelGGL((gam_convmod_bn_kernel<9, GATED>), grid, dim3(512), 0, s, a);
     else return hipErrorInvalidValue;
   } else {
     if (a.d > 1024) return hipErrorInvalidValue;
     dim3 grid(gam_cdiv(a.Ta, 8), a.B);
     if ((a.ks == 5 || a.ks == 9) && a.d % 4 == 0) {
       dim3 g4(gam_cdiv(a.Ta, 16), a.B);
-      if (a.ks == 5) hipLaunchKernelGGL(gam_convmod_ln4_kernel<5>, g4, dim3(256), 0, s, a);
-      else hipLaunchKernelGGL(gam_convmod_ln4_kernel<9>, g4, dim3(256), 0, s, a);
+      if (a.ks == 5) hipLaunchKernelGGL((gam_convmod_ln4_kernel<5, GATED>), g4, dim3(256), 0, s, a);
+      else hipLaunchKernelGGL((gam_convmod_ln4_kernel<9, GATED>), g4, dim3(256), 0, s, a);
     } else if (a.ks == 5) {
       const size_t sm = ((8 + 4) * a.d + 32) * sizeof(float);
-      hipLaunchKernelGGL(gam_convmod_ln_kernel<5>, grid, dim3(256), sm, s, a);
+      hipLaunchKernelGGL((gam_convmod_ln_kernel<5, GATED>), grid, dim3(256), sm, s, a);
     } else if (a.ks == 31) {
       const size_t sm = ((8 + 30) * a.d + 32) * sizeof(float);
       static std::atomic<unsigned long long> attr_devs{0};
-      if (hipError_t e = gam_set_max_lds(reinterpret_cast<const void*>(gam_convmod_ln_kernel<31>), 160 * 1024, attr_devs)) return e;
-      hipLaunchKernelGGL(gam_convmod_ln_kernel<31>, grid, dim3(256), sm, s, a);
+      if (hipError_t e = gam_set_max_lds(reinterpret_cast<const void*>(gam_convmod_ln_kernel<31, GATED>), 160 * 1024, attr_devs)) return e;
+      hipLaunchKernelGGL((gam_convmod_ln_kernel<31, GATED>), grid, dim3(256), sm, s, a);
     } else if (a.ks == 9) {
       const size_t sm = ((8 + 8) * a.d + 32) * sizeof(float);
       if (sm > 64 * 1024) {
         static std::atomic<unsigned long long> attr_devs9{0};
-        if (hipError_t e = gam_set_max_lds(reinterpret_cast<const void*>(gam_convmod_ln_kernel<9>), 160 * 1024, attr_devs9)) return e;
-      }
-      hipLaunchKernelGGL(gam_convmod_ln_kernel<9>, grid, dim3(256), sm, s, a);
+        if (hipError_t e = gam_set_max_lds(reinterpret_cast<const void*>(gam_convmod_ln_kernel<9, GATED>), 160 * 1024, attr_devs9)) return e;
+      }
+      hipLaunchKernelGGL((gam_convmod_ln_kernel<9, GATED>), grid, dim3(256), sm, s, a);
     } else return hipErrorInvalidValue;
   }
   return hipGetLastError();
 }
+
+static inline hipError_t gam_launch_convmod(const GamConvModArgs& a, int layer_norm, hipStream_t s, bool gated = false) {
+  return gated ? gam_launch_convmod_t<true>(a, layer_norm, s) : gam_launch_convmod_t<false>(a, layer_norm, s);
+}
+
+template <int VEC>
+__global__ __launch_bounds__(256) void gam_glu_kernel(const float* __restrict__ u, float* __restrict__ y, size_t rows, int d) {
+  const int dq = d / VEC;
+  const size_t total = rows * (size_t)dq;
+  for (size_t i = (size_t)blockIdx.x * 256 + threadIdx.x; i < total; i += (size_t)gridDim.x * 256) {
+    const size_t row = i / dq;
+    const int c = (int)(i % dq) * VEC;
+    const float* up = u + row * (size_t)(2 * d);
+    if (VEC == 4) {
+      const f32x4 va = *reinterpret_cast<const f32x4*>(up + c), vb = *reinterpret_cast<const f32x4*>(up + d + c);
+      f32x4 o;
+      o.x = va.x * gam_sigmoid(vb.x);
+      o.y = va.y * gam_sigmoid(vb.y);
+      o.z = va.z * gam_sigmoid(vb.z);
+      o.w = va.w * gam_sigmoid(vb.w);
+      *reinterpret_cast<f32x4*>(y + row * (size_t)d + c) = o;
+    } else {
+      y[row * (size_t)d + c] = up[c] * gam_sigmoid(up[d + c]);
+    }
+  }
+}
diff --git a/gigaam_amd/csrc/gam_gemm.h b/gigaam_amd/csrc/gam_gemm.h
--- a/gigaam_amd/csrc/gam_gemm.h
+++ b/gigaam_amd/csrc/gam_gemm.h
@@ -230,6 +230,7 @@
   if (a.ldw == 0) a.ldw = a.K;
   if (a.M <= 0 || a.N <= 0) return hipSuccess;
   if (a.K % GAM_GEMM_BK != 0 || a.K <= 0) return hipErrorInvalidValue;
+  if (act == GAM_ACT_GLU) return hipErrorInvalidValue;
   const int grid = gam_cdiv(a.M, GAM_GEMM_BM) * gam_cdiv(a.N, GAM_GEMM_BN);
   switch (act) {
     case GAM_ACT_SILU: gam_launch_gemm_t<GAM_ACT_SILU>(a, grid, stream); break;
@@ -277,7 +278,19 @@
       if (g.R != nullptr) x += g.R[orow * g.ldr + col + e];
       v[e] = x;
     }
-    if (VEC == 4) {
+    if (ACT == GAM_ACT_GLU) {
+      float gt[4];
+#pragma unroll
+      for (int e = 0; e < 4; ++e) gt[e] = __shfl_xor(v[e % VEC], 1);
+      if ((col & 4) == 0) {
+        f32x4 o;
+        o.x = v[0] * gam_sigmoid(gt[0]);
+        o.y = v[1 % VEC] * gam_sigmoid(gt[1]);
+        o.z = v[2 % VEC] * gam_sigmoid(gt[2]);
+        o.w = v[3 % VEC] * gam_sigmoid(gt[3]);
+        *reinterpret_cast<f32x4*>(g.C + orow * g.ldc + col / 2) = o;
+      }
+    } else if (VEC == 4) {
       if (g.c_guard) gam_range_note(g.range_flag, v[0], v[1 % VEC], v[2 % VEC], v[3 % VEC]);
       if (g.c_split) gam_store4(g.C, (size_t)orow * g.ldc, col, v[0], v[1 % VEC], v[2 % VEC], v[3 % VEC], g.c_split);
       else *reinterpret_cast<f32x4*>(g.C + orow * g.ldc + col) = (f32x4){v[0], v[1 % VEC], v[2 % VEC], v[3 % VEC]};
@@ -288,8 +301,11 @@
   }
 }
 
+static inline bool gam_glu_ok(const GamGemmArgs& a) { return a.N % 8 == 0 && a.c_split == 0 && a.R == nullptr; }
+
 static inline hipError_t gam_launch_splitk_reduce(const GamGemmArgs& a, int act, int S, hipStream_t stream) {
   auto al16 = [](const void* p) { return (reinterpret_cast<uintptr_t>(p) & 15) == 0; };
+  if (act == GAM_ACT_GLU && (!gam_glu_ok(a) || a.ldc % 4 != 0 || !al16(a.C) || !al16(a.partial))) return hipErrorInvalidValue;
   const bool vec = a.N % 4 == 0 && a.ldc % 4 == 0 && al16(a.C) && al16(a.partial) &&
                    (a.R == nullptr || (a.ldr % 4 == 0 && al16(a.R)));
   const size_t total = (size_t)a.M * (vec ? a.N / 4 : a.N);
@@ -301,6 +317,7 @@
   switch (act) {
     case GAM_ACT_SILU: GAM_RED(GAM_ACT_SILU); break;
     case GAM_ACT_RELU: GAM_RED(GAM_ACT_RELU); break;
+    case GAM_ACT_GLU: GAM_RED(GAM_ACT_GLU); break;
     default: GAM_RED(GAM_ACT_NONE); break;
   }
 #undef GAM_RED
diff --git a/gigaam_amd/csrc/gam_gemm_sp.h b/gigaam_amd/csrc/gam_gemm_sp.h
--- a/gigaam_amd/csrc/gam_gemm_sp.h
+++ b/gigaam_amd/csrc/gam_gemm_sp.h
@@ -341,7 +341,14 @@
           v[hf] = t;
         }
         if (g.c_guard) { gam_range_note(g.range_flag, v[0].x, v[0].y, v[0].z, v[0].w); gam_range_note(g.range_flag, v[1].x, v[1].y, v[1].z, v[1].w); }
-        if (g.c_split == 2) {
+        if (ACT == GAM_ACT_GLU) {
+          f32x4 o;
+          o.x = v[0].x * gam_sigmoid(v[1].x);
+          o.y = v[0].y * gam_sigmoid(v[1].y);
+          o.z = v[0].z * gam_sigmoid(v[1].z);
+          o.w = v[0].w * gam_sigmoid(v[1].w);
+          *reinterpret_cast<f32x4*>(g.C + orow * g.ldc + (ecol >> 1)) = o;
+        } else if (g.c_split == 2) {
           _Float16* cp = reinterpret_cast<_Float16*>(g.C) + orow * g.ldc + ecol;
           const gam_half4 h0 = __builtin_convertvector(v[0], gam_half4), h1 = __builtin_convertvector(v[1], gam_half4);
           if (both) *reinterpret_cast<gam_half8*>(cp) = (gam_half8){h0[0], h0[1], h0[2], h0[3], h1[0], h1[1], h1[2], h1[3]};
@@ -471,6 +478,7 @@
   if (a.K <= 0 || a.K % 32 != 0 || a.Asp == nullptr || a.Wsp == nullptr) return hipErrorInvalidValue;
   if (a.a_mode == 0 ? (a.lda % 32 != 0) : (a.conv_c % 32 != 0)) return hipErrorInvalidValue;
   if (!gam_gemm_sp_epilogue_ok(a)) return hipErrorInvalidValue;
+  if (act == GAM_ACT_GLU && !gam_glu_ok(a)) return hipErrorInvalidValue;
   int mt = a.sp_mt, nw = a.sp_nw, ns = a.sp_ns;
   if (mt < 2 || mt > 4 || (nw != 2 && nw != 4) || (nw == 2 && mt == 4)) {
     const GamSpPlan p = gam_gemm_sp_plan(a.M, a.N, a.K, a.a_mode);
@@ -523,6 +531,7 @@
   switch (act) {
     case GAM_ACT_SILU: GAM_LSP(GAM_ACT_SILU); break;
     case GAM_ACT_RELU: GAM_LSP(GAM_ACT_RELU); break;
+    case GAM_ACT_GLU: GAM_LSP(GAM_ACT_GLU); break;
     default: GAM_LSP(GAM_ACT_NONE); break;
   }
 #undef GAM_LSP
@@ -582,6 +591,14 @@
   }
 }
 
+__global__ __launch_bounds__(256) void gam_glu_rows_kernel(const float* __restrict__ x, float* __restrict__ y, int d, int K) {
+  const size_t total = (size_t)2 * d * K, stride = (size_t)gridDim.x * 256;
+  for (size_t i = (size_t)blockIdx.x * 256 + threadIdx.x; i < total; i += stride) {
+    const int j = (int)(i / (size_t)K), k = (int)(i % (size_t)K);
+    y[i] = x[(size_t)gam_glu_col(j, d) * K + k];
+  }
+}
+
 __global__ __launch_bounds__(256) void gam_rowscale_kernel(const float* __restrict__ x, float* __restrict__ rs, int rows,
                                                            int K, long lda) {
   const int row = blockIdx.x * 4 + (threadIdx.x >> 6), lane = threadIdx.x & 63;
diff --git a/gigaam_amd/engine.py b/gigaam_amd/engine.py
--- a/gigaam_amd/engine.py
+++ b/gigaam_amd/engine.py
@@ -1278,18 +1278,31 @@
         return out
 
     def op_gemm(self, a: Tensor, w: Tensor, bias: Optional[Tensor] = None, act: int = 0, resid: Optional[Tensor] = None,
-                alpha: float = 1.0) -> Tensor:
+                alpha: float = 1.0, c_split: int = 0) -> Tensor:
         a = self._dev(a, torch.float32)
         w = self._dev(w, torch.float32)
         bias = None if bias is None else self._dev(bias, torch.float32)
         resid = None if resid is None else self._dev(resid, torch.float32)
         m, k = a.shape
         n = w.shape[0]
-        out = torch.empty((m, n), dtype=torch.float32, device=self.device)
-        with torch.cuda.device(self.device):
-            rc = self.lib.gam_op_gemm_ex(self._h, _ptr(a), _ptr(w), _ptr(bias), _ptr(resid), alpha, _ptr(out), m, n, k, act,
-                                         self._stream())
-        self._check(rc, "gam_op_gemm_ex")
+        out = torch.empty((m, n // 2 if act == 3 and not c_split else n), dtype=torch.float32, device=self.device)
+        with torch.cuda.device(self.device):
+            if c_split:
+                rc = self.lib.gam_op_gemm_fmt(self._h, _ptr(a), _ptr(w), _ptr(bias), _ptr(resid), alpha, _ptr(out), m, n, k, act, c_split,
+                                              self._stream())
+            else:
+                rc = self.lib.gam_op_gemm_ex(self._h, _ptr(a), _ptr(w), _ptr(bias), _ptr(resid), alpha, _ptr(out), m, n, k, act,
+                                             self._stream())
+        self._check(rc, "gam_op_gemm_fmt" if c_split else "gam_op_gemm_ex")
+        return out
+
+    def op_glu(self, u: Tensor) -> Tensor:
+        u = self._dev(u, torch.float32).contiguous()
+        rows, d2 = u.shape
+        out = torch.empty((rows, d2 // 2), dtype=torch.float32, device=self.device)
+        with torch.cuda.device(self.device):
+            rc = self.lib.gam_op_glu(self._h, _ptr(u), _ptr(out), rows, d2 // 2, self._stream())
+        self._check(rc, "gam_op_glu")
         return out
 
     def op_attention(self, q: Tensor, k: Tensor, v: Tensor, lens: Optional[Tensor] = None) -> Tensor:
@@ -1343,15 +1356,21 @@
             rc = self.lib.gam_op_layernorm(self._h, C.byref(op), self._stream())
         self._check(rc, "gam_op_layernorm")
 
+    def op_convmod_gated(self, u: Tensor, z: Tensor, dw_w: Tensor, dw_b: Tensor, n_scale: Tensor, n_shift: Tensor, lens: Tensor, B: int,
+                         Ta: int, Tv: int, d: int, ks: int, layer_norm: bool, z_split: int = 0, cu: Optional[Tensor] = None) -> None:
+        self.op_convmod(u, z, dw_w, dw_b, n_scale, n_shift, lens, B, Ta, Tv, d, ks, layer_norm, z_split, cu, _gated=True)
+
     def op_convmod(self, u: Tensor, z: Tensor, dw_w: Tensor, dw_b: Tensor, n_scale: Tensor, n_shift: Tensor, lens: Tensor, B: int,
-                   Ta: int, Tv: int, d: int, ks: int, layer_norm: bool, z_split: int = 0, cu: Optional[Tensor] = None) -> None:
-        what = "op_convmod"
+                   Ta: int, Tv: int, d: int, ks: int, layer_norm: bool, z_split: int = 0, cu: Optional[Tensor] = None,
+                   _gated: bool = False) -> None:
+        what = "op_convmod_gated" if _gated else "op_convmod"
         ptrs = [self._op_ptr(what, n, t) for n, t in (("u", u), ("z", z), ("dw_w", dw_w), ("dw_b", dw_b), ("n_scale", n_scale),
                                                       ("n_shift", n_shift))]
         ptrs += [self._op_ptr(what, "lens", lens, torch.int32), self._op_ptr(what, "cu", cu, torch.int32)]
         with torch.cuda.device(self.device):
-            rc = self.lib.gam_op_convmod(self._h, *ptrs, B, Ta, Tv, d, ks, int(bool(layer_norm)), z_split, self._stream())
-        self._check(rc, "gam_op_convmod")
+            fn = self.lib.gam_op_convmod_gated if _gated else self.lib.gam_op_convmod
+            rc = fn(self._h, *ptrs, B, Ta, Tv, d, ks, int(bool(layer_norm)), z_split, self._stream())
+        self._check(rc, "gam_" + what)
 
     def profile_enable(self, on=True) -> None:
         self._check(self.lib.gam_profile_enable(self._h, int(on)), "gam_profile_enable")
diff --git a/include/gigaam_hip.h b/include/gigaam_hip.h
--- a/include/gigaam_hip.h
+++ b/include/gigaam_hip.h
@@ -176,6 +176,11 @@
                 int M, int N, int K, int act, void* stream);
 int gam_op_gemm_ex(gam_handle* h, const float* A, const float* W, const float* bias, const float* R, float alpha,
                    float* C, int M, int N, int K, int act, void* stream);
+int gam_op_gemm_fmt(gam_handle* h, const float* A, const float* W, const float* bias, const float* R, float alpha,
+                    float* C, int M, int N, int K, int act, int c_split, void* stream);
+int gam_op_glu(gam_handle* h, const float* u, float* y, int64_t rows, int d, void* stream);
+int gam_glu_column(int j, int d);
+int gam_glu_interleave(const float* w, const float* b, int d, int K, float* w_out, float* b_out);
 
 int gam_op_attention(gam_handle* h, const float* q, const float* k, const float* v, float* ctx,
                      const int32_t* lens, int B, int T, int H, void* stream);
@@ -207,6 +212,9 @@
 int gam_op_convmod(gam_handle* h, const float* u, float* z, const float* dw_w, const float* dw_b, const float* n_scale,
                    const float* n_shift, const int32_t* lens, const int32_t* cu, int B, int Ta, int Tv, int d, int ks,
                    int layer_norm, int z_split, void* stream);
+int gam_op_convmod_gated(gam_handle* h, const float* u, float* z, const float* dw_w, const float* dw_b, const float* n_scale,
+                         const float* n_shift, const int32_t* lens, const int32_t* cu, int B, int Ta, int Tv, int d, int ks,
+                         int layer_norm, int z_split, void* stream);
 
 int gam_tune_sp(int mt, int nw, int splitk);
 int gam_plan_sp(int M, int N, int K, int n_cu, int* mt, int* nw, int* splitk);
```
